# bfloat16/latent-diffusion-speech

Measured on AMD Instinct MI355X. Metric: mel_frames_per_sec, higher is better.
Workload: dtype f32; 1 GPU; configs[1]: batch=16x512-frame utterances per GPU, 50-step dpm-solver, unet1d denoiser, 80-ch mel; pipeline=sampler, utterances_per_gpu=16, frames=512, nfe=50, method=dpm-solver, parallelism=batch-shard x1

## Files before the change

latent-diffusion-speech_amd/csrc/attention_k4p.hip:

```cpp
#include "k4p.h"
#include "k8b3.h"
#include "kernels.h"

#include <hip/hip_ext.h>

#include <math.h>

namespace lds {

typedef float f32x16 __attribute__((ext_vector_type(16)));
typedef float f32x4 __attribute__((ext_vector_type(4)));
typedef float f32x2 __attribute__((ext_vector_type(2)));
typedef unsigned int att_u32x4 __attribute__((ext_vector_type(4)));
typedef _Float16 att_f16x8 __attribute__((ext_vector_type(8)));

static __device__ __forceinline__ void att_split8(const f32x4 e0, const f32x4 e1, att_u32x4& p1, att_u32x4& p2) {
    unsigned a[4], b[4];
    k8h_split_pair(e0[0], e0[1], a[0], b[0]);
    k8h_split_pair(e0[2], e0[3], a[1], b[1]);
    k8h_split_pair(e1[0], e1[1], a[2], b[2]);
    k8h_split_pair(e1[2], e1[3], a[3], b[3]);
    p1 = att_u32x4{a[0], a[1], a[2], a[3]};
    p2 = att_u32x4{b[0], b[1], b[2], b[3]};
}
static __device__ __forceinline__ f32x16 att_mfma3(const att_u32x4 a1, const att_u32x4 a2, const att_u32x4 b1, const att_u32x4 b2, f32x16 c) {
    c = __builtin_amdgcn_mfma_f32_32x32x16_f16(__builtin_bit_cast(att_f16x8, a2), __builtin_bit_cast(att_f16x8, b1), c, 0, 0, 0);
    c = __builtin_amdgcn_mfma_f32_32x32x16_f16(__builtin_bit_cast(att_f16x8, a1), __builtin_bit_cast(att_f16x8, b2), c, 0, 0, 0);
    c = __builtin_amdgcn_mfma_f32_32x32x16_f16(__builtin_bit_cast(att_f16x8, a1), __builtin_bit_cast(att_f16x8, b1), c, 0, 0, 0);
    return c;
}

template <int D, int NW, int NST, int KS = 1>
struct AttCfg {
    static constexpr int KB = 64;
    static constexpr int DQ = D / 8, DT = (D + 31) / 32;
    static constexpr int KROWS = DQ * 2;
    static constexpr int VCH = D / 4;
    static constexpr int KPW = KROWS / NW, VPW = VCH / NW;
    static constexpr int PER_TILE = KPW + VPW;
    static constexpr int STAGE = 2 * KB * D;
    static constexpr size_t LDS_BYTES = (size_t)NST * STAGE * sizeof(float) + 256;
    static_assert(KROWS % NW == 0 && VCH % NW == 0, "tile must split evenly over the waves");
    static_assert(KS == 1 || (size_t)(KS - 1) * (NW / KS) * (2 + 16 * DT) * 64 * sizeof(float) <= LDS_BYTES, "the join's partials reuse the K/V stages");
};

static __device__ __forceinline__ float max3(float a, float b, float c) {
    float d;
    asm("v_max3_f32 %0, %1, %2, %3" : "=v"(d) : "v"(a), "v"(b), "v"(c));
    return d;
}

template <int Y, int PER_TILE>
static __device__ __forceinline__ void att_wait_younger(int y) {
    if constexpr (Y == 0) {
        asm volatile("s_waitcnt vmcnt(0)" ::: "memory");
    } else {
        constexpr int N = (Y * PER_TILE > 63) ? 63 : Y * PER_TILE;
        if (y >= Y) asm volatile("s_waitcnt vmcnt(%0)" ::"n"(N) : "memory");
        else att_wait_younger<Y - 1, PER_TILE>(y);
    }
}

template <int D, int NW, int KPW, int VPW>
static __device__ __forceinline__ void att_issue_tile(const __amdgpu_buffer_rsrc_t rk, const __amdgpu_buffer_rsrc_t rv, const int* koff,
                                                      const int* voff, int wave, int kt, float* st) {
#pragma unroll
    for (int i = 0; i < KPW; ++i)
        __builtin_amdgcn_raw_ptr_buffer_load_lds(rk, (__attribute__((address_space(3))) void*)(st + (wave + NW * i) * 256), 16, koff[i], kt * (64 * 16), 0, 0);
#pragma unroll
    for (int i = 0; i < VPW; ++i)
        __builtin_amdgcn_raw_ptr_buffer_load_lds(rv, (__attribute__((address_space(3))) void*)(st + 64 * D + (wave + NW * i) * 256), 16, voff[i],
                                                 kt * (64 * D * 4), 0, 0);
}

template <int D, int NW, int NST, int KS, bool F16>
__global__ void __launch_bounds__(NW * 64) attention_k4p_kernel(const float* __restrict__ qk, const float* __restrict__ vt, float* __restrict__ out,
                                                                int C, int Tbuf, float scale2, int out_bf3, const int* __restrict__ lens, int lvl) {
    using Cfg = AttCfg<D, NW, NST, KS>;
    constexpr int NWQ = NW / KS;
    constexpr int KB = Cfg::KB, DQ = Cfg::DQ, DT = Cfg::DT, KPW = Cfg::KPW, VPW = Cfg::VPW, STAGE = Cfg::STAGE, PER_TILE = Cfg::PER_TILE;
    extern __shared__ __attribute__((aligned(16))) float smem[];
    const int lane = threadIdx.x & 63, wave = __builtin_amdgcn_readfirstlane((int)(threadIdx.x >> 6));
    const int c = lane & 31, h = lane >> 5;
    const int gx = gridDim.x, gy = gridDim.y, total = gx * gy * gridDim.z;
    const int id = (blockIdx.z * gy + blockIdx.y) * gx + blockIdx.x;
    const int per = total >> 3, rem = total & 7, xcd = id & 7;
    const int L = xcd * per + (xcd < rem ? xcd : rem) + (id >> 3);
    const int qblk = L % gx, hd = (L / gx) % gy, b = L / (gx * gy);
    const int qw = wave % NWQ, ks = wave / NWQ;
    const int tq = qblk * (NWQ * 32) + qw * 32 + c;
    const int T = ragged_len(lens, b, lvl, Tbuf);
    const int Tp = Tbuf + 2, T4 = (Tbuf + 3) & ~3;
    const float* qb = qk + ((long long)b * 2 * C + (long long)hd * D) * Tp;

    f32x4 qv[DQ];
#pragma unroll
    for (int kq = 0; kq < DQ; ++kq) {
        qv[kq] = f32x4{0.f, 0.f, 0.f, 0.f};
        if (tq < T) qv[kq] = *reinterpret_cast<const f32x4*>(qb + ((long long)(kq * 2 + h) * Tp + tq + 1) * 4);
    }

    const __amdgpu_buffer_rsrc_t rk =
        __builtin_amdgcn_make_buffer_rsrc(const_cast<float*>(qk + ((long long)b * 2 * C + C + (long long)hd * D) * Tp), 0, D * Tp * 4, 0x00020000);
    const __amdgpu_buffer_rsrc_t rv =
        __builtin_amdgcn_make_buffer_rsrc(const_cast<float*>(vt + ((long long)b * C + (long long)hd * D) * T4), 0, D * T4 * 4, 0x00020000);
    int koff[KPW], voff[VPW];
#pragma unroll
    for (int i = 0; i < KPW; ++i) koff[i] = (((wave + NW * i) * Tp) + lane + 1) * 16;
#pragma unroll
    for (int i = 0; i < VPW; ++i) voff[i] = ((wave + NW * i) * 64 + lane) * 16;
    const int nt = (qblk * (NWQ * 32) >= T) ? 0 : (T + KB - 1) / KB;
    for (int t = 0; t < NST - 1 && t < nt; ++t) att_issue_tile<D, NW, KPW, VPW>(rk, rv, koff, voff, wave, t, smem + t * STAGE);
#pragma unroll
    for (int kq = 0; kq < DQ; ++kq) qv[kq] *= scale2;
    att_u32x4 qh1[F16 ? DQ / 2 : 1], qh2[F16 ? DQ / 2 : 1];
    if constexpr (F16) {
#pragma unroll
        for (int t = 0; t < DQ / 2; ++t) att_split8(qv[2 * t], qv[2 * t + 1], qh1[t], qh2[t]);
    }

    f32x16 o[DT];
#pragma unroll
    for (int i = 0; i < DT; ++i)
#pragma unroll
        for (int r = 0; r < 16; ++r) o[i][r] = 0.f;
    float m_run = -INFINITY, l_run = 0.f;

    const bool resident = (KS == 4) && nt <= NST - 1;
    if (resident) {
        asm volatile("s_waitcnt vmcnt(0)" ::: "memory");
        __builtin_amdgcn_s_barrier();
        asm volatile("" ::: "memory");
    }
    int sc = 0, sn = NST - 1;
    for (int kt = 0; kt < nt; ++kt) {
        if (!resident) {
            const int younger = (nt - 1 - kt < NST - 2) ? (nt - 1 - kt) : (NST - 2);
            att_wait_younger<NST - 2, PER_TILE>(younger);
            __builtin_amdgcn_s_barrier();
            asm volatile("" ::: "memory");
            if (kt + NST - 1 < nt) att_issue_tile<D, NW, KPW, VPW>(rk, rv, koff, voff, wave, kt + NST - 1, smem + sn * STAGE);
        }
        const float* Kc = smem + sc * STAGE;
        const float* Vc = Kc + KB * D;
        const int h0 = (KS == 1) ? 0 : (KS == 2) ? ks : (ks & 1);
        const int h1 = (KS == 1) ? KB / 32 : (KS == 2 || (kt & 1) == (ks >> 1)) ? h0 + 1 : h0;
#pragma unroll 1
        for (int half = h0; half < h1; ++half) {
            const int kbase = kt * KB + half * 32;
            if (kbase >= T) break;
            f32x4 ka[DQ], va[4][DT];
#pragma unroll
            for (int kq = 0; kq < DQ; ++kq) ka[kq] = *reinterpret_cast<const f32x4*>(Kc + ((kq * 2 + h) * KB + half * 32 + c) * 4);
            __builtin_amdgcn_sched_barrier(0);
            f32x16 s;
// ... 53 lines not shown
#pragma unroll
                for (int ss = 0; ss < 2; ++ss) {
                    att_u32x4 p1, p2;
                    att_split8(f32x4{s[8 * ss], s[8 * ss + 1], s[8 * ss + 2], s[8 * ss + 3]}, f32x4{s[8 * ss + 4], s[8 * ss + 5], s[8 * ss + 6], s[8 * ss + 7]}, p1, p2);
#pragma unroll
                    for (int i = 0; i < DT; ++i) {
                        att_u32x4 v1, v2;
                        att_split8(va[2 * ss][i], va[2 * ss + 1][i], v1, v2);
                        o[i] = att_mfma3(v1, v2, p1, p2, o[i]);
                    }
                }
            } else {
#pragma unroll
                for (int g = 0; g < 4; ++g)
#pragma unroll
                    for (int i = 0; i < DT; ++i)
#pragma unroll
                        for (int e = 0; e < 4; ++e) o[i] = __builtin_amdgcn_mfma_f32_32x32x2f32(va[g][i][e], s[4 * g + e], o[i], 0, 0, 0);
            }
        }
        sc = (sc + 1 == NST) ? 0 : sc + 1;
        sn = (sn + 1 == NST) ? 0 : sn + 1;
    }
    if constexpr (KS >= 2) {
        __syncthreads();
        constexpr int RED = (2 + 16 * DT) * 64;
        if (ks >= 1) {
            float* red = smem + ((ks - 1) * NWQ + qw) * RED + lane;
            red[0] = m_run; red[64] = l_run;
#pragma unroll
            for (int i = 0; i < DT; ++i)
#pragma unroll
                for (int r = 0; r < 16; ++r) red[(2 + i * 16 + r) * 64] = o[i][r];
        }
        __syncthreads();
        if (ks >= 1) return;
#pragma unroll
        for (int q = 1; q < KS; ++q) {
            const float* red = smem + ((q - 1) * NWQ + qw) * RED + lane;
            const float m1 = red[0], l1 = red[64];
            const float m = fmaxf(m_run, m1);
            const float a0 = __builtin_amdgcn_exp2f(m_run - m), a1 = __builtin_amdgcn_exp2f(m1 - m);
            l_run = l_run * a0 + l1 * a1;
#pragma unroll
            for (int i = 0; i < DT; ++i)
#pragma unroll
                for (int r = 0; r < 16; ++r) o[i][r] = o[i][r] * a0 + red[(2 + i * 16 + r) * 64] * a1;
            m_run = m;
        }
    }
    float l;
    {
        const auto sw = __builtin_amdgcn_permlane32_swap(__float_as_uint(l_run), __float_as_uint(l_run), false, false);
        l = __uint_as_float(sw[0]) + __uint_as_float(sw[1]);
    }
    if (tq < Tbuf && out_bf3) {
        const bool live = tq < T;
        const float rl = 1.0f / l;
        char* ob = reinterpret_cast<char*>(out);
        const int npl = (out_bf3 == 2) ? 2 : 3;
#pragma unroll
        for (int i = 0; i < DT; ++i)
#pragma unroll
            for (int g = 0; g < 4; ++g) {
                if (i * 32 + 8 * g >= D) break;
                const int q = (hd * D + i * 32) / 8 + g;
                unsigned pa[3], pb[3];
                if (out_bf3 == 2) {
                    sp_split_pair<FMT_F16X2>(o[i][4 * g] * rl, o[i][4 * g + 1] * rl, pa);
                    sp_split_pair<FMT_F16X2>(o[i][4 * g + 2] * rl, o[i][4 * g + 3] * rl, pb);
                } else {
                    sp_split_pair<FMT_BF16X3>(o[i][4 * g] * rl, o[i][4 * g + 1] * rl, pa);
                    sp_split_pair<FMT_BF16X3>(o[i][4 * g + 2] * rl, o[i][4 * g + 3] * rl, pb);
                }
#pragma unroll
                for (int pl = 0; pl < 3; ++pl) {
                    if (pl >= npl) break;
                    char* e = ob + ((((long long)b * (C >> 3) + q) * npl + pl) * Tp + tq + 1) * 16 + h * 8;
                    k8_store_wt(e, live ? k8_u32x2{pa[pl], pb[pl]} : k8_u32x2{0u, 0u});
                    if (tq == 0) *reinterpret_cast<k8_u32x2*>(e - 16) = k8_u32x2{0u, 0u};
                    if (tq == Tbuf - 1) *reinterpret_cast<k8_u32x2*>(e + 16) = k8_u32x2{0u, 0u};
                }
            }
    } else if (tq < Tbuf) {
        const bool live = tq < T;
        const float rl = 1.0f / l;
        float* ob = out + (long long)b * C * Tp;
#pragma unroll
        for (int i = 0; i < DT; ++i)
#pragma unroll
            for (int g = 0; g < 4; ++g) {
                if (i * 32 + 8 * g >= D) break;
                const int q = (hd * D + i * 32) / 8 + g;
#pragma unroll
                for (int hh = 0; hh < 2; ++hh) {
                    const long long off = ((long long)(q * 2 + hh) * Tp + tq + 1) * 4 + 2 * h;
                    k4p_store_wt(ob + off, live ? f32x2{o[i][4 * g + hh] * rl, o[i][4 * g + 2 + hh] * rl} : f32x2{0.f, 0.f});
                    if (tq == 0) *reinterpret_cast<f32x2*>(ob + off - 4) = f32x2{0.f, 0.f};
                    if (tq == Tbuf - 1) *reinterpret_cast<f32x2*>(ob + off + 4) = f32x2{0.f, 0.f};
                }
            }
    }
}

template <int D, int NW, int NST, int KS, bool F16>
static hipError_t launch_cfg(const float* qk, const float* vt, float* out, int B, int C, int T, int heads, float scale, int out_bf3, const int* lens, int lvl, hipStream_t s) {
    using Cfg = AttCfg<D, NW, NST, KS>;
    auto kern = attention_k4p_kernel<D, NW, NST, KS, F16>;
    if (Cfg::LDS_BYTES > 48 * 1024) {
        static std::atomic<unsigned long long> attr_done{0};
        hipError_t e = ensure_max_dynamic_lds(reinterpret_cast<const void*>(kern), attr_done);
        if (e != hipSuccess) return e;
    }
    constexpr int QPB = NW / KS * 32;
    hipEvent_t e0, e1;
    if (prof_attach_events(&e0, &e1)) hipExtLaunchKernelGGL(kern, dim3((T + QPB - 1) / QPB, heads, B), dim3(NW * 64), Cfg::LDS_BYTES, s, e0, e1, 0, qk, vt, out, C, T, scale, out_bf3, lens, lvl);
    else hipLaunchKernelGGL(kern, dim3((T + QPB - 1) / QPB, heads, B), dim3(NW * 64), Cfg::LDS_BYTES, s, qk, vt, out, C, T, scale, out_bf3, lens, lvl);
    return hipGetLastError();
}

template <int D, bool F16>
static hipError_t launch_dk(const float* qk, const float* vt, float* out, int B, int C, int T, int heads, int out_bf3, int tile_batch, const int* lens, int lvl, hipStream_t s) {
    const float scale = 1.4426950408889634f / sqrtf((float)D);
    constexpr int NST = (D == 64) ? 2 : 3;
    const long long hb = (long long)heads * (tile_batch > 0 ? tile_batch : 16);
    if ((long long)((T + 127) / 128) * hb >= 512) return launch_cfg<D, 4, NST, 1, F16>(qk, vt, out, B, C, T, heads, scale, out_bf3, lens, lvl, s);
    constexpr int NSTL = (D == 32) ? 9 : (D == 48) ? 5 : 4;
    if (tile_batch > 0 && T > 64 && (long long)((T + 63) / 64) * hb < 256) return launch_cfg<D, 4, NSTL, 4, F16>(qk, vt, out, B, C, T, heads, scale, out_bf3, lens, lvl, s);
    if (T > 32) return launch_cfg<D, 4, NST, 2, F16>(qk, vt, out, B, C, T, heads, scale, out_bf3, lens, lvl, s);
    return launch_cfg<D, 1, 2, 1, F16>(qk, vt, out, B, C, T, heads, scale, out_bf3, lens, lvl, s);
}

static hipError_t attention_any(const float* qk, const float* vt, float* out, int B, int C, int T, int heads, int out_bf3, bool math_f16, int tile_batch, hipStream_t s,
                                const int* lens = nullptr, int lvl = 0) {
    if (C % heads) return hipErrorInvalidValue;
    ProfScope ps(s, math_f16 ? "attention_f16" : "attention", 4.0 * B * (double)T * T * C, 4.0 * 4.0 * B * C * T, true);
    if (math_f16) {
        switch (C / heads) {
            case 32: return launch_dk<32, true>(qk, vt, out, B, C, T, heads, out_bf3, tile_batch, lens, lvl, s);
            case 48: return launch_dk<48, true>(qk, vt, out, B, C, T, heads, out_bf3, tile_batch, lens, lvl, s);
            case 64: return launch_dk<64, true>(qk, vt, out, B, C, T, heads, out_bf3, tile_batch, lens, lvl, s);
            default: return hipErrorInvalidValue;
        }
    }
    switch (C / heads) {
        case 32: return launch_dk<32, false>(qk, vt, out, B, C, T, heads, out_bf3, tile_batch, lens, lvl, s);
        case 48: return launch_dk<48, false>(qk, vt, out, B, C, T, heads, out_bf3, tile_batch, lens, lvl, s);
        case 64: return launch_dk<64, false>(qk, vt, out, B, C, T, heads, out_bf3, tile_batch, lens, lvl, s);
        default: return hipErrorInvalidValue;
    }
}
hipError_t launch_attention_k4p(const float* qk, const float* vt, float* out, int B, int C, int T, int heads, hipStream_t s, int tile_batch, const int* lens, int lvl) {
    return attention_any(qk, vt, out, B, C, T, heads, 0, false, tile_batch, s, lens, lvl);
}
hipError_t launch_attention_k4p_out_bf3(const float* qk, const float* vt, void* out, int B, int C, int T, int heads, hipStream_t s, int fmt, int tile_batch, const int* lens, int lvl) {
    return attention_any(qk, vt, (float*)out, B, C, T, heads, fmt == FMT_F16X2 ? 2 : 1, fmt == FMT_F16X2, tile_batch, s, lens, lvl);
}
template <int NW, int NST, int KS>
__global__ void __launch_bounds__(NW * 64) attention_k4p_rel_kernel(const float* __restrict__ qk, const float* __restrict__ vt, const float* __restrict__ relp,
                                                                    float* __restrict__ out, int C, int Tbuf, float scale2, const int* __restrict__ qlens,
                                                                    const int* __restrict__ klens, int left, int right) {
    constexpr int D = 64;
    using Cfg = AttCfg<D, NW, NST, KS>;
    constexpr int NWQ = NW / KS;
    constexpr int KB = Cfg::KB, DQ = Cfg::DQ, DT = Cfg::DT, KPW = Cfg::KPW, VPW = Cfg::VPW, STAGE = Cfg::STAGE, PER_TILE = Cfg::PER_TILE;
    static_assert(KS == 1 || KS == 2, "no latency-mode variant");
    extern __shared__ __attribute__((aligned(16))) float smem[];
    const int lane = threadIdx.x & 63, wave = __builtin_amdgcn_readfirstlane((int)(threadIdx.x >> 6));
    const int c = lane & 31, h = lane >> 5;
    const int gx = gridDim.x, gy = gridDim.y, total = gx * gy * gridDim.z;
    const int id = (blockIdx.z * gy + blockIdx.y) * gx + blockIdx.x;
    const int per = total >> 3, rem = total & 7, xcd = id & 7;
    const int Lid = xcd * per + (xcd < rem ? xcd : rem) + (id >> 3);
    const int qblk = Lid % gx, hd = (Lid / gx) % gy, b = Lid / (gx * gy);
    const int qw = wave % NWQ, ks = wave / NWQ;
    const int q0 = qblk * (NWQ * 32) + qw * 32;
    const int tq = q0 + c;
    const int Tq = qlens ? (qlens[b] < Tbuf ? qlens[b] : Tbuf) : Tbuf;
    const int Tk = klens ? (klens[b] < Tq ? klens[b] : Tq) : Tq;
    const int Tp = Tbuf + 2, T4 = (Tbuf + 3) & ~3;
    const float* qb = qk + ((long long)b * 2 * C + (long long)hd * D) * Tp;

    f32x4 qv[DQ];
#pragma unroll
// ... 58 lines not shown
            __builtin_amdgcn_sched_barrier(0);
            if (kbase - q0 - 31 >= right) {
#pragma unroll
                for (int r = 0; r < 16; ++r) s[r] += pR;
            } else if (kbase + 31 - q0 <= -left) {
#pragma unroll
                for (int r = 0; r < 16; ++r) s[r] += pL;
            } else {
#pragma unroll
                for (int r = 0; r < 16; ++r) {
                    int d = kbase + (r & 3) + 8 * (r >> 2) + 4 * h - tq;
                    d = d < -left ? -left : (d > right ? right : d);
                    s[r] += rp[d + left];
                }
            }
            if (kbase + 32 > Tk) {
#pragma unroll
                for (int r = 0; r < 16; ++r)
                    if (kbase + (r & 3) + 8 * (r >> 2) + 4 * h >= Tk) s[r] = -INFINITY;
            }
            float mt = max3(max3(max3(s[0], s[1], s[2]), max3(s[3], s[4], s[5]), max3(s[6], s[7], s[8])),
                            max3(max3(s[9], s[10], s[11]), max3(s[12], s[13], s[14]), s[15]), m_run);
            {
                const auto sw = __builtin_amdgcn_permlane32_swap(__float_as_uint(mt), __float_as_uint(mt), false, false);
                mt = max3(mt, __uint_as_float(sw[0]), __uint_as_float(sw[1]));
            }
            const float alpha = __builtin_amdgcn_exp2f(m_run - mt);
            m_run = mt;
            const f32x2 mm = {mt, mt}, aa = {alpha, alpha};
            f32x2 lsum = {0.f, 0.f};
#pragma unroll
            for (int r = 0; r < 16; r += 2) {
                const f32x2 d = f32x2{s[r], s[r + 1]} - mm;
                s[r] = __builtin_amdgcn_exp2f(d[0]);
                s[r + 1] = __builtin_amdgcn_exp2f(d[1]);
                lsum += f32x2{s[r], s[r + 1]};
            }
            l_run = fmaf(l_run, alpha, lsum[0] + lsum[1]);
#pragma unroll
            for (int i = 0; i < DT; ++i)
#pragma unroll
                for (int r = 0; r < 16; r += 2) {
                    const f32x2 t = f32x2{o[i][r], o[i][r + 1]} * aa;
                    o[i][r] = t[0]; o[i][r + 1] = t[1];
                }
#pragma unroll
            for (int g = 0; g < 4; ++g)
#pragma unroll
                for (int i = 0; i < DT; ++i)
#pragma unroll
                    for (int e = 0; e < 4; ++e) o[i] = __builtin_amdgcn_mfma_f32_32x32x2f32(va[g][i][e], s[4 * g + e], o[i], 0, 0, 0);
        }
        sc = (sc + 1 == NST) ? 0 : sc + 1;
        sn = (sn + 1 == NST) ? 0 : sn + 1;
    }
    if constexpr (KS == 2) {
        __syncthreads();
        constexpr int RED = (2 + 16 * DT) * 64;
        if (ks >= 1) {
            float* red = smem + qw * RED + lane;
            red[0] = m_run; red[64] = l_run;
#pragma unroll
            for (int i = 0; i < DT; ++i)
#pragma unroll
                for (int r = 0; r < 16; ++r) red[(2 + i * 16 + r) * 64] = o[i][r];
        }
        __syncthreads();
        if (ks >= 1) return;
        const float* red = smem + qw * RED + lane;
        const float m1 = red[0], l1 = red[64];
        const float m = fmaxf(m_run, m1);
        const float a0 = (m_run == -INFINITY) ? 0.f : __builtin_amdgcn_exp2f(m_run - m), a1 = (m1 == -INFINITY) ? 0.f : __builtin_amdgcn_exp2f(m1 - m);
        l_run = l_run * a0 + l1 * a1;
#pragma unroll
        for (int i = 0; i < DT; ++i)
#pragma unroll
            for (int r = 0; r < 16; ++r) o[i][r] = o[i][r] * a0 + red[(2 + i * 16 + r) * 64] * a1;
    }
    float l;
    {
        const auto sw = __builtin_amdgcn_permlane32_swap(__float_as_uint(l_run), __float_as_uint(l_run), false, false);
        l = __uint_as_float(sw[0]) + __uint_as_float(sw[1]);
    }
    if (tq < Tbuf) {
        const bool live = tq < Tq;
        const float rl = 1.0f / l;
        float* ob = out + (long long)b * C * Tp;
#pragma unroll
        for (int i = 0; i < DT; ++i)
#pragma unroll
            for (int g = 0; g < 4; ++g) {
                const int q = (hd * D + i * 32) / 8 + g;
#pragma unroll
                for (int hh = 0; hh < 2; ++hh) {
                    const long long off = ((long long)(q * 2 + hh) * Tp + tq + 1) * 4 + 2 * h;
                    k4p_store_wt(ob + off, live ? f32x2{o[i][4 * g + hh] * rl, o[i][4 * g + 2 + hh] * rl} : f32x2{0.f, 0.f});
                    if (tq == 0) *reinterpret_cast<f32x2*>(ob + off - 4) = f32x2{0.f, 0.f};
                    if (tq == Tbuf - 1) *reinterpret_cast<f32x2*>(ob + off + 4) = f32x2{0.f, 0.f};
                }
            }
    }
}

template <int NW, int NST, int KS>
static hipError_t launch_rel_cfg(const float* qk, const float* vt, const float* relp, float* out, int B, int C, int T, int heads, const int* qlens,
                                 const int* klens, int left, int right, hipStream_t s) {
    using Cfg = AttCfg<64, NW, NST, KS>;
    auto kern = attention_k4p_rel_kernel<NW, NST, KS>;
    if (Cfg::LDS_BYTES > 48 * 1024) {
        static std::atomic<unsigned long long> attr_done{0};
        hipError_t e = ensure_max_dynamic_lds(reinterpret_cast<const void*>(kern), attr_done);
        if (e != hipSuccess) return e;
    }
    constexpr int QPB = NW / KS * 32;
    const float scale = 1.4426950408889634f / 8.0f;
    hipEvent_t e0, e1;
    const dim3 grid((T + QPB - 1) / QPB, heads, B);
    if (prof_attach_events(&e0, &e1)) hipExtLaunchKernelGGL(kern, grid, dim3(NW * 64), Cfg::LDS_BYTES, s, e0, e1, 0, qk, vt, relp, out, C, T, scale, qlens, klens, left, right);
    else hipLaunchKernelGGL(kern, grid, dim3(NW * 64), Cfg::LDS_BYTES, s, qk, vt, relp, out, C, T, scale, qlens, klens, left, right);
    return hipGetLastError();
}

hipError_t launch_attention_k4p_rel(const float* qk, const float* vt, const float* relp, float* out, int B, int C, int T, int heads, const int* qlens,
                                    const int* klens, int left, int right, hipStream_t s) {
    if (B <= 0 || heads < 1 || C != heads * 64 || T <= 0 || left < 0 || right < 0 || left + right + 1 > kW2vbertRelStride) return hipErrorInvalidValue;
    ProfScope ps(s, "attention_rel", 4.0 * B * (double)T * T * C, 4.0 * 4.0 * B * C * T, true);
    if ((long long)((T + 127) / 128) * heads * 16 >= 512) return launch_rel_cfg<4, 2, 1>(qk, vt, relp, out, B, C, T, heads, qlens, klens, left, right, s);
    if (T > 32) return launch_rel_cfg<4, 2, 2>(qk, vt, relp, out, B, C, T, heads, qlens, klens, left, right, s);
    return launch_rel_cfg<1, 2, 1>(qk, vt, relp, out, B, C, T, heads, qlens, klens, left, right, s);
}

hipError_t launch_attention_k4p_f16math(const float* qk, const float* vt, float* out, int B, int C, int T, int heads, hipStream_t s, int tile_batch) {
    return attention_any(qk, vt, out, B, C, T, heads, 0, true, tile_batch, s);
}

}
```

latent-diffusion-speech_amd/csrc/conv_dma.hip:

```cpp
#include "gn_chan.h"
#include "k4p.h"
#include "kernels.h"

#include <hip/hip_ext.h>

#include <stdio.h>
#include <stdlib.h>

namespace lds {

typedef float f32x16 __attribute__((ext_vector_type(16)));
typedef float f32x4 __attribute__((ext_vector_type(4)));
typedef float f32x2 __attribute__((ext_vector_type(2)));

static __device__ __forceinline__ float erf_fast(float x) {
    const float ax = fabsf(x);
    const float t = __builtin_amdgcn_rcpf(fmaf(0.3275911f, ax, 1.0f));
    float pl = fmaf(1.061405429f, t, -1.453152027f);
    pl = fmaf(pl, t, 1.421413741f);
    pl = fmaf(pl, t, -0.284496736f);
    pl = fmaf(pl, t, 0.254829592f);
    const float e = __builtin_amdgcn_exp2f(ax * ax * -1.4426950408889634f);
    return copysignf(fmaf(-pl * t, e, 1.0f), x);
}

template <int CTRL, int ROW_MASK, bool BOUND>
static __device__ __forceinline__ float dpp_add(float v) {
    return v + __builtin_bit_cast(float, __builtin_amdgcn_update_dpp(0, __builtin_bit_cast(int, v), CTRL, ROW_MASK, 0xf, BOUND));
}
static __device__ __forceinline__ float wave_sum_to_lane63(float v) {
    v = dpp_add<0x111, 0xf, true>(v);
    v = dpp_add<0x112, 0xf, true>(v);
    v = dpp_add<0x114, 0xf, true>(v);
    v = dpp_add<0x118, 0xf, true>(v);
    v = dpp_add<0x142, 0xa, false>(v);
    v = dpp_add<0x143, 0xc, false>(v);
    return v;
}

template <int BM, int BN, int KT, int STRIDE, bool UPS, int BK, int NST, int DIL = 1>
struct DmaCfg {
    static constexpr bool SPLIT = BM == 32;
    static constexpr int TM = SPLIT ? 1 : BM / 64, TN = BN / 64;
    static constexpr int KR = BK / 4;
    static constexpr int XW = UPS ? (BN / 2 + 2) : ((BN - 1) * STRIDE + (KT - 1) * DIL + 1);
    static constexpr int WI = KT * KR * BM / 64;
    static constexpr int WPW = WI / 4;
    static constexpr int RPW = KR / 4;
    static constexpr int NXI = (RPW * XW + 63) / 64;
    static constexpr int PER_TILE = WPW + NXI;
    static constexpr int KQW = SPLIT ? BK / 16 : BK / 8;
    static constexpr int G = KT * KQW;
    static constexpr int NB = (G % 3 == 0 && TM * TN < 4) ? 3 : 2;
    static constexpr int NACC = (TM * TN >= 2) ? 1 : 2;
    static constexpr int STAGE = KT * BK * BM + KR * XW * 4;
    static constexpr size_t LDS_BYTES = (size_t)NST * STAGE * sizeof(float);
    static constexpr int OCC_LDS = (int)((160 * 1024) / LDS_BYTES);
    static constexpr int OCC = (TM * TN >= 4) ? (OCC_LDS < 2 ? OCC_LDS : 2) : (OCC_LDS < 4 ? (OCC_LDS < 1 ? 1 : OCC_LDS) : 4);
    static_assert(WI % 4 == 0 && KR % 4 == 0, "tile does not split evenly over 4 waves");
    static_assert(!SPLIT || (BN == 64 && BK % 16 == 0), "split-K tile is 32 x 64");
};

template <int BM, int BN, int KT, int STRIDE, bool UPS, int BK, int NST, int DIL = 1, bool VOC = false, bool GNF = false, bool GELU = false, int ACT2 = 0>
struct DmaKernel {
    using Cfg = DmaCfg<BM, BN, KT, STRIDE, UPS, BK, NST, DIL>;
    static constexpr int TM = Cfg::TM, TN = Cfg::TN, KR = Cfg::KR, XW = Cfg::XW, WPW = Cfg::WPW, RPW = Cfg::RPW, NXI = Cfg::NXI;
    static constexpr int G = Cfg::G, NB = Cfg::NB, NACC = Cfg::NACC, STAGE = Cfg::STAGE, PER_TILE = Cfg::PER_TILE, KQW = Cfg::KQW;
    static constexpr bool SPLIT = Cfg::SPLIT;

    const DmaConvArgs& p;
    float* smem;
    int lane, wave, c, h, wm, wn, ks, b, m0, t0;
    int ksp, kc0, ctile;
    int Lout;
    float gcg[GNF ? 8 : 1], gkc;
    GnPart gp0, gp1;
    float gs, gsn, ginv;
    int kofs_a, kofs_b;
    int woff[WPW];
    int xoff[NXI];
    __amdgpu_buffer_rsrc_t rw, rx1, rx2;
    bool xact[NXI];
    int arow;
    int bcol[TN];
    f32x16 acc[NACC][TM][TN];
    f32x4 aop[NB][TM], bop[NB][TN];
    float lmu[TN], lrs[TN];
    static constexpr bool EARLY = TM * TN == 1 || VOC;
    f32x2 rsv[EARLY ? TM * TN * 8 : 1];
    float kbv[EARLY ? TM * 16 : 1];

    __device__ __forceinline__ DmaKernel(const DmaConvArgs& p_, float* s_) : p(p_), smem(s_) {}

    __device__ __forceinline__ void setup_keep_acc() {
        const int tid = threadIdx.x;
        lane = tid & 63;
        wave = __builtin_amdgcn_readfirstlane(tid >> 6);
        c = lane & 31; h = lane >> 5;
        wm = SPLIT ? 0 : wave >> 1; ks = SPLIT ? wave >> 1 : 0; wn = wave & 1;
        kofs_a = ks * KQW * 2 * BM * 4; kofs_b = ks * KQW * 2 * XW * 4;
        const int nMb = p.Mp / BM;
        const int gx = gridDim.x, total = gx * gridDim.y;
        const int id = blockIdx.y * gx + blockIdx.x;
        const int xcd = id & 7, slot = id >> 3, per = total >> 3, rem = total & 7;
        const int L = xcd * per + (xcd < rem ? xcd : rem) + slot;
        const int mb = L % nMb;
        const int tb = L / nMb;
        const int nN = gx / nMb;
        const int nb = tb % nN;
        const int by = tb / nN, S = p.ksplit > 1 ? p.ksplit : 1;
        b = by / S; ksp = by - b * S;
        kc0 = ksp * (p.Ci / BK / S);
        ctile = (b * nN + nb) * nMb + mb;
        m0 = mb * BM; t0 = nb * BN;
        Lout = ragged_len(p.lens, b, p.lvl_out, p.To);
#pragma unroll
        for (int i = 0; i < WPW; ++i) {
            const int q = (wave + 4 * i) * 64 + lane;
            const int tap = q / (KR * BM);
            const int rem = q - tap * (KR * BM);
            const int rr = rem / BM, m = rem - rr * BM;
            woff[i] = ((tap * (p.Ci / 4) + rr) * p.Mp + m0 + m) * 16;
        }
        const int Tp = p.Tsrc + 2 * p.xpad;
        const int e0 = UPS ? (((t0 - 1) >> 1) + p.xpad) : (t0 * STRIDE - p.pad + p.xpad);
#pragma unroll
        for (int i = 0; i < NXI; ++i) {
            const int qq = i * 64 + lane;
            const int rl = qq / XW, col = qq - rl * XW;
            xact[i] = qq < RPW * XW;
            xoff[i] = ((wave * RPW + rl) * Tp + e0 + col) * 16;
        }
        rw = __builtin_amdgcn_make_buffer_rsrc(const_cast<float*>(p.w), 0, KT * p.Ci * p.Mp * 4, 0x00020000);
        rx1 = __builtin_amdgcn_make_buffer_rsrc(const_cast<float*>(p.x1 + (long long)b * p.C1 * Tp), 0, p.C1 * Tp * 4, 0x00020000);
        rx2 = __builtin_amdgcn_make_buffer_rsrc(const_cast<float*>(p.x2 ? p.x2 + (long long)b * p.C2 * Tp : p.x1), 0, p.C2 * Tp * 4, 0x00020000);
        arow = wm * TM * 32 + c;
#pragma unroll
        for (int j = 0; j < TN; ++j) bcol[j] = wn * TN * 32 + j * 32 + c;
    }
    __device__ __forceinline__ bool dead_tile() const { return !VOC && p.lens && t0 >= Lout; }
    __device__ __forceinline__ int voc_len() const { return p.vlen[b]; }
    __device__ __forceinline__ void setup() {
        setup_keep_acc();
#pragma unroll
        for (int a = 0; a < NACC; ++a)
#pragma unroll
            for (int i = 0; i < TM; ++i)
#pragma unroll
                for (int j = 0; j < TN; ++j)
#pragma unroll
                    for (int r = 0; r < 16; ++r) acc[a][i][j][r] = 0.f;
    }

    __device__ __forceinline__ void issue_tile(int kc, float* st) {
        const int ws = kc * (KR * 16) * p.Mp;
#pragma unroll
        for (int i = 0; i < WPW; ++i)
            __builtin_amdgcn_raw_ptr_buffer_load_lds(rw, (__attribute__((address_space(3))) void*)(st + ((wave + 4 * i) * 64) * 4), 16, woff[i], ws, 0, 0);
        const int k0 = kc * BK;
        const bool s2 = k0 >= p.C1;
        const int xsoff = (s2 ? k0 - p.C1 : k0) * (p.Tsrc + 2 * p.xpad) * 4;
        float* xs = st + KT * BK * BM + wave * RPW * XW * 4;
#pragma unroll
        for (int i = 0; i < NXI; ++i)
            if (xact[i]) {
                if (s2) __builtin_amdgcn_raw_ptr_buffer_load_lds(rx2, (__attribute__((address_space(3))) void*)(xs + i * 64 * 4), 16, xoff[i], xsoff, 0, 0);
                else __builtin_amdgcn_raw_ptr_buffer_load_lds(rx1, (__attribute__((address_space(3))) void*)(xs + i * 64 * 4), 16, xoff[i], xsoff, 0, 0);
            }
    }

    template <int SLOT>
    __device__ __forceinline__ void load_ops(const float* st, int tap, int kq) {
        const float* wt = st + ((tap * KR + kq * 2 + h) * BM + arow) * 4 + kofs_a;
        const float* xs = st + KT * BK * BM + (kq * 2 + h) * XW * 4 + kofs_b;
#pragma unroll
        for (int i = 0; i < TM; ++i) aop[SLOT][i] = *reinterpret_cast<const f32x4*>(wt + i * 32 * 4);
#pragma unroll
        for (int j = 0; j < TN; ++j) {
            const int col = UPS ? (((t0 + bcol[j] + tap - 1) >> 1) - ((t0 - 1) >> 1)) : (bcol[j] * STRIDE + tap * DIL);
            bop[SLOT][j] = *reinterpret_cast<const f32x4*>(xs + col * 4);
        }
    }
    template <int SLOT>
    __device__ __forceinline__ void mfma_ops() {
        if constexpr (GNF) {
#pragma unroll
            for (int j = 0; j < TN; ++j) bop[SLOT][j] *= gs;
        }
#pragma unroll
        for (int jj = 0; jj < 4; ++jj)
#pragma unroll
            for (int i = 0; i < TM; ++i)
#pragma unroll
                for (int j = 0; j < TN; ++j)
                    acc[jj % NACC][i][j] = __builtin_amdgcn_mfma_f32_32x32x2f32(aop[SLOT][i][jj], bop[SLOT][j][jj], acc[jj % NACC][i][j], 0, 0, 0);
    }
    template <int g0, int g1>
    __device__ __forceinline__ void preload(const float* cur) {
        if constexpr (g0 < g1 && g0 < G) {
            load_ops<g0 % NB>(cur, g0 / KQW, g0 % KQW);
            preload<g0 + 1, g1>(cur);
        }
    }
    __device__ __forceinline__ void tile_sync(int kc, int nk, float* cur) {
        const int younger = (nk - 2 - kc < NST - 2) ? (nk - 2 - kc) : (NST - 2);
        wait_younger<NST - 2>(younger);
        asm volatile("s_waitcnt lgkmcnt(0)" ::: "memory");
        __builtin_amdgcn_s_barrier();
        asm volatile("" ::: "memory");
        if (kc + NST < nk) issue_tile(kc0 + kc + NST, cur);
    }
    template <int g>
    __device__ __forceinline__ void kstep(float* cur, const float* nxt, int kc, int nk) {
        if constexpr (g < G) {
            constexpr int gp = g + NB - 1;
            if constexpr (gp < G) {
                load_ops<gp % NB>(cur, gp / KQW, gp % KQW);
            } else {
                if (kc + 1 < nk) {
                    if constexpr (gp == G) tile_sync(kc, nk, cur);
                    load_ops<gp % NB>(nxt, (gp - G) / KQW, (gp - G) % KQW);
                }
            }
            mfma_ops<g % NB>();
            __builtin_amdgcn_sched_barrier(0);
            kstep<g + 1>(cur, nxt, kc, nk);
        }
    }

    __device__ __forceinline__ void ln_columns() {
#pragma unroll
        for (int j = 0; j < TN; ++j) {
            const int n = t0 + wn * TN * 32 + j * 32 + c;
            const bool ok = n < p.To;
            const float2* src = p.ln_part + (long long)b * p.ln_np * p.Tsrc + (ok ? n : 0);
            ln_column_stats(src, p.Tsrc, p.ln_np, p.ln_eps, ok, lmu[j], lrs[j]);
        }
    }

    __device__ __forceinline__ float* gnf_tail() const { return smem + NST * STAGE + BM; }
    __device__ __forceinline__ int gnf_group(int k) const {
        const int pos = (kc0 + k) * BK + ks * (SPLIT ? BK / 2 : BK);
        const int g = (int)(((float)pos + 0.5f) * ginv);
        return g < p.gnf_groups ? g : p.gnf_groups - 1;
    }
    __device__ __forceinline__ void gnf_request() {
        const int G_ = p.gnf_groups, gsz = p.Ci / G_;
        const int gTv = ragged_len(p.lens, b, p.lvl_in, p.Tsrc);
        ginv = 1.0f / (float)gsz;
        gp0 = gn_part_load(p.gnf_part, b, p.Ci, p.Tsrc, gsz >> 4, wave, lane, 0, gTv);
        gp1 = gn_part_load(p.gnf_part, b, p.Ci, p.Tsrc, gsz >> 4, (wave + 4 < G_) ? wave + 4 : wave, lane, 0, gTv);
        if ((int)threadIdx.x < BM) {
            const int m = m0 + (int)threadIdx.x;
            gkc = p.gnf_c2[m];
#pragma unroll
            for (int g = 0; g < 8; ++g) gcg[g] = (g < G_) ? p.gnf_cg[g * p.Mp + m] : 0.f;
        }
    }
    __device__ __forceinline__ void gnf_prepare() {
        const int G_ = p.gnf_groups, gsz = p.Ci / G_;
        float* tail = gnf_tail();
#pragma unroll
        for (int e = 0; e < 2; ++e) {
            const int g = wave + 4 * e;
            float rs = 1.f, rm = 0.f;
            if (g < G_) {
                float mu, var;
                gnf_group_stats(p.gnf_part, b, p.Ci, p.Tsrc, gsz >> 4, g, lane, e ? gp1 : gp0, mu, var, ragged_len(p.lens, b, p.lvl_in, p.Tsrc));
                rs = __builtin_amdgcn_rsqf(var + p.gnf_eps); rm = rs * mu;
            }
            if (lane == 0) { tail[g] = rs; tail[8 + g] = rm; }
        }
        asm volatile("s_waitcnt lgkmcnt(0)" ::: "memory");
    }
    __device__ __forceinline__ void gnf_rows() {
        const float* tail = gnf_tail();
        if ((int)threadIdx.x < BM) {
            float kc = gkc;
#pragma unroll
            for (int g = 0; g < 8; ++g) kc = fmaf(-tail[8 + g], gcg[g], kc);
            smem[NST * STAGE + threadIdx.x] = kc;
        }
        gs = tail[gnf_group(0)];
        gsn = tail[gnf_group(1)];
    }
    __device__ __forceinline__ void gnf_advance(int k) {
        gs = gsn;
        gsn = gnf_tail()[gnf_group(k + 2)];
    }

    template <int Y>
    __device__ __forceinline__ void wait_younger(int y) {
        if constexpr (Y == 0) {
            asm volatile("s_waitcnt vmcnt(0)" ::: "memory");
        } else {
            constexpr int N = (Y * PER_TILE > 63) ? 63 : Y * PER_TILE;
            if (y >= Y) asm volatile("s_waitcnt vmcnt(%0)" ::"n"(N) : "memory");
            else wait_younger<Y - 1>(y);
        }
    }

    __device__ __forceinline__ bool res_tile(int tile0, int n) const {
        return p.res && tile0 < p.plain_from && tile0 < p.Cout && n < p.To;
    }
    __device__ __forceinline__ void early_loads() {
#pragma unroll
        for (int i = 0; i < TM; ++i) {
            const int tile0 = m0 + wm * TM * 32 + i * 32;
#pragma unroll
            for (int j = 0; j < TN; ++j) {
                const int n = t0 + wn * TN * 32 + j * 32 + c;
                f32x2* rs = rsv + (i * TN + j) * 8;
#pragma unroll
                for (int e = 0; e < 8; ++e) rs[e] = f32x2{0.f, 0.f};
                if (res_tile(tile0, n)) {
                    const int Tpo = p.To + 2 * p.opad;
                    const float* rb = p.res + (long long)b * k4p_ck() * Tpo + k4p_off(tile0, n);
#pragma unroll
                    for (int e = 0; e < 8; ++e) rs[e] = *reinterpret_cast<const f32x2*>(rb + e * Tpo * 4);
                }
            }
#pragma unroll
            for (int r = 0; r < 16; ++r) kbv[i * 16 + r] = (p.bias && !p.ln_part) ? p.bias[tile0 + (r & 3) + 8 * (r >> 2) + 4 * h] : 0.f;
        }
    }

    __device__ __forceinline__ void mainloop() {
        static_assert(G % NB == 0 && NB - 1 <= G, "ring slots must keep their phase across K-steps");
        const int nk = p.Ci / BK / (p.ksplit > 1 ? p.ksplit : 1);
        if constexpr (GNF) gnf_request();
        if constexpr (EARLY) early_loads();
        for (int t = 0; t < NST && t < nk; ++t) issue_tile(kc0 + t, smem + t * STAGE);
        if (p.ln_part) ln_columns();
        if constexpr (GNF) gnf_prepare();
        wait_younger<NST - 1>((nk - 1 < NST - 1) ? nk - 1 : NST - 1);
        __builtin_amdgcn_s_barrier();
        asm volatile("" ::: "memory");
        if constexpr (GNF) gnf_rows();
        preload<0, NB - 1>(smem);
        int sc = 0;
        for (int kc = 0; kc < nk; ++kc) {
            const int sn = (sc + 1 == NST) ? 0 : sc + 1;
            kstep<0>(smem + sc * STAGE, smem + sn * STAGE, kc, nk);
            sc = sn;
            if constexpr (GNF) gnf_advance(kc);
        }
        if constexpr (GNF) __syncthreads();
    }

    __device__ __forceinline__ void finalize(bool geglu) {
        if constexpr (NACC == 2) {
#pragma unroll
            for (int i = 0; i < TM; ++i)
#pragma unroll
                for (int j = 0; j < TN; ++j) acc[0][i][j] += acc[1][i][j];
        }
        const bool ln = p.ln_part != nullptr;
        if (EARLY && !ln) {
#pragma unroll
            for (int i = 0; i < TM; ++i)
#pragma unroll
                for (int j = 0; j < TN; ++j)
#pragma unroll
                    for (int r = 0; r < 16; ++r) acc[0][i][j][r] += kbv[i * 16 + r];
        } else if (ln || p.bias) {
            float k1[TM][16], k2[TM][16];
#pragma unroll
            for (int i = 0; i < TM; ++i)
#pragma unroll
                for (int r = 0; r < 16; ++r) {
                    const int m = m0 + wm * TM * 32 + i * 32 + (r & 3) + 8 * (r >> 2) + 4 * h;
                    k1[i][r] = ln ? p.ln_c1[m] : 0.f;
                    k2[i][r] = ln ? p.ln_c2[m] : p.bias[m];
                }
#pragma unroll
            for (int i = 0; i < TM; ++i)
#pragma unroll
                for (int j = 0; j < TN; ++j)
#pragma unroll
                    for (int r = 0; r < 16; ++r) {
                        const float v = acc[0][i][j][r];
                        acc[0][i][j][r] = ln ? lrs[j] * (v - lmu[j] * k1[i][r]) + k2[i][r] : v + k2[i][r];
                    }
        }
        if constexpr (GNF) {
#pragma unroll
            for (int i = 0; i < TM; ++i)
#pragma unroll
                for (int r = 0; r < 16; ++r) {
                    const float kc = smem[NST * STAGE + wm * TM * 32 + i * 32 + (r & 3) + 8 * (r >> 2) + 4 * h];
#pragma unroll
                    for (int j = 0; j < TN; ++j) acc[0][i][j][r] += kc;
                }
        }
        if (geglu) {
#pragma unroll
            for (int j = 0; j < TN; ++j)
#pragma unroll
                for (int r = 0; r < 16; ++r) {
                    const float g = acc[0][TM - 1][j][r];
                    if constexpr (ACT2 == 2) acc[0][0][j][r] *= 1.0f / (1.0f + expf(-g));
                    else acc[0][0][j][r] *= 0.5f * g * (1.0f + erf_fast(g * 0.70710678118654752440f));
                }
        }
        if constexpr (ACT2 == 1) {
#pragma unroll
            for (int i = 0; i < TM; ++i)
#pragma unroll
                for (int j = 0; j < TN; ++j)
#pragma unroll
                    for (int r = 0; r < 16; ++r) {
                        const float v = acc[0][i][j][r];
                        acc[0][i][j][r] = v / (1.0f + expf(-v));
                    }
        }
        if constexpr (GELU) {
#pragma unroll
            for (int i = 0; i < TM; ++i)
#pragma unroll
                for (int j = 0; j < TN; ++j)
#pragma unroll
                    for (int r = 0; r < 16; ++r) {
                        const float v = acc[0][i][j][r];
                        acc[0][i][j][r] = 0.5f * v * (1.0f + erf_fast(v * 0.70710678118654752440f));
                    }
        }
// ... 16 lines not shown
            if (c0 + rl < Cn) ob[rl * p.To] = v;
        }
    }

    __device__ __forceinline__ void store_vt(int c0, int i, int j, int n) {
        const int T4 = (p.To + 3) & ~3, D = p.vt_D, Cv = p.Cout - p.plain_from;
        if (n >= T4) return;
        const bool real = n < p.To;
        const int head0 = c0 / D, rem0 = c0 - head0 * D;
        float* ob = p.out2 + (long long)b * Cv * T4 + (long long)(n >> 2) * D * 4 + (n & 3);
#pragma unroll
        for (int r = 0; r < 16; ++r) {
            const int rl = (r & 3) + 8 * (r >> 2) + 4 * h;
            int d = rem0 + rl, head = head0;
            if (d >= D) { d -= D; ++head; }
            if (c0 + rl < Cv) ob[(long long)head * D * T4 + d * 4] = real ? acc[0][i][j][r] : 0.f;
        }
    }

    __device__ __forceinline__ int k4p_off(int tile0, int n) const { return (((tile0 >> 3) * 2) * (p.To + 2 * p.opad) + n + p.opad) * 4 + 2 * h; }
    __device__ __forceinline__ int k4p_ck() const { return (p.plain_from < p.Cout) ? p.plain_from : p.Cout; }

    __device__ __forceinline__ void add_residual(int tile0, int i, int j, int n) {
        if (n >= p.To) return;
        f32x2 rv[8];
        if constexpr (EARLY) {
#pragma unroll
            for (int e = 0; e < 8; ++e) rv[e] = rsv[(i * TN + j) * 8 + e];
        } else {
            const int Tpo = p.To + 2 * p.opad;
            const float* rb = p.res + (long long)b * k4p_ck() * Tpo + k4p_off(tile0, n);
#pragma unroll
            for (int e = 0; e < 8; ++e) rv[e] = *reinterpret_cast<const f32x2*>(rb + e * Tpo * 4);
        }
#pragma unroll
        for (int g = 0; g < 4; ++g)
#pragma unroll
            for (int hh = 0; hh < 2; ++hh) {
                acc[0][i][j][4 * g + hh] += rv[2 * g + hh][0];
                acc[0][i][j][4 * g + 2 + hh] += rv[2 * g + hh][1];
            }
    }

    __device__ __forceinline__ void add_running_sum(int tile0, int i, int j, int n) {
        if (n >= p.To) return;
        const int Tpo = p.To + 2 * p.opad;
        const float* ab = p.acc_in + (long long)b * (p.out_plain ? p.Cout : k4p_ck()) * Tpo + k4p_off(tile0, n);
        f32x2 av[8];
#pragma unroll
        for (int e = 0; e < 8; ++e) av[e] = *reinterpret_cast<const f32x2*>(ab + e * Tpo * 4);
#pragma unroll
        for (int g = 0; g < 4; ++g)
#pragma unroll
            for (int hh = 0; hh < 2; ++hh) {
                acc[0][i][j][4 * g + hh] += av[2 * g + hh][0];
                acc[0][i][j][4 * g + 2 + hh] += av[2 * g + hh][1];
            }
    }

    __device__ __forceinline__ void store_phases(int tile0, int i, int j, int n) {
        const int lg = p.ph_log2, Tpo = p.ph_Tout + 2 * p.opad;
        const long long ob = (long long)b * p.ph_Cout * Tpo;
        const int Lv = p.vlen ? voc_len() : 0x7fffffff;
#pragma unroll
        for (int r = 0; r < 16; ++r) {
            const int m = tile0 + (r & 3) + 8 * (r >> 2) + 4 * h;
            const int co = m >> lg, f = (n << lg) + (m & ((1 << lg) - 1)) - p.ph_tpad;
            const bool ok = n < p.To && f >= 0 && f < p.ph_Tout && co < p.ph_Cout;
            const long long off = ob + (long long)(((co >> 3) * 2 + (co & 1)) * Tpo + f + p.opad) * 4 + ((co & 7) >> 1);
            const float v = (f < Lv) ? acc[0][i][j][r] : 0.f;
            if (ok) {
                p.out[off] = v;
                if (p.out_act) p.out_act[off] = (v >= 0.f) ? v : v * p.act_slope;
            }
        }
    }

    __device__ __forceinline__ void store_k4p(int tile0, int i, int j, int n) {
        const int Tpo = p.To + 2 * p.opad;
        const int Ck = k4p_ck();
        const bool ok = n < p.To;
        const long long o0 = (long long)b * Ck * Tpo + k4p_off(tile0, n);
        float* ob = p.out + o0;
        if (ok) {
            if constexpr (VOC) {
            if constexpr (BN < 256) {
                if (p.vlen && n >= voc_len()) {
#pragma unroll
                    for (int r = 0; r < 16; ++r) acc[0][i][j][r] = 0.f;
                }
            }
            if (p.out_div != 1.0f) {
#pragma unroll
                for (int r = 0; r < 16; ++r) acc[0][i][j][r] = acc[0][i][j][r] / p.out_div;
            }
            if (p.act_slope != 0.f && p.out_act) {
#pragma unroll
                for (int g = 0; g < 4; ++g)
#pragma unroll
                    for (int hh = 0; hh < 2; ++hh) k4p_store_wt(ob + (2 * g + hh) * Tpo * 4, f32x2{acc[0][i][j][4 * g + hh], acc[0][i][j][4 * g + 2 + hh]});
                ob = p.out_act + o0;
            }
            if (p.act_slope != 0.f) {
#pragma unroll
                for (int r = 0; r < 16; ++r) { const float v = acc[0][i][j][r]; acc[0][i][j][r] = (v >= 0.f) ? v : v * p.act_slope; }
            }
            }
#pragma unroll
            for (int g = 0; g < 4; ++g)
#pragma unroll
                for (int hh = 0; hh < 2; ++hh)
                    k4p_store_wt(ob + (2 * g + hh) * Tpo * 4, f32x2{acc[0][i][j][4 * g + hh], acc[0][i][j][4 * g + 2 + hh]});
            if (p.opad == 1) {
                if (n == 0) {
#pragma unroll
                    for (int e = 0; e < 8; ++e) *reinterpret_cast<f32x2*>(ob + e * Tpo * 4 - 4) = f32x2{0.f, 0.f};
                }
                if (n == p.To - 1) {
#pragma unroll
                    for (int e = 0; e < 8; ++e) *reinterpret_cast<f32x2*>(ob + e * Tpo * 4 + 4) = f32x2{0.f, 0.f};
                }
            }
        }
        if (p.gnpart_out) {
            const float k0 = __builtin_bit_cast(float, __builtin_amdgcn_readfirstlane(__builtin_bit_cast(int, acc[0][i][j][0])));
            const float k1 = __builtin_bit_cast(float, __builtin_amdgcn_readfirstlane(__builtin_bit_cast(int, acc[0][i][j][8])));
            float a1 = 0.f, a2 = 0.f, b1 = 0.f, b2 = 0.f;
#pragma unroll
            for (int r = 0; r < 8; ++r) {
                const float d0 = acc[0][i][j][r] - k0, d1 = acc[0][i][j][r + 8] - k1;
                a1 += d0; a2 = fmaf(d0, d0, a2);
                b1 += d1; b2 = fmaf(d1, d1, b2);
            }
            if (n >= Lout) { a1 = 0.f; a2 = 0.f; b1 = 0.f; b2 = 0.f; }
            a1 = wave_sum_to_lane63(a1); a2 = wave_sum_to_lane63(a2);
            b1 = wave_sum_to_lane63(b1); b2 = wave_sum_to_lane63(b2);
            const int n0 = n - c;
            const int nv = (Lout - n0 < 32) ? Lout - n0 : 32;
            if (lane == 63 && nv > 0) {
                const float cnt = 16.0f * (float)nv, rc = 1.0f / cnt;
                float2* gp = p.gnpart_out + ((long long)b * (Ck >> 4) + (tile0 >> 4)) * ((p.To + 31) >> 5) + (n0 >> 5);
                gp[0] = make_float2(k0 + a1 * rc, fmaxf(a2 - a1 * a1 * rc, 0.f));
                if (tile0 + 16 < Ck) gp[(p.To + 31) >> 5] = make_float2(k1 + b1 * rc, fmaxf(b2 - b1 * b1 * rc, 0.f));
            }
        }
        if (p.lnpart_out) {
            float s1 = 0.f;
#pragma unroll
            for (int r = 0; r < 16; ++r) s1 += acc[0][i][j][r];
            const float m16 = s1 * (1.0f / 16.0f);
            float qv = 0.f;
#pragma unroll
            for (int r = 0; r < 16; ++r) { const float d = acc[0][i][j][r] - m16; qv += d * d; }
            const float mo = __shfl_xor(m16, 32, 64), qo = __shfl_xor(qv, 32, 64);
            const float d = mo - m16;
            if (h == 0 && ok)
                p.lnpart_out[((long long)b * (Ck >> 5) + (tile0 >> 5)) * p.To + n] = make_float2(0.5f * (m16 + mo), (qv + qo) + d * d * 8.0f);
        }
    }

    __device__ __forceinline__ int tile_ch(int i, bool geglu) const {
        return geglu ? (m0 + wm * 64) / 2 : (m0 + wm * TM * 32 + i * 32);
    }

    __device__ __forceinline__ bool join_halves() {
        if constexpr (NACC == 2) acc[0][0][0] += acc[1][0][0];
        __syncthreads();
        float* red = smem + wn * 16 * 64 + lane;
        if (ks == 1) {
#pragma unroll
            for (int r = 0; r < 16; ++r) red[r * 64] = acc[0][0][0][r];
        }
        __syncthreads();
        if (ks == 1) return false;
#pragma unroll
        for (int r = 0; r < 16; ++r) acc[0][0][0][r] += red[r * 64];
        if constexpr (NACC == 2) acc[1][0][0] = f32x16{0.f, 0.f, 0.f, 0.f, 0.f, 0.f, 0.f, 0.f, 0.f, 0.f, 0.f, 0.f, 0.f, 0.f, 0.f, 0.f};
        return true;
    }

    __device__ __forceinline__ bool cluster_join() {
        const int S = p.ksplit;
        if constexpr (NACC == 2) {
#pragma unroll
            for (int i = 0; i < TM; ++i)
#pragma unroll
                for (int j = 0; j < TN; ++j) {
                    acc[0][i][j] += acc[1][i][j];
#pragma unroll
// ... 29 lines not shown
            const float* pq = all + (long long)q * (TM * TN * 1024);
#pragma unroll
            for (int i = 0; i < TM; ++i)
#pragma unroll
                for (int j = 0; j < TN; ++j)
#pragma unroll
                    for (int r = 0; r < 16; ++r) acc[0][i][j][r] += __hip_atomic_load(pq + ((i * TN + j) * 16 + r) * 64, __ATOMIC_RELAXED, __HIP_MEMORY_SCOPE_AGENT);
        }
        if (threadIdx.x == 0) __hip_atomic_store(p.kcount + ctile, 0u, __ATOMIC_RELAXED, __HIP_MEMORY_SCOPE_AGENT);
        return true;
    }

    __device__ __forceinline__ void epilogue() {
        const bool geglu = (p.epi == EPI_GEGLU || (ACT2 == 2 && p.epi == EPI_GLU)) && (TM == 2);
        if constexpr (SPLIT) {
            if (!join_halves()) return;
        }
        if constexpr (TM * TN <= 2 && !VOC) {
            if (p.ksplit > 1) {
                if (!cluster_join()) return;
            }
        }
        finalize(geglu);
        const int ni = geglu ? 1 : TM;
        if (p.res) {
#pragma unroll
            for (int i = 0; i < TM; ++i) {
                if (i >= ni) break;
#pragma unroll
                for (int j = 0; j < TN; ++j) {
                    const int tile0 = tile_ch(i, geglu);
                    if (tile0 < p.plain_from && tile0 < p.Cout) add_residual(tile0, i, j, t0 + wn * TN * 32 + j * 32 + c);
                }
            }
        }
        if constexpr (VOC) {
            if (p.acc_in) {
#pragma unroll
                for (int i = 0; i < TM; ++i)
#pragma unroll
                    for (int j = 0; j < TN; ++j) {
                        const int tile0 = tile_ch(i, geglu);
                        if (tile0 < p.Cout) add_running_sum(tile0, i, j, t0 + wn * TN * 32 + j * 32 + c);
                    }
            }
        } else {
            if (p.lens) {
#pragma unroll
                for (int j = 0; j < TN; ++j) {
                    if (t0 + wn * TN * 32 + j * 32 + c >= Lout) {
#pragma unroll
                        for (int i = 0; i < TM; ++i)
#pragma unroll
                            for (int r = 0; r < 16; ++r) acc[0][i][j][r] = 0.f;
                    }
                }
            }
        }
#pragma unroll
        for (int i = 0; i < TM; ++i) {
            if (i >= ni) break;
#pragma unroll
            for (int j = 0; j < TN; ++j) {
                const int n = t0 + wn * TN * 32 + j * 32 + c;
                const int tile0 = tile_ch(i, geglu);
                if constexpr (VOC && KT == 2) {
                    if (p.ph_Tout) { store_phases(tile0, i, j, n); continue; }
                }
                if (p.out_plain) store_plain(p.out, p.Cout, tile0, i, j, n);
                else if (tile0 >= p.plain_from) {
                    if (p.vt_D) store_vt(tile0 - p.plain_from, i, j, n);
                    else store_plain(p.out2, p.Cout - p.plain_from, tile0 - p.plain_from, i, j, n);
                }
                else if (tile0 < p.Cout) store_k4p(tile0, i, j, n);
            }
        }
    }
};

template <int BM, int BN, int KT, int STRIDE, bool UPS, int BK, int NST, int DIL = 1, bool VOC = false, bool GNF = false, bool GELU = false, int ACT2 = 0>
__global__ void __launch_bounds__(256, ((VOC && KT == 2) ? 2 : DmaCfg<BM, BN, KT, STRIDE, UPS, BK, NST, DIL>::OCC)) conv_dma_kernel(const DmaConvArgs p) {
    extern __shared__ __attribute__((aligned(16))) float smem[];
    DmaKernel<BM, BN, KT, STRIDE, UPS, BK, NST, DIL, VOC, GNF, GELU, ACT2> k(p, smem);
    k.setup();
    if (!k.dead_tile()) k.mainloop();
    k.epilogue();
}

struct DmaPairArgs { DmaConvArgs a3, a1; };

template <int BM, int BN, int BK3, int BK1, int NST>
struct PairCfg {
    using C3 = DmaCfg<BM, BN, 3, 1, false, BK3, NST, 1>;
    using C1 = DmaCfg<BM, BN, 1, 1, false, BK1, NST, 1>;
    static constexpr size_t LDS_BYTES = C3::LDS_BYTES > C1::LDS_BYTES ? C3::LDS_BYTES : C1::LDS_BYTES;
    static constexpr int OCC = C3::OCC < C1::OCC ? C3::OCC : C1::OCC;
    static_assert(C3::NACC == C1::NACC && C3::TM == C1::TM && C3::TN == C1::TN && C3::SPLIT == C1::SPLIT, "the phases share the accumulators");
};

template <int BM, int BN, int BK3, int BK1, int NST>
__global__ void __launch_bounds__(256, (PairCfg<BM, BN, BK3, BK1, NST>::OCC)) conv_dma_pair_kernel(const DmaPairArgs pp) {
    extern __shared__ __attribute__((aligned(16))) float smem[];
    using K3 = DmaKernel<BM, BN, 3, 1, false, BK3, NST, 1, false>;
    using K1 = DmaKernel<BM, BN, 1, 1, false, BK1, NST, 1, false>;
    K1 k1(pp.a1, smem);
    {
        K3 k3(pp.a3, smem);
        k3.setup();
        if (!k3.dead_tile()) k3.mainloop();
#pragma unroll
        for (int a = 0; a < K3::NACC; ++a)
#pragma unroll
            for (int i = 0; i < K3::TM; ++i)
#pragma unroll
                for (int j = 0; j < K3::TN; ++j) k1.acc[a][i][j] = k3.acc[a][i][j];
    }
    __syncthreads();
    k1.setup_keep_acc();
    if (!k1.dead_tile()) k1.mainloop();
    k1.epilogue();
}

static thread_local char g_dcfg[96] = "";
const char* conv_dma_last_config() { return g_dcfg; }

template <int BM, int BN, int KT, int STRIDE, bool UPS, int BK, int NST, int DIL = 1, bool VOC = false, bool GNF = false, bool GELU = false, int ACT2 = 0>
static hipError_t launch_dma_cfg(const DmaConvArgs& a, hipStream_t s) {
    using Cfg = DmaCfg<BM, BN, KT, STRIDE, UPS, BK, NST, DIL>;
    if (GNF != (a.gnf_part != nullptr) || GELU != (a.epi == EPI_GELU) || (ACT2 == 1) != (a.epi == EPI_SWISH) || (ACT2 == 2) != (a.epi == EPI_GLU)) return hipErrorInvalidValue;
    const size_t lds_bytes = Cfg::LDS_BYTES + (GNF ? (BM + 32) * sizeof(float) : 0);
    const int nN = (a.To + BN - 1) / BN;
    const int S = a.ksplit > 1 ? a.ksplit : 1;
    if (S > 1 && (Cfg::TM * Cfg::TN > 2 || VOC || (a.Ci / BK) % S)) return hipErrorInvalidValue;
    dim3 grid((a.Mp / BM) * nN, a.B * S);
    auto kern = conv_dma_kernel<BM, BN, KT, STRIDE, UPS, BK, NST, DIL, VOC, GNF, GELU, ACT2>;
    if (lds_bytes > 48 * 1024) {
        static std::atomic<unsigned long long> attr_done{0};
        hipError_t e = ensure_max_dynamic_lds(reinterpret_cast<const void*>(kern), attr_done);
        if (e != hipSuccess) return e;
    }
    const char* gtag = GNF ? " GNF" : GELU ? " GELU" : ACT2 == 1 ? " SWISH" : ACT2 == 2 ? " GLU" : "";
    if (!VOC && S > 1) snprintf(g_dcfg, sizeof(g_dcfg), "BM%d BN%d KT%d S%d U%d BK%d NST%d KS%d%s grid %ux%u lds %zu", BM, BN, KT, STRIDE, (int)UPS, BK, NST, S, gtag, grid.x, grid.y, lds_bytes);
    else if (!VOC) snprintf(g_dcfg, sizeof(g_dcfg), "BM%d BN%d KT%d S%d U%d BK%d NST%d%s grid %ux%u lds %zu", BM, BN, KT, STRIDE, (int)UPS, BK, NST, gtag, grid.x, grid.y, lds_bytes);
    else snprintf(g_dcfg, sizeof(g_dcfg), "BM%d BN%d KT%d S%d U%d BK%d NST%d D%d grid %ux%u lds %zu", BM, BN, KT, STRIDE, (int)UPS, BK, NST, DIL, grid.x, grid.y, Cfg::LDS_BYTES);
    hipEvent_t e0, e1;
    if (prof_attach_events(&e0, &e1)) hipExtLaunchKernelGGL(kern, grid, dim3(256), lds_bytes, s, e0, e1, 0, a);
    else hipLaunchKernelGGL(kern, grid, dim3(256), lds_bytes, s, a);
    return hipGetLastError();
}

#define DCASE(BM, BN, KT, ST, UP, BK, NS) return launch_dma_cfg<BM, BN, KT, ST, UP, BK, NS>(a, s)

static void dma_pick(const DmaConvArgs& a, int cfg, int& bm, int& bn, int& bk, int& nst) {
    const bool k32 = (a.Ci % 32 == 0) && (a.C1 % 32 == 0), k64 = (a.Ci % 64 == 0) && (a.C1 % 64 == 0);
    const long long kNominalBatch = a.tile_batch > 0 ? a.tile_batch : 16;
    auto blocks = [&](int bm, int bn) -> long long { return (a.Mp % bm) ? -1 : (long long)(a.Mp / bm) * ((a.To + bn - 1) / bn) * kNominalBatch; };
    if (cfg) {
        bm = cfg / 1000000; bn = (cfg / 1000) % 1000; bk = (cfg / 10) % 100; nst = cfg % 10;
    } else if (a.stride == 1 && !a.ups && a.epi != EPI_GEGLU && k32 && (blocks(64, 64) <= 256 || (blocks(64, 64) < 512 && blocks(64, 64) % 256))) {
        bm = 32; bn = 64; bk = (a.KT == 1 && k64) ? 64 : 32; nst = 2;
    } else {
        struct Cand { int bm, bn, bk, nst; double eff; };
        Cand cands[3];
        int nc = 0;
        if (a.stride == 2 || a.ups) {
            cands[nc++] = {64, 64, 32, 2, 0.93};
        } else if (a.KT == 3) {
            cands[nc++] = {64, 64, 32, 2, 0.93};
            if (a.Mp % 128 == 0) cands[nc++] = {128, 128, 16, 2, 1.0};
        } else if (a.epi == EPI_GEGLU) {
            if (a.To > 64) cands[nc++] = {128, 128, a.Ci >= 384 ? 16 : 32, 2, 1.0};
            else cands[nc++] = {128, 64, 32, 2, 0.97};
        } else {
            if (a.Ci > 512) cands[nc++] = {64, 64, 64, 2, 0.93};
            else if (blocks(64, 64) <= 768) cands[nc++] = {64, 64, 32, 2, 0.93};
            else cands[nc++] = {64, 64, 16, 3, 0.93};
            if (a.Mp % 128 == 0) cands[nc++] = {128, 64, 32, 2, 0.97};
        }
        double best = 1e300;
        bm = cands[0].bm; bn = cands[0].bn; bk = cands[0].bk; nst = cands[0].nst;
        for (int i = 0; i < nc; ++i) {
            const Cand& c = cands[i];
            const long long nblk = blocks(c.bm, c.bn);
            if (nblk < 0) continue;
            const int xw = a.ups ? c.bn / 2 + 2 : (c.bn - 1) * a.stride + a.KT;
            const double lds = 4.0 * c.nst * (a.KT * c.bk * c.bm + (c.bk / 4) * xw * 4);
            int r = (int)(160.0 * 1024 / lds);
            r = r < 1 ? 1 : (r > 4 ? 4 : r);
            if (c.bm * c.bn >= 128 * 128 && r > 2) r = 2;
            const long long n = (nblk + 255) / 256;
            static const double e[5] = {1.0, 0.62, 0.9, 1.0, 1.0};
            const double cost = ((double)(n / r) * r / e[r] + (double)(n % r) / e[n % r]) * c.bm * c.bn / c.eff;
            if (cost < best) { best = cost; bm = c.bm; bn = c.bn; bk = c.bk; nst = c.nst; }
        }
        if (bm == 128 && bn == 128 && (long long)(a.Mp / 128) * ((a.To + 127) / 128) * a.B < 192) bn = 64;
    }
}

static int cluster_split(const DmaConvArgs& a, int bm, int bn, int nk, int nk2, int min_steps) {
    if (a.tile_batch <= 0 || !a.kpart || !a.kcount || a.voc || bm * bn > 128 * 64) return 1;
    const int blk = bm * bn > 64 * 64 ? 2 : 1;
    const long long tiles = (long long)(a.Mp / bm) * ((a.To + bn - 1) / bn) * a.B;
    if (tiles * 4 > a.kcount_cap) return 1;
    int S = 1;
    while (S < 16 && tiles * S * 2 <= 256 && nk % (S * 2) == 0 && nk / (S * 2) >= min_steps && (nk2 == 0 || (nk2 % (S * 2) == 0)) &&
           tiles * 4 * (S * 2) * blk * 1024 <= a.kpart_cap)
        S *= 2;
    return S;
}

template <int BM, int BN, int BK3, int BK1, int NST>
static hipError_t launch_pair_cfg(const DmaConvArgs& a3, const DmaConvArgs& a1, hipStream_t s) {
    using Cfg = PairCfg<BM, BN, BK3, BK1, NST>;
    const int nN = (a1.To + BN - 1) / BN;
    const int S = a1.ksplit > 1 ? a1.ksplit : 1;
    if (S > 1 && (Cfg::C1::TM * Cfg::C1::TN != 1 || a3.ksplit != a1.ksplit || (a3.Ci / BK3) % S || (a1.Ci / BK1) % S)) return hipErrorInvalidValue;
    dim3 grid((a1.Mp / BM) * nN, a1.B * S);
    auto kern = conv_dma_pair_kernel<BM, BN, BK3, BK1, NST>;
    if (Cfg::LDS_BYTES > 48 * 1024) {
        static std::atomic<unsigned long long> attr_done{0};
        hipError_t e = ensure_max_dynamic_lds(reinterpret_cast<const void*>(kern), attr_done);
        if (e != hipSuccess) return e;
    }
    if (S > 1) snprintf(g_dcfg, sizeof(g_dcfg), "BM%d BN%d KT3+1 S1 U0 BK%d+%d NST%d KS%d grid %ux%u lds %zu", BM, BN, BK3, BK1, NST, S, grid.x, grid.y, Cfg::LDS_BYTES);
    else snprintf(g_dcfg, sizeof(g_dcfg), "BM%d BN%d KT3+1 S1 U0 BK%d+%d NST%d grid %ux%u lds %zu", BM, BN, BK3, BK1, NST, grid.x, grid.y, Cfg::LDS_BYTES);
    DmaPairArgs pp{a3, a1};
    hipEvent_t e0, e1;
    if (prof_attach_events(&e0, &e1)) hipExtLaunchKernelGGL(kern, grid, dim3(256), Cfg::LDS_BYTES, s, e0, e1, 0, pp);
    else hipLaunchKernelGGL(kern, grid, dim3(256), Cfg::LDS_BYTES, s, pp);
    return hipGetLastError();
}

static int pair_variant(const DmaConvArgs& a3, const DmaConvArgs& a1) {
    auto plain = [](const DmaConvArgs& a) {
        return !a.voc && a.stride == 1 && !a.ups && a.dil == 1 && a.epi == EPI_NONE && a.xpad == 1 && a.opad == 1 && !a.ln_part && !a.ph_Tout && a.act_slope == 0.f &&
               !a.acc_in && a.out_div == 1.0f && a.Ci % 16 == 0 && a.C1 % 16 == 0 && a.Mp % 64 == 0 && a.B > 0 && a.To > 0;
    };
    if (!plain(a3) || !plain(a1) || a3.KT != 3 || a3.pad != 1 || a1.KT != 1 || a1.pad != 0 || a3.Mp != a1.Mp || a3.To != a1.To || a3.B != a1.B ||
        a3.Tsrc != a1.Tsrc || a1.res || a1.out_plain || a1.plain_from < a1.Cout || a1.lnpart_out)
        return 0;
    int bm, bn, bk, nst;
    dma_pick(a3, 0, bm, bn, bk, nst);
    const bool k3_32 = (a3.Ci % 32 == 0) && (a3.C1 % 32 == 0);
    const bool k1_64 = (a1.Ci % 64 == 0) && (a1.C1 % 64 == 0), k1_32 = (a1.Ci % 32 == 0) && (a1.C1 % 32 == 0);
    if (!k3_32 || bk != 32 || nst != 2 || !k1_32 || bn != 64 || (bm != 32 && bm != 64)) return 0;
    return (bm << 16) | (bn << 8) | (k1_64 ? 64 : 32);
}
bool conv_dma_pair_applies(const DmaConvArgs& a3, const DmaConvArgs& a1) { return pair_variant(a3, a1) != 0; }

hipError_t launch_conv_dma_pair(const DmaConvArgs& a3_, const DmaConvArgs& a1_, hipStream_t s) {
    DmaConvArgs a3 = a3_, a1 = a1_;
    const int pv = pair_variant(a3, a1);
    if (pv) {
        const int bm = pv >> 16, bn = (pv >> 8) & 255, bk1 = pv & 255;
        a3.ksplit = a1.ksplit = cluster_split(a1, bm, bn, a3.Ci / 32, a1.Ci / bk1, 1);
    }
    switch (pv) {
        case (32 << 16) | (64 << 8) | 64: return launch_pair_cfg<32, 64, 32, 64, 2>(a3, a1, s);
        case (32 << 16) | (64 << 8) | 32: return launch_pair_cfg<32, 64, 32, 32, 2>(a3, a1, s);
        case (64 << 16) | (64 << 8) | 64: return launch_pair_cfg<64, 64, 32, 64, 2>(a3, a1, s);
        case (64 << 16) | (64 << 8) | 32: return launch_pair_cfg<64, 64, 32, 32, 2>(a3, a1, s);
        default: return hipErrorNotSupported;
    }
}

hipError_t launch_conv_dma(const DmaConvArgs& a_, int cfg, hipStream_t s) {
    DmaConvArgs a = a_;
    a.ksplit = 1;
    if (a.Ci % 16 || a.C1 % 16 || a.Mp % 64 || a.B <= 0 || a.To <= 0 || a.xpad < 1 || a.opad < 1 || a.pad < 0 || a.pad > a.xpad) return hipErrorInvalidValue;
    if (a.voc) {
        if (a.stride != 1 || a.ups || a.epi != EPI_NONE || cfg != 0) return hipErrorInvalidValue;
        if (a.ph_Tout) {
            if (a.KT != 2 || a.dil != 1 || a.pad != 1 || a.res || a.acc_in || a.out_plain || a.out_div != 1.0f || a.ph_log2 < 0 || a.ph_log2 > 4 ||
                a.ph_Cout << a.ph_log2 != a.Co || a.ph_Cout % 8)
                return hipErrorInvalidValue;
            return launch_dma_cfg<64, 128, 2, 1, false, 16, 2, 1, true>(a, s);
        }
#define VCASE(KT_, D_) if (a.KT == KT_ && a.dil == D_) return launch_dma_cfg<64, 128, KT_, 1, false, 16, 2, D_, true>(a, s)
        if (a.Mp == 64 && a.KT == 11 && a.To >= 1024 && !a.vlen) {
#define WCASE(D_) if (a.dil == D_) return launch_dma_cfg<64, 256, 11, 1, false, 16, 2, D_, true>(a, s)
            WCASE(1); WCASE(3); WCASE(5);
#undef WCASE
        }
        VCASE(3, 1); VCASE(3, 3); VCASE(3, 5); VCASE(7, 1); VCASE(7, 3); VCASE(7, 5); VCASE(11, 1); VCASE(11, 3); VCASE(11, 5);
#undef VCASE
        return hipErrorInvalidValue;
    }
    if (a.dil != 1 || a.act_slope != 0.f || a.acc_in || a.out_div != 1.0f || a.ph_Tout) return hipErrorInvalidValue;
    if (a.KT != 1 && a.KT != 3 && !(a.KT == 2 && a.stride == 2 && (a.epi == EPI_GELU || a.epi == EPI_NONE))) return hipErrorInvalidValue;
    const bool k32 = (a.Ci % 32 == 0) && (a.C1 % 32 == 0), k64 = (a.Ci % 64 == 0) && (a.C1 % 64 == 0);
    int bm, bn, bk, nst;
    if (a.epi == EPI_GLU) {
        DmaConvArgs t = a;
        t.epi = EPI_GEGLU;
        dma_pick(t, cfg, bm, bn, bk, nst);
    } else {
        dma_pick(a, cfg, bm, bn, bk, nst);
    }
    if ((a.epi == EPI_GEGLU || a.epi == EPI_GLU) && bm != 128) return hipErrorInvalidValue;
    if (a.Mp % bm) return hipErrorInvalidValue;
// ... 34 lines not shown
            if (k32) ECASE(64, 64, 1, 1, 32, 2);
            ECASE(64, 64, 1, 1, 16, 2);
        } else if (a.KT == 3 && a.stride == 1) {
            if (bm == 128 && bn == 128) ECASE(128, 128, 3, 1, 16, 2);
            if (bm == 128 && bn == 64) ECASE(128, 64, 3, 1, 16, 2);
            if (k32) ECASE(64, 64, 3, 1, 32, 2);
            ECASE(64, 64, 3, 1, 16, 2);
        } else if (a.KT == 3 && a.stride == 2) {
            if (k32) ECASE(64, 64, 3, 2, 32, 2);
            ECASE(64, 64, 3, 2, 16, 2);
        } else if (a.KT == 2 && a.stride == 2) {
            if (k32) ECASE(64, 64, 2, 2, 32, 2);
            ECASE(64, 64, 2, 2, 16, 2);
        }
#undef ECASE
        return hipErrorInvalidValue;
    }
    if (cfg == 0) a.ksplit = cluster_split(a, bm, bn, a.Ci / bk, 0, 2);
    const int key = a.KT * 100 + a.stride * 10 + (a.ups ? 1 : 0);
    const int tk = bm * 1000 + bn;
    if (key == 110) {
        if (tk == 64064) {
            if (bk == 64 && nst == 2) DCASE(64, 64, 1, 1, false, 64, 2);
            if (bk == 64 && nst == 3) DCASE(64, 64, 1, 1, false, 64, 3);
            if (bk == 32 && nst == 2) DCASE(64, 64, 1, 1, false, 32, 2);
            if (bk == 32 && nst == 3) DCASE(64, 64, 1, 1, false, 32, 3);
            if (bk == 16 && nst == 2) DCASE(64, 64, 1, 1, false, 16, 2);
            if (bk == 16 && nst == 3) DCASE(64, 64, 1, 1, false, 16, 3);
            if (bk == 64 && nst == 4) DCASE(64, 64, 1, 1, false, 64, 4);
            if (bk == 32 && nst == 4) DCASE(64, 64, 1, 1, false, 32, 4);
            if (bk == 32 && nst == 5) DCASE(64, 64, 1, 1, false, 32, 5);
            if (bk == 16 && nst == 4) DCASE(64, 64, 1, 1, false, 16, 4);
            if (bk == 16 && nst == 6) DCASE(64, 64, 1, 1, false, 16, 6);
        } else if (tk == 32064) {
            if (bk == 64) DCASE(32, 64, 1, 1, false, 64, 2);
            if (bk == 32) DCASE(32, 64, 1, 1, false, 32, 2);
        } else if (tk == 128064) {
            if (bk == 32 && nst == 2) DCASE(128, 64, 1, 1, false, 32, 2);
            if (bk == 32 && nst == 3) DCASE(128, 64, 1, 1, false, 32, 3);
            if (bk == 16 && nst == 2) DCASE(128, 64, 1, 1, false, 16, 2);
            if (bk == 16 && nst == 3) DCASE(128, 64, 1, 1, false, 16, 3);
            if (bk == 32 && nst == 4) DCASE(128, 64, 1, 1, false, 32, 4);
            if (bk == 16 && nst == 4) DCASE(128, 64, 1, 1, false, 16, 4);
        } else if (tk == 128128) {
            if (bk == 32 && nst == 2) DCASE(128, 128, 1, 1, false, 32, 2);
            if (bk == 32 && nst == 3) DCASE(128, 128, 1, 1, false, 32, 3);
            if (bk == 16 && nst == 2) DCASE(128, 128, 1, 1, false, 16, 2);
            if (bk == 16 && nst == 3) DCASE(128, 128, 1, 1, false, 16, 3);
            if (bk == 16 && nst == 4) DCASE(128, 128, 1, 1, false, 16, 4);
        }
    } else if (key == 310) {
        if (tk == 64064) {
            if (bk == 32 && nst == 2) DCASE(64, 64, 3, 1, false, 32, 2);
            if (bk == 32 && nst == 3) DCASE(64, 64, 3, 1, false, 32, 3);
            if (bk == 16 && nst == 2) DCASE(64, 64, 3, 1, false, 16, 2);
            if (bk == 16 && nst == 3) DCASE(64, 64, 3, 1, false, 16, 3);
            if (bk == 16 && nst == 4) DCASE(64, 64, 3, 1, false, 16, 4);
            if (bk == 32 && nst == 4) DCASE(64, 64, 3, 1, false, 32, 4);
        } else if (tk == 32064) {
            if (bk == 32) DCASE(32, 64, 3, 1, false, 32, 2);
        } else if (tk == 128064) {
            if (bk == 16 && nst == 2) DCASE(128, 64, 3, 1, false, 16, 2);
            if (bk == 16 && nst == 3) DCASE(128, 64, 3, 1, false, 16, 3);
        } else if (tk == 128128) {
            if (bk == 16 && nst == 2) DCASE(128, 128, 3, 1, false, 16, 2);
            if (bk == 16 && nst == 3) DCASE(128, 128, 3, 1, false, 16, 3);
        }
    } else if (key == 320 && tk == 64064) {
        if (bk == 32 && nst == 2) DCASE(64, 64, 3, 2, false, 32, 2);
        if (bk >= 16 && nst == 3) DCASE(64, 64, 3, 2, false, 16, 3);
        if (bk == 16 && nst == 2) DCASE(64, 64, 3, 2, false, 16, 2);
    } else if (key == 220 && tk == 64064) {
        if (bk == 32) DCASE(64, 64, 2, 2, false, 32, 2);
        DCASE(64, 64, 2, 2, false, 16, 2);
    } else if (key == 311 && tk == 64064) {
        if (bk == 32 && nst == 2) DCASE(64, 64, 3, 1, true, 32, 2);
        if (bk >= 16 && nst == 3) DCASE(64, 64, 3, 1, true, 16, 3);
        if (bk == 16 && nst == 2) DCASE(64, 64, 3, 1, true, 16, 2);
    }
    return hipErrorInvalidValue;
}

}
```

latent-diffusion-speech_amd/csrc/k4p.h:

```cpp
#pragma once
#include <hip/hip_runtime.h>

namespace lds {

__host__ __device__ inline long long k4p_index(int C, int T, int b, int c, int t) {
    return ((((long long)b * (C >> 3) + (c >> 3)) * 2 + (c & 1)) * (T + 2) + (t + 1)) * 4 + ((c & 7) >> 1);
}
__host__ __device__ inline long long k4p_floats(int B, int C, int T) { return (long long)B * C * (T + 2); }

typedef float k4p_f32x2 __attribute__((ext_vector_type(2)));
static __device__ __forceinline__ void k4p_store_wt(float* p, k4p_f32x2 v) {
    __hip_atomic_store(reinterpret_cast<unsigned long long*>(p), __builtin_bit_cast(unsigned long long, v), __ATOMIC_RELAXED, __HIP_MEMORY_SCOPE_AGENT);
}

static __device__ __forceinline__ int ragged_len(const int* lens, int b, int lvl, int T) {
    if (!lens) return T;
    int n = lens[b];
    for (int i = 0; i < lvl; ++i) n = (n - 1) / 2 + 1;
    return n < T ? n : T;
}

}
```

latent-diffusion-speech_amd/csrc/kernels.h:

```cpp
#pragma once
#include <hip/hip_runtime.h>
#include <stddef.h>
#include <stdint.h>

#include <atomic>
#include <string>

namespace lds {

enum { ACT_NONE = 0, ACT_LRELU = 2 };
enum { EPI_NONE = 0, EPI_GEGLU = 1, EPI_TANH = 2, EPI_GELU = 3, EPI_SWISH = 4, EPI_GLU = 5 };

struct ConvArgs {
    const float* x1; const float* x2;
    int C1, C2;
    int Tsrc;
    int Tin;
    long long xb1, xb2;
    const float* w;
    int Mp, Co, Ci, KT, stride, dil, pad, ups;
    int act_in; float slope;
    const float* bias;
    const float* bias_bc;
    const float* res;
    int epi;
    int accum;
    float out_div;
    float* out;
    int Cout;
    int To;
    int phases, tpad, Tout;
    int B;
    const int* vlen; const int* vlen_in;
};

hipError_t launch_conv_gemm(const ConvArgs& a, int tile, hipStream_t s);
const char* conv_gemm_last_config();

bool conv_small_applies(const ConvArgs& a);
hipError_t launch_conv_small(const ConvArgs& a, hipStream_t s);
bool conv_mono_applies(const ConvArgs& a);
hipError_t launch_conv_mono(const ConvArgs& a, hipStream_t s);
const char* conv_small_last_config();

struct ConvDownArgs {
    const float* x; const float* w; const float* bias; float* out;
    int Ci, Co, K, stride, pad, L, To, B;
    float slope;
    int tile;
    const int* vlen_in; const int* vlen;
};
hipError_t launch_conv_down(const ConvDownArgs& a, hipStream_t s);
const char* conv_down_last_config();
hipError_t launch_vae_head(const float* y, const float* noise, float* out, float* z, int B, int C, int T, int only_mean, hipStream_t s,
                           const int* tlen = nullptr);

struct VocPairArgs {
    const float* x; float* out;
    const float* w1; const float* b1; int Mp1;
    const float* w2; const float* b2; int Mp2;
    int C, KT, dil, B, T;
    int accum; float out_div; float slope;
    const int* vlen;
};
bool voc_pair_applies(int C, int KT, int dil);
hipError_t launch_voc_pair(const VocPairArgs& a, hipStream_t s);
const char* voc_pair_last_config();

size_t packed_conv_elems(int Co, int Ci, int K, int* Mp_out);

struct DmaConvArgs {
    const float* x1; const float* x2;
    int C1, C2, Tsrc;
    const float* w;
    const float* bias;
    int Mp, Co, Ci, KT, stride, pad, ups;
    const float* res;
    int epi;
    float* out;
    int out_plain;
    int plain_from; float* out2;
    int vt_D;
    float2* lnpart_out;
    float2* gnpart_out;
    const float2* ln_part; int ln_np; float ln_eps; const float* ln_c1; const float* ln_c2;
    const float2* gnf_part; int gnf_groups; float gnf_eps; const float* gnf_cg; const float* gnf_c2;
    int Cout, To, B;
    int voc;
    int dil;
    int xpad, opad;
    float act_slope;
    float* out_act;
    const float* acc_in;
    float out_div;
    int ph_log2, ph_tpad, ph_Tout, ph_Cout;
    int out_f32;
    float acc_scale;
    int tile_batch;
    const int* lens; int lvl_in, lvl_out;
    const int* vlen;
    int ksplit;
    float* kpart; unsigned* kcount;
    long long kpart_cap; int kcount_cap;
};
hipError_t launch_conv_dma(const DmaConvArgs& a, int cfg, hipStream_t s);
hipError_t launch_conv_dma_pair(const DmaConvArgs& a3, const DmaConvArgs& a1, hipStream_t s);
bool conv_dma_pair_applies(const DmaConvArgs& a3, const DmaConvArgs& a1);
const char* conv_dma_last_config();

hipError_t launch_conv_bf3(const DmaConvArgs& a, int cfg, int nprod, int fmt, hipStream_t s);
hipError_t launch_conv_bf3_pair(const DmaConvArgs& a3, const DmaConvArgs& a1, int fmt, hipStream_t s);
bool conv_bf3_pair_applies(const DmaConvArgs& a3, const DmaConvArgs& a1);
const char* conv_bf3_last_config();
void conv_bf3_set_debug_rule(int r);
hipError_t launch_to_k8b3(const float* in, void* out, int B, int C, int T, int Ctot, int c_off, hipStream_t s, int fmt = 0, const int* lens = nullptr);
hipError_t launch_from_k8b3(const void* in, float* out, int B, int C, int T, hipStream_t s, int fmt = 0);
hipError_t launch_gn_stream_bf3(const void* x1, const void* x2, int C1, int C2, int T, int groups, float eps, const float* gamma,
                                const float* beta, const float* scale_shift, int ss_stride, int ss_off, int silu, const float2* gp1,
                                const float2* gp2, void* y, int B, hipStream_t s, int fmt = 0, const int* lens = nullptr, int lvl = 0);
hipError_t launch_gn_partials_bf3(const void* x, int C, int T, float2* gp, int B, hipStream_t s, int fmt = 0);
hipError_t launch_resample_k8b3(const void* in, void* out, int B, int C, int Tin, int Tout, hipStream_t s, int fmt = 0, const int* lens = nullptr, int lvl_in = 0, int lvl_out = 0);

hipError_t launch_to_k4p(const float* in, float* out, int B, int C, int T, int Ctot, int c_off, hipStream_t s, const int* lens = nullptr);
hipError_t launch_from_k4p(const float* in, float* out, int B, int C, int T, hipStream_t s);
hipError_t launch_from_k4p_pad(const float* in, float* out, int B, int C, int T, int pad, hipStream_t s);
hipError_t launch_plain_to_vt(const float* in, float* out, int B, int C, int T, int D, hipStream_t s);
hipError_t launch_gn_stream(const float* x1, const float* x2, int C1, int C2, int T, int groups, float eps,
                            const float* gamma, const float* beta, const float* scale_shift, int ss_stride, int ss_off,
                            int silu, const float2* gp1, const float2* gp2, float* y, int B, hipStream_t s, const int* lens = nullptr, int lvl = 0);
hipError_t launch_gn_partials(const float* x, int C, int T, float2* gp, int B, hipStream_t s);
hipError_t launch_to_k4p_act(const float* in, float* raw, float* act, float slope, int B, int C, int T, int pad, hipStream_t s, const int* vlen = nullptr);
hipError_t launch_k4p_zero_pads(float* x, int B, int C, int T, int pad, hipStream_t s);
hipError_t launch_resample_k4p(const float* in, float* out, int B, int C, int Tin, int Tout, hipStream_t s, const int* lens = nullptr, int lvl_in = 0, int lvl_out = 0);
hipError_t launch_attention_k4p(const float* qk, const float* vt, float* out, int B, int C, int T, int heads, hipStream_t s, int tile_batch = 0,
                                const int* lens = nullptr, int lvl = 0);
hipError_t launch_attention_k4p_f16math(const float* qk, const float* vt, float* out, int B, int C, int T, int heads, hipStream_t s, int tile_batch = 0);
hipError_t launch_attention_k4p_out_bf3(const float* qk, const float* vt, void* out, int B, int C, int T, int heads, hipStream_t s, int fmt = 0, int tile_batch = 0,
                                        const int* lens = nullptr, int lvl = 0);

hipError_t launch_logmel(const float* audio, const int* slen, long long L, int Fmax, const double* basis, const float* filtT, int n_mels,
                         float* logspec, float* pmax, float* out, int out_k4p, int B, hipStream_t s);
hipError_t launch_whisper_pos(float* x, const float* posk, int n_ctx, float2* lnpart, const int* lens, int B, int C, int T, hipStream_t s);
hipError_t launch_whisper_ln_post(const float* x, const float2* lnpart, const float* gamma, const float* beta, float eps, float* out, const int* lens,
                                  int B, int C, int T, hipStream_t s, int lvl = 1);

hipError_t launch_hubert_conv0(const float* audio, const int* slen, long long L, int pad, const float* w0, const float* gamma, const float* beta, float eps,
                               const int* nlen, int N0, int C, float2* part, float2* stat, float* out, int B, hipStream_t s);
hipError_t launch_hubert_posconv(const float* x, const float* wp, const float* bias, float* out, const int* nlen, int B, int C, int T, int K, int groups,
                                 hipStream_t s);
hipError_t launch_hubert_ln(const float* x, const float* gamma, const float* beta, float eps, float* out, const int* nlen, int B, int C, int T, hipStream_t s);
hipError_t launch_hubert_store_frames(const float* x, float* out, const int* nlen, int B, int C, int T, hipStream_t s);

hipError_t launch_w2v_conv0(const float* audio, const int* slen, long long L, const float* w0, const float* bias, const float* gamma, const float* beta,
                            float eps, const int* nlen, int N0, int C, float* out, int B, hipStream_t s);
hipError_t launch_w2v_ln_act(const float* x, const float* gamma, const float* beta, float eps, float* out, float2* part, const int* nlen, int B, int C, int T,
                             hipStream_t s);
hipError_t launch_w2v_lnpart(const float* x, float2* part, const int* nlen, int B, int C, int T, hipStream_t s);

constexpr int kW2vbertRelStride = 80;
hipError_t launch_w2vbert_fbank(const float* audio, const int* slen, long long L, int Nmax, int Rmax, const double* basis, const float* filtT, int n_mels,
                                int stride, float mel_floor, float* logspec, double2* stat, float* out, int B, hipStream_t s);
hipError_t launch_w2vbert_feats_k4p(const float* feats, float* out, float2* part, const int* vlen, int B, int C, int T, hipStream_t s);
hipError_t launch_w2vbert_relpos(const float* qk, const float* E, float* relp, const int* qlen, int B, int C, int T, int heads, int NR, hipStream_t s);
hipError_t launch_attention_k4p_rel(const float* qk, const float* vt, const float* relp, float* out, int B, int C, int T, int heads, const int* qlens,
                                    const int* klens, int left, int right, hipStream_t s);
hipError_t launch_w2vbert_dwconv(const float* x, const float* wp, const float* gamma, const float* beta, float eps, float* out, const int* vlen,
                                 const int* nlen, int B, int C, int T, int K, hipStream_t s);

enum { IN_PLAIN = 0, IN_SILU = 1, IN_SINUSOID = 2 };
hipError_t launch_small_linear(const float* W, const float* bias, const float* in, int in_stride, int in_mode,
                               const float* freqs, float* out, int out_stride, int out_silu, int M, int K, int B, hipStream_t s);

enum {
    EW_X0 = 1,
    EW_AXPBY = 2,
    EW_DPM2 = 3,
    EW_UNIPC_PRED = 4,
    EW_UNIPC_CORR = 5,
    EW_UNIPC_CORR1 = 6,
    EW_DDPM = 7,
    EW_DDIM = 8,
    EW_PLMS_PRED = 9,
    EW_LIN4 = 10,
    EW_COPY = 11
};
hipError_t launch_ew(int op, float* out, const float* a, const float* b, const float* c, const float* d,
                     float c0, float c1, float c2, float c3, float c4, long long n, hipStream_t s);
// ... 39 lines not shown
```

latent-diffusion-speech_amd/csrc/model.hip:

```cpp
#include "../../include/lds.h"
#include "../../include/lds_test.h"
#include "k4p.h"
#include "k8b3.h"
#include "kernels.h"

#include <math.h>
#include <stdarg.h>
#include <stdio.h>
#include <stdlib.h>
#include <string.h>

#include <algorithm>
#include <atomic>
#include <map>
#include <mutex>
#include <string>
#include <vector>

using namespace lds;

static thread_local char g_err[512] = "";
static int fail(int code, const char* fmt, ...) {
    va_list ap;
    va_start(ap, fmt);
// ... 3058 lines not shown
        HIP_TRY(launch_attention_k4p_rel(w.qk, w.v, w.relp, w.att, B, C, T, c.n_head, w.rows, w.valid, c.left_max, c.right_max, st));
        DOpt oo;
        oo.res = x; oo.lnpart_out = w.lnp;
        LDS_TRY(run_dconv(bw.out, w.att, C, nullptr, 0, T, oo, xn, B, st));
        std::swap(x, xn);
        {
            LensScope lv(w.valid);
            DOpt og;
            og.epi = EPI_GLU;
            og.ln_part = w.lnp; og.ln_np = C / 32; og.ln_eps = c.eps; og.ln_c1 = bw.pw1_c1; og.ln_c2 = bw.pw1_c2;
            LDS_TRY(run_dconv(bw.pw1, x, C, nullptr, 0, T, og, glu, B, st));
        }
        HIP_TRY(launch_w2vbert_dwconv(glu, bw.dw, bw.dw_g, bw.dw_b, c.eps, dwo, w.valid, w.rows, B, C, T, c.dw_kernel, st));
        DOpt op;
        op.res = x; op.lnpart_out = w.lnp;
        LDS_TRY(run_dconv(bw.pw2, dwo, C, nullptr, 0, T, op, xn, B, st));
        std::swap(x, xn);
        LDS_TRY(ffn(bw.f2a, bw.f2_c1, bw.f2_c2, bw.f2b, x, xn, nullptr));
        std::swap(x, xn);
        HIP_TRY(launch_hubert_ln(x, bw.fin_g, bw.fin_b, c.eps, xn, w.rows, B, C, T, st));
        std::swap(x, xn);
        if (&bw != &h->blocks.back()) { HIP_TRY(launch_w2v_lnpart(x, w.lnp, w.rows, B, C, T, st)); }
    }
    HIP_TRY(launch_hubert_store_frames(x, enc, w.rows, B, C, T, st));
    return LDS_OK;
}

static int w2vbert_audio_check(const lds_w2vbert* h, const float* audio, const int32_t* lengths, const void* out, const void* ws, int B, int64_t L, int& N,
                               int& R, int32_t* nfr) {
    if (!h || !audio || !out || !ws) return fail(LDS_EINVAL, "null argument");
    LDS_TRY(w2vbert_shape_check(h, B, L, N, R));
    if (lengths) LDS_TRY(clip_lens_check("length", lengths, B, kW2vbertMinSamples, L));
    for (int b = 0; b < B; ++b) nfr[b] = lengths ? w2vbert_frames(lengths[b]) : N;
    return LDS_OK;
}
extern "C" int lds_w2vbert_fbank(lds_w2vbert* h, const float* audio, const int32_t* lengths, float* out, void* ws, size_t ws_bytes, int B, int64_t L, void* stream) {
    int N, R;
    int32_t nfr[64];
    LDS_TRY(w2vbert_audio_check(h, audio, lengths, out, ws, B, L, N, R, nfr));
    return w2vbert_run(h, audio, L, lengths, nullptr, nfr, N, R, out, nullptr, ws, ws_bytes, B, stream);
}
extern "C" int lds_w2vbert_encode(lds_w2vbert* h, const float* audio, const int32_t* lengths, float* out, void* ws, size_t ws_bytes, int B, int64_t L, void* stream) {
    int N, R;
    int32_t nfr[64];
    LDS_TRY(w2vbert_audio_check(h, audio, lengths, out, ws, B, L, N, R, nfr));
    return w2vbert_run(h, audio, L, lengths, nullptr, nfr, N, R, nullptr, out, ws, ws_bytes, B, stream);
}
extern "C" int lds_w2vbert_encode_features(lds_w2vbert* h, const float* feats, const int32_t* n_frames, float* out, void* ws, size_t ws_bytes, int B, int R,
                                           void* stream) {
    if (!h || !feats || !out || !ws) return fail(LDS_EINVAL, "null argument");
    LDS_TRY(range_check("w2vbert", "B", B, 1, 64));
    if (R < 1 || R > h->cfg.n_ctx) return fail(LDS_EINVAL, "w2vbert: %d rows outside 1 .. n_ctx %d", R, h->cfg.n_ctx);
    const int st = h->cfg.stride;
    int32_t nfr[64];
    for (int b = 0; b < B; ++b) {
        nfr[b] = n_frames ? n_frames[b] : R * st;
        if (nfr[b] < 2 || nfr[b] < st || (nfr[b] + st - 1) / st > R) return fail(LDS_EINVAL, "n_frames[%d] = %d outside %d .. %d", b, nfr[b], st > 2 ? st : 2, R * st);
    }
    return w2vbert_run(h, nullptr, 0, nullptr, feats, nfr, R * st, R, nullptr, out, ws, ws_bytes, B, stream);
}

extern "C" int lds_test_conv(const lds_conv_test* a, float* out, int B, void* stream) {
    if (!a || !out) return fail(LDS_EINVAL, "bad argument");
    hipStream_t st = (hipStream_t)stream;
    Owner own;
    ConvW W;
    const int Ci = a->C1 + a->C2;
    if (!pack_conv(own, a->w, a->bias, a->Co, Ci, a->K, W)) return fail(LDS_ENOMEM, "test conv: upload failed");
    ConvOpt o;
    o.pad = a->pad; o.dil = a->dil;
    o.act_in = a->act_in; o.slope = a->slope; o.res = a->res; o.epi = a->epilogue; o.tile = a->tile;
    Src s{a->x1, a->C1, a->x2, a->C2, a->Tsrc};
    const int r = run_conv(W, s, o, out, B, st);
    HIP_TRY(hipStreamSynchronize(st));
    return r;
}

struct TmpDev {
    std::vector<void*> p;
    ~TmpDev() { for (void* q : p) (void)hipFree(q); }
    float* f(size_t n) { void* d = nullptr; if (hipMalloc(&d, n * sizeof(float) + 65536) != hipSuccess) return nullptr; p.push_back(d); return (float*)d; }
};

static int dconv_test_impl(const lds_dconv_test* a, float* out, float* lnpart, int B, int iters, float* ms_out, void* stream, int bf3 = 0, int nprod = 0, int fmt = 0,
                           const int* alt_cfgs = nullptr, int n_alt = 0) {
    hipStream_t st = (hipStream_t)stream;
    Owner own;
    TmpDev tmp;
    ConvW W;
    const int Ci = a->C1 + a->C2, T = a->T;
    bool ok = (a->epilogue == EPI_GEGLU) ? pack_geglu(own, a->w, a->bias, a->Co, Ci, W) : pack_conv(own, a->w, a->bias, a->Co, Ci, a->K, W);
    if (ok && bf3) ok = make_split_twin(own, W, fmt);
    if (!ok) return fail(LDS_ENOMEM, "test dconv: upload failed");
    auto act_floats = [&](int C, int Tl) { return bf3 ? (size_t)B * split_floats(fmt, C, Tl) : (size_t)B * C * (Tl + 2); };
    auto to_act = [&](const float* src, float* dst, int C, int Tl) { return bf3 ? launch_to_k8b3(src, dst, B, C, Tl, C, 0, st, fmt) : launch_to_k4p(src, dst, B, C, Tl, C, 0, st); };
    auto from_act = [&](const float* src, float* dst, int C, int Tl) { return bf3 ? launch_from_k8b3(src, dst, B, C, Tl, st, fmt) : launch_from_k4p(src, dst, B, C, Tl, st); };
    float* k1 = tmp.f(act_floats(a->C1, T));
    float* k2 = a->C2 ? tmp.f(act_floats(a->C2, T)) : nullptr;
    if (!k1 || (a->C2 && !k2)) return fail(LDS_ENOMEM, "test dconv: alloc failed");
    HIP_TRY(to_act(a->x1, k1, a->C1, T));
    if (a->C2) HIP_TRY(to_act(a->x2, k2, a->C2, T));
    const int Cout = (a->epilogue == EPI_GEGLU) ? a->Co / 2 : a->Co;
    const int Tin = a->ups ? 2 * T : T;
    const int To = (Tin + 2 * a->pad - (a->K - 1) - 1) / a->stride + 1;
    const int Ck = a->v_split ? (Cout / 3) * 2 : Cout;
    DOpt o;
    o.stride = a->stride; o.pad = a->pad; o.ups = a->ups; o.epi = a->epilogue; o.cfg = a->cfg; o.out_plain = a->plain_out;
    const bool qk_f32 = bf3 && a->v_split;
    o.out_f32 = qk_f32 ? 1 : 0;
    float* kres = nullptr;
    if (a->res) {
        kres = tmp.f(act_floats(Ck, To));
        if (!kres) return fail(LDS_ENOMEM, "alloc");
        HIP_TRY(to_act(a->res, kres, Ck, To));
        o.res = kres;
    }
    float* kout = a->plain_out ? out : tmp.f(qk_f32 ? (size_t)B * Ck * (To + 2) : act_floats(Ck, To));
    float* vout = nullptr;
    if (!kout) return fail(LDS_ENOMEM, "alloc");
    const int To4 = (To + 3) & ~3;
    if (a->v_split) {
        vout = tmp.f((size_t)B * (Cout - Ck) * To4);
        if (!vout) return fail(LDS_ENOMEM, "alloc");
        HIP_TRY(hipMemsetAsync(vout, 0xff, sizeof(float) * B * (Cout - Ck) * To4, st));
        o.plain_from = Ck; o.out2 = vout;
        if (a->v_split > 1) o.vt_D = a->v_split;
    }
    o.lnpart_out = (float2*)lnpart;
    auto run = [&]() { return bf3 ? run_dconv_bf3(W, k1, a->C1, k2, a->C2, T, o, kout, B, st, nprod, fmt) : run_dconv(W, k1, a->C1, k2, a->C2, T, o, kout, B, st); };
    int r = run();
    if (r == LDS_OK && iters > 0 && ms_out) {
        hipEvent_t e0, e1;
        HIP_TRY(hipEventCreate(&e0));
        HIP_TRY(hipEventCreate(&e1));
        HIP_TRY(hipEventRecord(e0, st));
        for (int i = 0; i < iters && r == LDS_OK; ++i) {
            if (n_alt > 0) o.cfg = alt_cfgs[i % n_alt];
            r = run();
        }
        HIP_TRY(hipEventRecord(e1, st));
        HIP_TRY(hipEventSynchronize(e1));
        float ms = 0.f;
        HIP_TRY(hipEventElapsedTime(&ms, e0, e1));
        *ms_out = ms / iters;
        (void)hipEventDestroy(e0);
        (void)hipEventDestroy(e1);
    }
    auto from_out = [&](const float* src, float* dst, int C, int Tl) { return qk_f32 ? launch_from_k4p(src, dst, B, C, Tl, st) : from_act(src, dst, C, Tl); };
    if (r == LDS_OK && !a->plain_out) {
        if (a->v_split > 1) {
            HIP_TRY(from_out(kout, out, Ck, To));
            HIP_TRY(hipMemcpyAsync(out + (size_t)B * Ck * To, vout, sizeof(float) * B * (Cout - Ck) * To4, hipMemcpyDeviceToDevice, st));
        } else if (a->v_split) {
            float* tmpo = tmp.f((size_t)B * Ck * To);
            if (!tmpo) return fail(LDS_ENOMEM, "alloc");
            HIP_TRY(from_out(kout, tmpo, Ck, To));
            for (int b = 0; b < B; ++b) {
                HIP_TRY(hipMemcpyAsync(out + (size_t)b * Cout * To, tmpo + (size_t)b * Ck * To, sizeof(float) * Ck * To, hipMemcpyDeviceToDevice, st));
                HIP_TRY(hipMemcpyAsync(out + (size_t)b * Cout * To + (size_t)Ck * To, vout + (size_t)b * (Cout - Ck) * To,
                                       sizeof(float) * (Cout - Ck) * To, hipMemcpyDeviceToDevice, st));
            }
        } else {
            HIP_TRY(from_out(kout, out, Ck, To));
        }
    }
    HIP_TRY(hipStreamSynchronize(st));
    return r;
}
extern "C" int lds_test_dconv(const lds_dconv_test* a, float* out, float* lnpart, int B, void* stream) {
    if (!a || !out) return fail(LDS_EINVAL, "bad argument");
    return dconv_test_impl(a, out, lnpart, B, 0, nullptr, stream);
}
extern "C" int lds_bench_dconv(const lds_dconv_test* a, float* out, int B, int iters, float* ms_out, char* cfg_out, size_t cfg_cap, void* stream) {
    if (!a || !out || !ms_out || iters <= 0) return fail(LDS_EINVAL, "bad argument");
    int r = dconv_test_impl(a, out, nullptr, B, iters, ms_out, stream);
    if (cfg_out && cfg_cap) snprintf(cfg_out, cfg_cap, "%s", conv_dma_last_config());
    return r;
}
extern "C" int lds_bench_dconv_alt(const lds_dconv_test* a, float* out, int B, int iters, const int* cfgs, int n, float* ms_out, void* stream) {
    if (!a || !out || !cfgs || n < 1 || !ms_out) return fail(LDS_EINVAL, "bad argument");
    return dconv_test_impl(a, out, nullptr, B, iters, ms_out, stream, 0, 0, 0, cfgs, n);
}
extern "C" int lds_test_dconv_split(const lds_dconv_test* a, float* out, float* lnpart, int B, int nprod, int fmt, void* stream) {
    if (!a || !out || (fmt != FMT_BF16X3 && fmt != FMT_F16X2)) return fail(LDS_EINVAL, "bad argument");
    return dconv_test_impl(a, out, lnpart, B, 0, nullptr, stream, 1, nprod, fmt);
}
extern "C" int lds_test_dconv_bf3(const lds_dconv_test* a, float* out, float* lnpart, int B, int nprod, void* stream) {
    return lds_test_dconv_split(a, out, lnpart, B, nprod, FMT_BF16X3, stream);
}
extern "C" int lds_bench_dconv_split(const lds_dconv_test* a, float* out, int B, int iters, int nprod, int fmt, float* ms_out, char* cfg_out, size_t cfg_cap,
                                     void* stream) {
    if (!a || !out || !ms_out || iters <= 0 || (fmt != FMT_BF16X3 && fmt != FMT_F16X2)) return fail(LDS_EINVAL, "bad argument");
    int r = dconv_test_impl(a, out, nullptr, B, iters, ms_out, stream, 1, nprod, fmt);
    if (cfg_out && cfg_cap) snprintf(cfg_out, cfg_cap, "%s", conv_bf3_last_config());
    return r;
}
extern "C" int lds_bench_dconv_bf3(const lds_dconv_test* a, float* out, int B, int iters, int nprod, float* ms_out, char* cfg_out, size_t cfg_cap, void* stream) {
    if (!a || !out || !ms_out || iters <= 0) return fail(LDS_EINVAL, "bad argument");
    int r = dconv_test_impl(a, out, nullptr, B, iters, ms_out, stream, 1, nprod, FMT_BF16X3);
    if (cfg_out && cfg_cap) snprintf(cfg_out, cfg_cap, "%s", conv_bf3_last_config());
    return r;
}

extern "C" int lds_test_gn_apply(const float* x1, const float* x2, int C1, int C2, int T, int groups, float eps, const float* gamma,
                                 const float* beta, const float* scale_shift, int silu, float* out, int B, void* stream) {
    hipStream_t st = (hipStream_t)stream;
    Owner own;
    TmpDev tmp;
    const int C = C1 + C2, nT = (T + 31) / 32;
    float* g = up_vec(own, gamma, C);
    float* be = up_vec(own, beta, C);
    float* k1 = tmp.f((size_t)B * C1 * (T + 2));
    float* k2 = C2 ? tmp.f((size_t)B * C2 * (T + 2)) : nullptr;
    float* ky = tmp.f((size_t)B * C * (T + 2));
    float* p1 = tmp.f((size_t)B * (C1 / 16) * nT * 2);
    float* p2 = C2 ? tmp.f((size_t)B * (C2 / 16) * nT * 2) : nullptr;
    if (!g || !be || !k1 || (C2 && (!k2 || !p2)) || !ky || !p1) return fail(LDS_ENOMEM, "alloc");
    HIP_TRY(launch_to_k4p(x1, k1, B, C1, T, C1, 0, st));
    HIP_TRY(launch_gn_partials(k1, C1, T, (float2*)p1, B, st));
    if (C2) {
        HIP_TRY(launch_to_k4p(x2, k2, B, C2, T, C2, 0, st));
        HIP_TRY(launch_gn_partials(k2, C2, T, (float2*)p2, B, st));
    }
    HIP_TRY(launch_gn_stream(k1, k2, C1, C2, T, groups, eps, g, be, scale_shift, 2 * C, 0, silu, (const float2*)p1, (const float2*)p2, ky, B, st));
    HIP_TRY(launch_from_k4p(ky, out, B, C, T, st));
    HIP_TRY(hipStreamSynchronize(st));
    return LDS_OK;
}

extern "C" int lds_bench_gn_stream(int C1, int C2, int T, int B, int iters, float* ms_out, void* stream) {
    hipStream_t st = (hipStream_t)stream;
// ... 111 lines not shown
    float* gp = tmp.f((size_t)B * (Cm / 16) * nT * 2);
    float* kpart = tmp.f((size_t)kClusterPartFloats);
    unsigned* kcount = (unsigned*)tmp.f(kClusterCounters);
    if (!kx || !km || !ko || !gp || !kpart || !kcount) return fail(LDS_ENOMEM, "alloc");
    HIP_TRY(hipMemsetAsync(kcount, 0, sizeof(unsigned) * kClusterCounters, st));
    HIP_TRY(to_act_any(f32 ? 0 : fmt + 1, x, kx, B, C, T, C, 0, st));
    DOpt o1;
    o1.gnpart_out = (float2*)gp;
    LDS_TRY(dconv_any(f32 ? 0 : fmt + 1, W1, kx, C, nullptr, 0, T, o1, km, B, st));
    if (f32) HIP_TRY(launch_from_k4p(km, mid, B, Cm, T, st));
    else HIP_TRY(launch_from_k8b3(km, mid, B, Cm, T, st, fmt));
    for (int rep = 0; rep < reps; ++rep) {
        {
            TileBatchScope tbs(tile_batch, kpart, kcount);
            DOpt o2;
            o2.cfg = cfg;
            o2.gnf_part = (const float2*)gp; o2.gnf_groups = groups; o2.gnf_eps = eps; o2.gnf_cg = cg; o2.gnf_c2 = c2;
            LDS_TRY(dconv_any(f32 ? 0 : fmt + 1, W2, km, Cm, nullptr, 0, T, o2, ko, B, st));
        }
        float* dst = out + (size_t)rep * B * Co * T;
        if (f32) HIP_TRY(launch_from_k4p(ko, dst, B, Co, T, st));
        else HIP_TRY(launch_from_k8b3(ko, dst, B, Co, T, st, fmt));
    }
    HIP_TRY(hipStreamSynchronize(st));
    return LDS_OK;
}

extern "C" int lds_test_cluster_join(const float* xa, const float* xb, const float* w, const float* bias, int Ci, int Co, int K, int T, int B, int fmt, int reps,
                                     float* out, float* ref_a, float* ref_b, char* cfg_out, size_t cfg_cap, void* stream) {
    hipStream_t st = (hipStream_t)stream;
    if (!xa || !xb || !w || !out || !ref_a || !ref_b || reps < 1 || (K != 1 && K != 3) || (fmt != -1 && fmt != FMT_BF16X3 && fmt != FMT_F16X2)) return fail(LDS_EINVAL, "bad argument");
    const bool f32 = fmt < 0;
    const int mode = f32 ? 0 : fmt + 1;
    Owner own;
    TmpDev tmp;
    ConvW W;
    if (!pack_conv(own, w, bias, Co, Ci, K, W) || (!f32 && !make_split_twin(own, W, fmt))) return fail(LDS_ENOMEM, "upload failed");
    auto act = [&](int Cc) { return f32 ? (size_t)Cc * (T + 2) : split_floats(fmt, Cc, T); };
    float* ka = tmp.f((size_t)B * act(Ci));
    float* kb = tmp.f((size_t)B * act(Ci));
    float* ko = tmp.f((size_t)B * act(Co));
    float* kpart = tmp.f((size_t)kClusterPartFloats);
    unsigned* kcount = (unsigned*)tmp.f(kClusterCounters);
    if (!ka || !kb || !ko || !kpart || !kcount) return fail(LDS_ENOMEM, "alloc");
    HIP_TRY(hipMemsetAsync(kcount, 0, sizeof(unsigned) * kClusterCounters, st));
    HIP_TRY(to_act_any(mode, xa, ka, B, Ci, T, Ci, 0, st));
    HIP_TRY(to_act_any(mode, xb, kb, B, Ci, T, Ci, 0, st));
    DOpt o;
    o.pad = K / 2;
    auto back = [&](float* dst) { return f32 ? launch_from_k4p(ko, dst, B, Co, T, st) : launch_from_k8b3(ko, dst, B, Co, T, st, fmt); };
    {
        TileBatchScope tbs(B, nullptr, nullptr);
        LDS_TRY(dconv_any(mode, W, ka, Ci, nullptr, 0, T, o, ko, B, st));
        HIP_TRY(back(ref_a));
        LDS_TRY(dconv_any(mode, W, kb, Ci, nullptr, 0, T, o, ko, B, st));
        HIP_TRY(back(ref_b));
    }
    for (int rep = 0; rep < reps; ++rep) {
        {
            TileBatchScope tbs(B, kpart, kcount);
            LDS_TRY(dconv_any(mode, W, (rep & 1) ? kb : ka, Ci, nullptr, 0, T, o, ko, B, st));
        }
        if (rep == 0 && cfg_out && cfg_cap) snprintf(cfg_out, cfg_cap, "%s", f32 ? conv_dma_last_config() : conv_bf3_last_config());
        HIP_TRY(back(out + (size_t)rep * B * Co * T));
    }
    HIP_TRY(hipStreamSynchronize(st));
    return LDS_OK;
}

extern "C" int lds_test_ln_chain_k4p(const float* x, const float* w1, const float* w2, const float* gamma, const float* beta, float eps,
                                     float* mid, float* out, int B, int C, int Co, int T, void* stream) {
    hipStream_t st = (hipStream_t)stream;
    Owner own;
    TmpDev tmp;
    ConvW W1, W2;
    float *c1 = nullptr, *c2 = nullptr;
    if (!pack_conv(own, w1, nullptr, C, C, 1, W1) || !pack_ln_fold(own, w2, nullptr, gamma, beta, Co, C, {}, W2, c1, c2)) return fail(LDS_ENOMEM, "upload failed");
    float* kx = tmp.f((size_t)B * C * (T + 2));
    float* km = tmp.f((size_t)B * C * (T + 2));
    float* ko = tmp.f((size_t)B * Co * (T + 2));
    float* part = tmp.f((size_t)B * (C / 32) * T * 2);
    if (!kx || !km || !ko || !part) return fail(LDS_ENOMEM, "alloc");
    HIP_TRY(launch_to_k4p(x, kx, B, C, T, C, 0, st));
    DOpt o1;
    o1.lnpart_out = (float2*)part;
    LDS_TRY(run_dconv(W1, kx, C, nullptr, 0, T, o1, km, B, st));
    DOpt o2;
    o2.ln_part = (const float2*)part; o2.ln_np = C / 32; o2.ln_eps = eps; o2.ln_c1 = c1; o2.ln_c2 = c2;
    LDS_TRY(run_dconv(W2, km, C, nullptr, 0, T, o2, ko, B, st));
    HIP_TRY(launch_from_k4p(km, mid, B, C, T, st));
    HIP_TRY(launch_from_k4p(ko, out, B, Co, T, st));
    HIP_TRY(hipStreamSynchronize(st));
    return LDS_OK;
}

extern "C" int lds_test_voc_step(const float* x, const float* w1, const float* b1, const float* w2, const float* b2, int C, int T, int K, int dil, int mode,
                                 const float* acc, float div, float* out, float* out_act, int B, void* stream) {
    hipStream_t st = (hipStream_t)stream;
    if (!x || !w1 || !w2 || !out || C % 64 || (K != 3 && K != 7 && K != 11)) return fail(LDS_EINVAL, "bad argument");
    Owner own;
    TmpDev tmp;
    ConvW W1, W2;
    if (!pack_conv(own, w1, b1, C, C, K, W1) || !pack_conv(own, w2, b2, C, C, K, W2)) return fail(LDS_ENOMEM, "upload failed");
    const int P = kVocPad;
    const size_t n = (size_t)B * C * (T + 2 * P) + 4096;
    float *raw = tmp.f(n), *act = tmp.f(n), *mid = tmp.f(n), *o_raw = tmp.f(n), *o_act = tmp.f(n), *kacc = tmp.f(n);
    if (!raw || !act || !mid || !o_raw || !o_act || !kacc) return fail(LDS_ENOMEM, "alloc");
    HIP_TRY(hipMemsetAsync(mid, 0xff, n * sizeof(float), st));
    HIP_TRY(hipMemsetAsync(act, 0xff, n * sizeof(float), st));
    HIP_TRY(launch_to_k4p_act(x, raw, act, 0.1f, B, C, T, P, st));
    HIP_TRY(launch_k4p_zero_pads(act, B, C, T, P, st));
    HIP_TRY(launch_k4p_zero_pads(mid, B, C, T, P, st));
    DOpt o1;
    o1.voc = 1; o1.xpad = P; o1.opad = P; o1.dil = dil; o1.pad = (K * dil - dil) / 2; o1.act_slope = 0.1f;
    LDS_TRY(run_dconv(W1, act, C, nullptr, 0, T, o1, mid, B, st));
    DOpt o2;
    o2.voc = 1; o2.xpad = P; o2.opad = P; o2.pad = (K - 1) / 2; o2.res = raw;
    if (mode == 0) {
        o2.out_plain = 1;
        LDS_TRY(run_dconv(W2, mid, C, nullptr, 0, T, o2, out, B, st));
    } else if (mode == 1) {
        o2.out_act = o_act; o2.act_slope = 0.1f;
        LDS_TRY(run_dconv(W2, mid, C, nullptr, 0, T, o2, o_raw, B, st));
        HIP_TRY(launch_from_k4p_pad(o_raw, out, B, C, T, P, st));
        if (out_act) HIP_TRY(launch_from_k4p_pad(o_act, out_act, B, C, T, P, st));
    } else {
        if (!acc) return fail(LDS_EINVAL, "mode 2 needs acc");
        HIP_TRY(launch_to_k4p_act(acc, kacc, nullptr, 0.f, B, C, T, P, st));
        o2.acc_in = kacc; o2.out_div = div; o2.out_plain = 1;
        LDS_TRY(run_dconv(W2, mid, C, nullptr, 0, T, o2, out, B, st));
    }
    HIP_TRY(hipStreamSynchronize(st));
    return LDS_OK;
}

static int attention_test_impl(const float* qkv, float* out, int B, int C, int T, int heads, int f16math, void* stream, int tile_batch = 0);
extern "C" int lds_test_attention_k4p(const float* qkv, float* out, int B, int C, int T, int heads, void* stream) {
    return attention_test_impl(qkv, out, B, C, T, heads, 0, stream);
}
extern "C" int lds_test_attention_f16math(const float* qkv, float* out, int B, int C, int T, int heads, void* stream) {
    return attention_test_impl(qkv, out, B, C, T, heads, 1, stream);
}
extern "C" int lds_test_attention_latency(const float* qkv, float* out, int B, int C, int T, int heads, int f16math, void* stream) {
    return attention_test_impl(qkv, out, B, C, T, heads, f16math, stream, B);
}
static int attention_test_impl(const float* qkv, float* out, int B, int C, int T, int heads, int f16math, void* stream, int tile_batch) {
    hipStream_t st = (hipStream_t)stream;
    TmpDev tmp;
    float* qkp = tmp.f((size_t)B * 2 * C * T);
    float* vpl = tmp.f((size_t)B * C * T);
    float* vt = tmp.f((size_t)B * C * (T + 3));
    float* kqk = tmp.f((size_t)B * 2 * C * (T + 2));
    float* ko = tmp.f((size_t)B * C * (T + 2));
    if (!qkp || !vpl || !vt || !kqk || !ko) return fail(LDS_ENOMEM, "alloc");
    for (int b = 0; b < B; ++b) {
        HIP_TRY(hipMemcpyAsync(qkp + (size_t)b * 2 * C * T, qkv + (size_t)b * 3 * C * T, sizeof(float) * 2 * C * T, hipMemcpyDeviceToDevice, st));
        HIP_TRY(hipMemcpyAsync(vpl + (size_t)b * C * T, qkv + (size_t)b * 3 * C * T + (size_t)2 * C * T, sizeof(float) * C * T, hipMemcpyDeviceToDevice, st));
    }
    HIP_TRY(launch_to_k4p(qkp, kqk, B, 2 * C, T, 2 * C, 0, st));
    HIP_TRY(launch_plain_to_vt(vpl, vt, B, C, T, C / heads, st));
    if (f16math) HIP_TRY(launch_attention_k4p_f16math(kqk, vt, ko, B, C, T, heads, st, tile_batch));
    else HIP_TRY(launch_attention_k4p(kqk, vt, ko, B, C, T, heads, st, tile_batch));
    HIP_TRY(launch_from_k4p(ko, out, B, C, T, st));
    HIP_TRY(hipStreamSynchronize(st));
    return LDS_OK;
}

extern "C" int lds_test_conv_transpose(const float* x, const float* w, const float* bias, float* out, int B, int Ci, int Co, int T, int K,
                                       int stride, int pad, float in_slope, void* stream) {
    hipStream_t st = (hipStream_t)stream;
    if (K % stride || pad != (K - stride + 1) / 2) return fail(LDS_EINVAL, "unsupported transposed-conv geometry");
    Owner own;
    ConvW W;
    if (!pack_convT(own, w, bias, Ci, Co, K, stride, W)) return fail(LDS_ENOMEM, "upload failed");
    Src s{x, Ci, nullptr, 0, T};
    ConvOpt o;
    o.pad = W.K - 1; o.phases = stride; o.tpad = pad; o.To = T + 1; o.Tout = (T - 1) * stride - 2 * pad + K; o.Cout = Co;
    if (in_slope != 1.0f) { o.act_in = ACT_LRELU; o.slope = in_slope; }
    int r = run_conv(W, s, o, out, B, st);
    HIP_TRY(hipStreamSynchronize(st));
    return r;
}

extern "C" int lds_test_split_roundtrip(const float* x, float* out, int B, int C, int T, int fmt, void* stream) {
    hipStream_t st = (hipStream_t)stream;
    if (!x || !out || (C & 7) || (fmt != FMT_BF16X3 && fmt != FMT_F16X2)) return fail(LDS_EINVAL, "bad argument");
    TmpDev tmp;
    float* k = tmp.f((size_t)B * split_floats(fmt, C, T));
    if (!k) return fail(LDS_ENOMEM, "alloc");
    HIP_TRY(launch_to_k8b3(x, k, B, C, T, C, 0, st, fmt));
    HIP_TRY(launch_from_k8b3(k, out, B, C, T, st, fmt));
    HIP_TRY(hipStreamSynchronize(st));
    return LDS_OK;
}
extern "C" int lds_test_k8b3_roundtrip(const float* x, float* out, int B, int C, int T, void* stream) { return lds_test_split_roundtrip(x, out, B, C, T, FMT_BF16X3, stream); }

extern "C" int lds_test_gn_apply_bf3(const float* x1, const float* x2, int C1, int C2, int T, int groups, float eps, const float* gamma,
                                     const float* beta, const float* scale_shift, int silu, float* out, int B, void* stream) {
    return lds_test_gn_apply_split(x1, x2, C1, C2, T, groups, eps, gamma, beta, scale_shift, silu, out, B, FMT_BF16X3, stream);
}
extern "C" int lds_test_gn_apply_split(const float* x1, const float* x2, int C1, int C2, int T, int groups, float eps, const float* gamma,
                                       const float* beta, const float* scale_shift, int silu, float* out, int B, int fmt, void* stream) {
    hipStream_t st = (hipStream_t)stream;
    if (fmt != FMT_BF16X3 && fmt != FMT_F16X2) return fail(LDS_EINVAL, "bad argument");
    Owner own;
    TmpDev tmp;
    const int C = C1 + C2, nT = (T + 31) / 32;
    float* g = up_vec(own, gamma, C);
    float* be = up_vec(own, beta, C);
    float* k1 = tmp.f((size_t)B * split_floats(fmt, C1, T));
    float* k2 = C2 ? tmp.f((size_t)B * split_floats(fmt, C2, T)) : nullptr;
    float* ky = tmp.f((size_t)B * split_floats(fmt, C, T));
    float* p1 = tmp.f((size_t)B * (C1 / 16) * nT * 2);
    float* p2 = C2 ? tmp.f((size_t)B * (C2 / 16) * nT * 2) : nullptr;
    if (!g || !be || !k1 || (C2 && (!k2 || !p2)) || !ky || !p1) return fail(LDS_ENOMEM, "alloc");
    HIP_TRY(launch_to_k8b3(x1, k1, B, C1, T, C1, 0, st, fmt));
    HIP_TRY(launch_gn_partials_bf3(k1, C1, T, (float2*)p1, B, st, fmt));
    if (C2) {
        HIP_TRY(launch_to_k8b3(x2, k2, B, C2, T, C2, 0, st, fmt));
        HIP_TRY(launch_gn_partials_bf3(k2, C2, T, (float2*)p2, B, st, fmt));
    }
    HIP_TRY(launch_gn_stream_bf3(k1, k2, C1, C2, T, groups, eps, g, be, scale_shift, 2 * C, 0, silu, (const float2*)p1, (const float2*)p2, ky, B, st, fmt));
    HIP_TRY(launch_from_k8b3(ky, out, B, C, T, st, fmt));
    HIP_TRY(hipStreamSynchronize(st));
    return LDS_OK;
}

extern "C" int lds_debug_set_touch_weights(int on) {
    g_touch_w.store(on ? 1 : 0);
    return LDS_OK;
}
extern "C" int lds_debug_set_voc_pair(int on) {
    g_voc_pair.store(on ? 1 : 0);
    return LDS_OK;
}
extern "C" int lds_test_voc_pair(const float* x, const float* w1, const float* b1, const float* w2, const float* b2, int C, int T, int K, int dil,
                                 const float* acc, float div, const int32_t* lengths, float* out, int B, void* stream) {
    hipStream_t st = (hipStream_t)stream;
    if (!x || !w1 || !w2 || !out || !voc_pair_applies(C, K, dil) || B < 1 || B > 64) return fail(LDS_EINVAL, "bad argument");
    Owner own;
    TmpDev tmp;
    ConvW W1, W2;
    if (!pack_conv(own, w1, b1, C, C, K, W1) || !pack_conv(own, w2, b2, C, C, K, W2)) return fail(LDS_ENOMEM, "upload failed");
    int* vl = nullptr;
    if (lengths) {
// ... 39 lines not shown
    return LDS_OK;
}
extern "C" int lds_test_conv_down(const float* x, const float* w, const float* b, int Ci, int Co, int K, int stride, int T, int B, float slope,
                                  int tile, float* out, char* cfg_out, size_t cfg_cap, void* stream) {
    return conv_down_test_impl(x, w, b, Ci, Co, K, stride, T, B, slope, nullptr, nullptr, tile, out, cfg_out, cfg_cap, stream);
}
extern "C" int lds_test_conv_down_ragged(const float* x, const float* w, const float* b, int Ci, int Co, int K, int stride, int T, int B, float slope,
                                         const int32_t* lengths_in, const int32_t* lengths_out, int tile, float* out, char* cfg_out, size_t cfg_cap,
                                         void* stream) {
    if (!lengths_in || !lengths_out || B < 1 || B > 64) return fail(LDS_EINVAL, "bad argument: lengths_in / lengths_out null or B %d outside 1 .. 64", B);
    return conv_down_test_impl(x, w, b, Ci, Co, K, stride, T, B, slope, lengths_in, lengths_out, tile, out, cfg_out, cfg_cap, stream);
}
extern "C" int lds_debug_set_gn_fold(int on) {
    g_gn_fold.store(on ? 1 : 0);
    return LDS_OK;
}
extern "C" int lds_debug_set_split_rule(int rule) {
    conv_bf3_set_debug_rule(rule);
    return LDS_OK;
}

static int test_upload_lens(TmpDev& tmp, const int32_t* host, int B, int*& dev, hipStream_t st) {
    dev = nullptr;
    if (!host) return LDS_OK;
    if (B < 1 || B > 64) return fail(LDS_EINVAL, "per-utterance lengths: 1 .. 64 batch elements (got %d)", B);
    dev = (int*)tmp.f(64);
    if (!dev) return fail(LDS_ENOMEM, "alloc");
    float t4[64];
    memcpy(t4, host, sizeof(int) * B);
    HIP_TRY(launch_set_list((float*)dev, t4, B, st));
    return LDS_OK;
}
struct TestActs {
    int fmt, B; hipStream_t st;
    size_t floats(int C, int T) const { return fmt < 0 ? (size_t)B * C * (T + 2) : (size_t)B * split_floats(fmt, C, T); }
    hipError_t to(const float* src, float* dst, int C, int T) const { return fmt < 0 ? launch_to_k4p(src, dst, B, C, T, C, 0, st) : launch_to_k8b3(src, dst, B, C, T, C, 0, st, fmt); }
    hipError_t from(const float* src, float* dst, int C, int T) const { return fmt < 0 ? launch_from_k4p(src, dst, B, C, T, st) : launch_from_k8b3(src, dst, B, C, T, st, fmt); }
};

extern "C" int lds_test_dconv_pair(const float* h, const float* x1, const float* x2, const float* w3, const float* b3, const float* w1, const float* b1, int B,
                                   int Cm, int C1, int C2, int Co, int T, const int32_t* lengths, int lvl, int tile_batch, int fmt, float* out, float* gnpart,
                                   char* cfg_out, size_t cfg_cap, void* stream) {
    hipStream_t st = (hipStream_t)stream;
    if (!h || !x1 || (C2 > 0) != (x2 != nullptr) || !w3 || !b3 || !w1 || !b1 || !out || !gnpart || B < 1 || T < 1 || Cm < 8 || C1 < 8 || C2 < 0 || (Cm & 7) || (C1 & 7) ||
        (C2 & 7) || Co < 32 || Co % 32 || lvl < 0 || tile_batch < 0 || (fmt != -1 && fmt != FMT_BF16X3 && fmt != FMT_F16X2))
        return fail(LDS_EINVAL, "bad argument");
    const bool f32 = fmt < 0;
    Owner own;
    TmpDev tmp;
    ConvW W3, W1;
    if (!pack_conv(own, w3, nullptr, Co, Cm, 3, W3) || !pack_conv(own, w1, nullptr, Co, C1 + C2, 1, W1)) return fail(LDS_ENOMEM, "upload failed");
    if (!f32 && !make_split_twin_pair(own, W3, W1, fmt)) return fail(LDS_ENOMEM, "upload failed");
    std::vector<float> bp(W3.Mp, 0.f);
    for (int co = 0; co < Co; ++co) bp[co] = b3[co] + b1[co];
    float* bias_pair = own.upload(bp);
    if (!bias_pair) return fail(LDS_ENOMEM, "upload failed");
    int* lens = nullptr;
    LDS_TRY(test_upload_lens(tmp, lengths, B, lens, st));
    const TestActs act{fmt, B, st};
    const int nT = (T + 31) / 32;
    float* kh = tmp.f(act.floats(Cm, T));
    float* k1 = tmp.f(act.floats(C1, T));
    float* k2 = C2 ? tmp.f(act.floats(C2, T)) : nullptr;
    float* ko = tmp.f(act.floats(Co, T));
    float* kpart = tile_batch ? tmp.f((size_t)kClusterPartFloats) : nullptr;
    unsigned* kcount = tile_batch ? (unsigned*)tmp.f(kClusterCounters) : nullptr;
    if (!kh || !k1 || (C2 && !k2) || !ko || (tile_batch && (!kpart || !kcount))) return fail(LDS_ENOMEM, "alloc");
    if (kcount) HIP_TRY(hipMemsetAsync(kcount, 0, sizeof(unsigned) * kClusterCounters, st));
    HIP_TRY(hipMemsetAsync(ko, 0xff, sizeof(float) * act.floats(Co, T), st));
    HIP_TRY(hipMemsetAsync(gnpart, 0xff, sizeof(float) * (size_t)B * (Co / 16) * nT * 2, st));
    HIP_TRY(act.to(h, kh, Cm, T));
    HIP_TRY(act.to(x1, k1, C1, T));
    if (C2) HIP_TRY(act.to(x2, k2, C2, T));
    int rc;
    {
        LensScope ls(lens);
        TileBatchScope tbs(tile_batch, kpart, kcount);
        rc = f32 ? run_dconv_pair(W3, kh, W1, k1, C1, k2, C2, T, bias_pair, (float2*)gnpart, ko, B, st, lvl)
                 : run_dconv_pair_bf3(W3, kh, W1, k1, C1, k2, C2, T, bias_pair, (float2*)gnpart, ko, B, st, fmt, lvl);
    }
    if (rc == 1) rc = fail(LDS_EINVAL, "dconv pair: no fused variant for Cm %d C1 %d C2 %d Co %d T %d (fmt %d, tile_batch %d)", Cm, C1, C2, Co, T, fmt, tile_batch);
    if (rc == LDS_OK) {
        if (cfg_out && cfg_cap) snprintf(cfg_out, cfg_cap, "%s", f32 ? conv_dma_last_config() : conv_bf3_last_config());
        HIP_TRY(act.from(ko, out, Co, T));
    }
    HIP_TRY(hipStreamSynchronize(st));
    return rc;
}

extern "C" int lds_test_dconv_ex(const lds_dconv_ex_test* a, float* out, float* gnpart, int B, char* cfg_out, size_t cfg_cap, void* stream) {
    hipStream_t st = (hipStream_t)stream;
    if (!a || !a->x1 || !a->w || !out || B < 1 || a->T < 1 || (a->C2 > 0) != (a->x2 != nullptr) || a->C1 < 8 || (a->C1 & 7) || a->C2 < 0 || (a->C2 & 7) || a->Co < 32 ||
        a->Co % 32 || a->K < 1 || a->stride < 1 || a->pad < 0 || (a->epilogue != EPI_NONE && a->epilogue != EPI_GELU) || a->lvl_in < 0 || a->lvl_out < 0 ||
        a->tile_batch < 0 || (a->fmt != -1 && a->fmt != FMT_BF16X3 && a->fmt != FMT_F16X2) || (a->ln_gamma != nullptr) != (a->ln_beta != nullptr))
        return fail(LDS_EINVAL, "bad argument");
    const bool f32 = a->fmt < 0, ln = a->ln_gamma != nullptr;
    const int mode = f32 ? 0 : a->fmt + 1;
    const int Ci = a->C1 + a->C2, T = a->T;
    const int To = (T + 2 * a->pad - (a->K - 1) - 1) / a->stride + 1;
    if (To < 1) return fail(LDS_EINVAL, "bad argument: no output frame");
    if (ln && (a->K != 1 || a->C2 || Ci % 32)) return fail(LDS_EINVAL, "the LayerNorm fold takes a 1x1 convolution over one source of a multiple of 32 channels");
    Owner own;
    TmpDev tmp;
    ConvW W, Wid;
    float *c1 = nullptr, *c2 = nullptr;
    bool ok = ln ? pack_ln_fold(own, a->w, a->bias, a->ln_gamma, a->ln_beta, a->Co, Ci, {}, W, c1, c2) : pack_conv(own, a->w, a->bias, a->Co, Ci, a->K, W);
    if (ok && ln) {
        std::vector<float> eye((size_t)Ci * Ci, 0.f);
        for (int c = 0; c < Ci; ++c) eye[(size_t)c * Ci + c] = 1.0f;
        ok = pack_conv(own, eye.data(), nullptr, Ci, Ci, 1, Wid);
    }
    if (ok && !f32) ok = make_split_twin(own, W, a->fmt) && (!ln || make_split_twin(own, Wid, a->fmt));
    if (!ok) return fail(LDS_ENOMEM, "test dconv: upload failed");
    int* lens = nullptr;
    LDS_TRY(test_upload_lens(tmp, a->lengths, B, lens, st));
    const TestActs act{a->fmt, B, st};
    float* k1 = tmp.f(act.floats(a->C1, T));
    float* k2 = a->C2 ? tmp.f(act.floats(a->C2, T)) : nullptr;
    float* kx = ln ? tmp.f(act.floats(Ci, T)) : nullptr;
    float* part = ln ? tmp.f((size_t)B * (Ci / 32) * T * 2) : nullptr;
    float* kres = a->res ? tmp.f(act.floats(a->Co, To)) : nullptr;
    float* ko = tmp.f(act.floats(a->Co, To));
    float* kpart = a->tile_batch ? tmp.f((size_t)kClusterPartFloats) : nullptr;
    unsigned* kcount = a->tile_batch ? (unsigned*)tmp.f(kClusterCounters) : nullptr;
    if (!k1 || (a->C2 && !k2) || (ln && (!kx || !part)) || (a->res && !kres) || !ko || (a->tile_batch && (!kpart || !kcount))) return fail(LDS_ENOMEM, "alloc");
    if (kcount) HIP_TRY(hipMemsetAsync(kcount, 0, sizeof(unsigned) * kClusterCounters, st));
    HIP_TRY(hipMemsetAsync(ko, 0xff, sizeof(float) * act.floats(a->Co, To), st));
    if (gnpart) HIP_TRY(hipMemsetAsync(gnpart, 0xff, sizeof(float) * (size_t)B * (a->Co / 16) * ((To + 31) / 32) * 2, st));
    HIP_TRY(act.to(a->x1, k1, a->C1, T));
    if (a->C2) HIP_TRY(act.to(a->x2, k2, a->C2, T));
    if (a->res) HIP_TRY(act.to(a->res, kres, a->Co, To));
    int rc = LDS_OK;
    {
        LensScope ls(lens);
        const float* xin = k1;
        if (ln) {
            DOpt oi;
            oi.lvl_in = oi.lvl_out = a->lvl_in;
            oi.lnpart_out = (float2*)part;
            rc = dconv_any(mode, Wid, k1, Ci, nullptr, 0, T, oi, kx, B, st);
            xin = kx;
        }
        if (rc == LDS_OK) {
            TileBatchScope tbs(a->tile_batch, kpart, kcount);
            DOpt o;
            o.stride = a->stride; o.pad = a->pad; o.epi = a->epilogue; o.res = kres;
            o.lvl_in = a->lvl_in; o.lvl_out = a->lvl_out;
            o.gnpart_out = (float2*)gnpart;
            if (ln) { o.ln_part = (const float2*)part; o.ln_np = Ci / 32; o.ln_eps = a->ln_eps; o.ln_c1 = c1; o.ln_c2 = c2; }
            rc = dconv_any(mode, W, xin, a->C1, k2, a->C2, T, o, ko, B, st);
        }
    }
    if (rc == LDS_OK) {
        if (cfg_out && cfg_cap) snprintf(cfg_out, cfg_cap, "%s", f32 ? conv_dma_last_config() : conv_bf3_last_config());
        HIP_TRY(act.from(ko, out, a->Co, To));
    }
    HIP_TRY(hipStreamSynchronize(st));
    return rc;
}

extern "C" int lds_test_voc_ups(const float* x, const float* w, const float* bias, int B, int Ci, int Co, int T, int K, int stride, const int32_t* lengths_in,
                                const int32_t* lengths_out, float* out, float* out_act, char* cfg_out, size_t cfg_cap, void* stream) {
    hipStream_t st = (hipStream_t)stream;
    int lg = 0;
    while ((1 << lg) < stride) ++lg;
    if (!x || !w || !out || !out_act || B < 1 || T < 1 || Ci < 16 || Ci % 16 || Co < 64 || Co % 64 || stride < 2 || stride > 16 || (1 << lg) != stride || K != 2 * stride ||
        (lengths_in != nullptr) != (lengths_out != nullptr))
        return fail(LDS_EINVAL, "bad argument");
    const int P = kVocPad, tpad = (K - stride + 1) / 2, Tn = (T - 1) * stride - 2 * tpad + K;
    for (int b = 0; b < B && lengths_in; ++b)
        if (lengths_in[b] < 0 || lengths_in[b] > T || lengths_out[b] < 0 || lengths_out[b] > Tn)
            return fail(LDS_EINVAL, "lengths_in[%d] = %d / lengths_out[%d] = %d outside 0 .. %d / 0 .. %d", b, lengths_in[b], b, lengths_out[b], T, Tn);
    Owner own;
    TmpDev tmp;
    ConvW W;
    if (!pack_convT(own, w, bias, Ci, Co, K, stride, W)) return fail(LDS_ENOMEM, "upload failed");
    int *vin = nullptr, *vout = nullptr;
    LDS_TRY(test_upload_lens(tmp, lengths_in, B, vin, st));
    LDS_TRY(test_upload_lens(tmp, lengths_out, B, vout, st));
    const size_t n_in = (size_t)B * Ci * (T + 2 * P), n_out = (size_t)B * Co * (Tn + 2 * P);
    float *scratch = tmp.f(n_in), *kin = tmp.f(n_in), *o_raw = tmp.f(n_out), *o_act = tmp.f(n_out);
    if (!scratch || !kin || !o_raw || !o_act) return fail(LDS_ENOMEM, "alloc");
    HIP_TRY(hipMemsetAsync(kin, 0xff, n_in * sizeof(float), st));
    HIP_TRY(hipMemsetAsync(o_raw, 0xff, n_out * sizeof(float), st));
    HIP_TRY(hipMemsetAsync(o_act, 0xff, n_out * sizeof(float), st));
    HIP_TRY(launch_to_k4p_act(x, scratch, kin, 0.1f, B, Ci, T, P, st, vin));
    HIP_TRY(launch_k4p_zero_pads(kin, B, Ci, T, P, st));
    DOpt o;
    o.voc = 1; o.xpad = P; o.opad = P; o.pad = 1; o.act_slope = 0.1f; o.out_act = o_act;
    o.ph_log2 = lg; o.ph_tpad = tpad; o.ph_Tout = Tn; o.vlen = vout;
    const int rc = run_dconv(W, kin, Ci, nullptr, 0, T, o, o_raw, B, st);
    if (rc == LDS_OK) {
        if (cfg_out && cfg_cap) snprintf(cfg_out, cfg_cap, "%s", conv_dma_last_config());
        HIP_TRY(launch_from_k4p_pad(o_raw, out, B, Co, Tn, P, st));
        HIP_TRY(launch_from_k4p_pad(o_act, out_act, B, Co, Tn, P, st));
    }
    HIP_TRY(hipStreamSynchronize(st));
    return rc;
}

extern "C" int lds_test_w2v_conv0(const float* audio, const int32_t* lengths, const float* w, const float* bias, const float* gamma, const float* beta,
                                  float eps, float* out, int B, int C, int64_t L, void* stream) {
    if (!audio || !w || !bias || !gamma || !beta || !out || B < 1 || B > 64 || L < 10 || L > ((int64_t)1 << 30)) return fail(LDS_EINVAL, "bad argument");
    hipStream_t st = (hipStream_t)stream;
    TmpDev tmp;
    const int N0 = (int)((L - 10) / 5 + 1);
    float* ko = tmp.f((size_t)B * C * (N0 + 2));
    int* dl = (int*)tmp.f(128);
    if (!ko || !dl) return fail(LDS_ENOMEM, "alloc");
    const int *slen = nullptr, *nlen = nullptr;
    if (lengths) {
        int32_t n0[64];
        for (int b = 0; b < B; ++b) {
            if (lengths[b] < 10 || lengths[b] > L) return fail(LDS_EINVAL, "length[%d] = %d outside 10 .. %lld", b, lengths[b], (long long)L);
            n0[b] = (lengths[b] - 10) / 5 + 1;
        }
        LDS_TRY(upload_clip_ints(lengths, B, dl, st));
        LDS_TRY(upload_clip_ints(n0, B, dl + 64, st));
        slen = dl; nlen = dl + 64;
    }
    HIP_TRY(launch_w2v_conv0(audio, slen, L, w, bias, gamma, beta, eps, nlen, N0, C, ko, B, st));
    HIP_TRY(launch_from_k4p(ko, out, B, C, N0, st));
    HIP_TRY(hipStreamSynchronize(st));
    return LDS_OK;
}
extern "C" int lds_test_w2v_ln_act(const float* x, const int32_t* n_frames, const float* gamma, const float* beta, float eps, float* out, float* part, int B,
                                   int C, int T, void* stream) {
    if (!x || !gamma || !beta || !out || B < 1 || B > 64 || T < 1 || C < 64 || C % 64) return fail(LDS_EINVAL, "bad argument");
    hipStream_t st = (hipStream_t)stream;
    TmpDev tmp;
    float* kx = tmp.f((size_t)B * C * (T + 2));
    float* ko = tmp.f((size_t)B * C * (T + 2));
    int* dl = (int*)tmp.f(64);
    if (!kx || !ko || !dl) return fail(LDS_ENOMEM, "alloc");
    const int* nlen = nullptr;
    if (n_frames) {
        for (int b = 0; b < B; ++b)
// ... 101 lines not shown
```

latent-diffusion-speech_amd/lds/native.py:

```python
import ctypes as C
import os

import numpy as np

_HERE = os.path.dirname(os.path.abspath(__file__))
LIB_PATH = os.path.join(_HERE, "liblds.so")
_lib = None

METHODS = {"dpm-solver": 1, "unipc": 2, "ddpm": 3, "ddim": 4, "pndm": 5}
TABLE_STRIDE = 16


class UNetCfg(C.Structure):
    _fields_ = [("out_dims", C.c_int), ("n_hidden", C.c_int), ("n_layers", C.c_int), ("n_heads", C.c_int),
                ("norm_groups", C.c_int), ("n_blocks", C.c_int), ("block_out_channels", C.c_int * 8)]


class VocoderCfg(C.Structure):
    _fields_ = [("inter_channels", C.c_int), ("upsample_initial_channel", C.c_int), ("n_ups", C.c_int),
                ("upsample_rates", C.c_int * 8), ("upsample_kernel_sizes", C.c_int * 8), ("resblock", C.c_int),
                ("n_kernels", C.c_int), ("resblock_kernel_sizes", C.c_int * 4), ("n_dil", C.c_int),
                ("resblock_dilation_sizes", (C.c_int * 4) * 4)]


# ... 81 lines not shown
lds_hubert_destroy               v:p
lds_hubert_workspace_bytes       i:piqip
lds_hubert_features              i:pppppziqip
lds_hubert_encode                i:ppppiipziqip
lds_w2v_create                   i:pipppp
lds_w2v_destroy                  v:p
lds_w2v_workspace_bytes          i:piqp
lds_w2v_features                 i:pppppziqp
lds_w2v_encode                   i:pppppziqp
lds_w2vbert_create               i:pipppp
lds_w2vbert_destroy              v:p
lds_w2vbert_workspace_bytes      i:piqp
lds_w2vbert_fbank                i:pppppziqp
lds_w2vbert_encode_features      i:pppppziip
lds_w2vbert_encode               i:pppppziqp
lds_lm_create                    i:pipppp
lds_lm_destroy                   v:p
lds_lm_workspace_bytes           i:piiip
lds_lm_encode                    i:pppppppziip
lds_lm_generate                  i:pppiiiiifffpppppzp
lds_lm_workspace_bytes_opts      i:piiiip
lds_lm_generate_opts             i:pppiiippppppzp
lds_kmeans_workspace_bytes       i:qiip
lds_kmeans_prepare               i:piipp
lds_kmeans_assign                i:pqppiipppzp
lds_kmeans_assign_ragged         i:piipqppiipppzp
lds_kmeans_update                i:ppqpppiippzp
lds_kmeans_seed                  i:pqiiqppppzp
lds_resample                     i:ppppiiiiqqp
lds_resample_ragged              i:ppppppiiiiqqp
lds_frame_rms                    i:ppqiiiqp
lds_volume_extract               i:ppqpqp
lds_volume_mask                  i:ppqifp
lds_resample_frames_ragged       i:ppppiiiip
lds_overlap_assemble             i:pqppipqpqp
lds_prof_enable                  i:i
lds_prof_summary                 i:pz
lds_unet_set_gemm_mode           i:pi
lds_unet_get_gemm_mode           i:p
lds_unet_set_latency_mode        i:pi
lds_unet_get_latency_mode        i:p
"""
_TEST = """
lds_test_conv                    i:ppip
lds_test_dconv                   i:pppip
lds_bench_dconv                  i:ppiippzp
lds_test_gn_apply                i:ppiiiifpppipip
lds_bench_gn_stream              i:iiiiipp
lds_test_gn_chain_k4p            i:pppppfiippiiiiip
lds_test_ln_chain_k4p            i:pppppfppiiiip
lds_test_attention_k4p           i:ppiiiip
lds_test_conv_transpose          i:ppppiiiiiiifp
lds_test_voc_step                i:pppppiiiiipfppip
lds_test_dconv_bf3               i:pppiip
lds_bench_dconv_bf3              i:ppiiippzp
lds_test_k8b3_roundtrip          i:ppiiip
lds_test_gn_apply_bf3            i:ppiiiifpppipip
lds_test_dconv_split             i:pppiiip
lds_bench_dconv_split            i:ppiiiippzp
lds_test_split_roundtrip         i:ppiiiip
lds_test_gn_apply_split          i:ppiiiifpppipiip
lds_debug_set_split_rule         i:i
lds_test_attention_f16math       i:ppiiiip
lds_test_attention_latency       i:ppiiiiip
lds_debug_set_gn_fold            i:i
lds_debug_set_voc_pair           i:i
lds_debug_set_touch_weights      i:i
lds_test_voc_pair                i:pppppiiiipfppip
lds_test_gn_fold_k4p             i:pppppfippppiiiiiiip
lds_bench_dconv_alt              i:ppiipipp
lds_debug_fill_u32               i:pzup
lds_debug_trace                  i:i
lds_debug_trace_count            i:
lds_debug_trace_get              i:ipzpp
lds_debug_unet_plan              i:piipz
lds_test_gn_fold_split           i:pppppfippppiiiiiiiiip
lds_test_cluster_join            i:ppppiiiiiiippppzp
lds_test_lm_sample               i:piiiifffppipp
lds_test_conv_down               i:pppiiiiiifippzp
lds_test_conv_down_ragged        i:pppiiiiiifppippzp
lds_test_lm_beam_step            i:piiiiiifiippppppppppppppppp
lds_test_dconv_pair              i:pppppppiiiiiipiiipppzp
lds_test_dconv_ex                i:pppipzp
lds_test_voc_ups                 i:pppiiiiiipppppzp
lds_test_w2v_conv0               i:ppppppfpiiqp
lds_test_w2v_ln_act              i:ppppfppiiip
lds_test_w2vbert_fbank           i:pppiqp
lds_test_w2vbert_attention       i:pppppiiiiiip
lds_test_w2vbert_dwconv          i:ppppfpppiiiip
lds_test_stft_dft                i:pppiiiippiqp
"""
SIGNATURES = dict(ln.split() for ln in (_PUBLIC + _TEST).splitlines() if ln)
EXPORTS = [ln.split()[0] for ln in _PUBLIC.splitlines() if ln]
TEST_EXPORTS = [ln.split()[0] for ln in _TEST.splitlines() if ln]


def lib():
    global _lib
    if _lib is None:
        if not os.path.exists(LIB_PATH):
            raise RuntimeError(f"{LIB_PATH} is missing: build it with `make -C latent-diffusion-speech_amd/csrc` "
                               "(there is no CPU fallback for the hot path)")
        L = C.CDLL(LIB_PATH)
        for n in EXPORTS + TEST_EXPORTS:
            ret, _, args = SIGNATURES[n].partition(":")
            fn = getattr(L, n)
            fn.restype, fn.argtypes = _RETURN[ret], [_KIND[k] for k in args]
        _lib = L
    return _lib


def check(rc):
    if rc != 0:
        raise RuntimeError(f"liblds error {rc}: {lib().lds_last_error().decode()}")


def _stream():
    import torch
    return C.c_void_p(torch.cuda.current_stream().cuda_stream)


def _dev(t, dtype=None):
    import torch
    if not t.is_cuda:
        raise RuntimeError("liblds needs tensors on a HIP device (no CPU fallback for the hot path)")
    if not t.is_contiguous():
        raise RuntimeError("liblds needs contiguous tensors")
    if dtype is not None and t.dtype != dtype:
        raise RuntimeError(f"expected {dtype}, got {t.dtype}")
    return C.c_void_p(t.data_ptr())


def _host_tensor_table(state):
    names, ptrs, numel, keep = [], [], [], []
    for k, v in state.items():
        a = v.detach().cpu().numpy() if hasattr(v, "detach") else np.asarray(v)
        a = np.ascontiguousarray(a, dtype=np.float32)
        keep.append(a)
        names.append(k.encode())
        ptrs.append(a.ctypes.data)
        numel.append(a.size)
    n = len(names)
    return (n, (C.c_char_p * n)(*names), (C.c_void_p * n)(*ptrs), (C.c_int64 * n)(*numel), keep)


class Workspace:

    def __init__(self):
        self.bufs = {}

    def get(self, nbytes, device):
        import torch
        key = (str(device), int(torch.cuda.current_stream(device).cuda_stream))
        buf = self.bufs.get(key)
        if buf is None or buf.numel() < nbytes:
            buf = torch.empty(int(nbytes), dtype=torch.uint8, device=device)
            self.bufs[key] = buf
        return buf


def _dev_or_null(t, dtype=None):
    return None if t is None else _dev(t, dtype)


def _host(a):
    return None if a is None else a.ctypes.data
# ... 875 lines not shown
```

Before: 23990 mel-frames/s.

## Vectorize k4p attention stores, magic-div tile order, late epilogue loads in DMA conv

```diff
diff --git a/latent-diffusion-speech_amd/csrc/attention_k4p.hip b/latent-diffusion-speech_amd/csrc/attention_k4p.hip
--- a/latent-diffusion-speech_amd/csrc/attention_k4p.hip
+++ b/latent-diffusion-speech_amd/csrc/attention_k4p.hip
@@ -71,6 +71,30 @@
     for (int i = 0; i < VPW; ++i)
         __builtin_amdgcn_raw_ptr_buffer_load_lds(rv, (__attribute__((address_space(3))) void*)(st + 64 * D + (wave + NW * i) * 256), 16, voff[i],
                                                  kt * (64 * D * 4), 0, 0);
+}
+
+template <int D>
+static __device__ __forceinline__ void att_store_k4p(const f32x16* o, float rl, float* ob, int C, int Tp, int hd, int h, int tq, int Tbuf, bool live) {
+    constexpr int DT = (D + 31) / 32;
+    const __amdgpu_buffer_rsrc_t ro = __builtin_amdgcn_make_buffer_rsrc(ob, 0, C * Tp * 4, 0x00020000);
+#pragma unroll
+    for (int i = 0; i < DT; ++i) {
+        f32x16 v;
+#pragma unroll
+        for (int r = 0; r < 16; ++r) v[r] = live ? o[i][r] * rl : 0.f;
+        k4p_f32x4 ent[4];
+        k4p_tile_entries(v, ent);
+        if (tq < Tbuf) {
+#pragma unroll
+            for (int g = 0; g < 4; ++g) {
+                if (i * 32 + 8 * g >= D) break;
+                const int off = k4p_entry_off((hd * D + i * 32) / 8 + g, h, Tp, tq + 1);
+                k4p_store16_wt(ro, off, ent[g]);
+                if (tq == 0) k4p_store16(ro, off - 16, k4p_f32x4{0.f, 0.f, 0.f, 0.f});
+                if (tq == Tbuf - 1) k4p_store16(ro, off + 16, k4p_f32x4{0.f, 0.f, 0.f, 0.f});
+            }
+        }
+    }
 }
 
 template <int D, int NW, int NST, int KS, bool F16>
@@ -290,24 +314,8 @@
                     if (tq == Tbuf - 1) *reinterpret_cast<k8_u32x2*>(e + 16) = k8_u32x2{0u, 0u};
                 }
             }
-    } else if (tq < Tbuf) {
-        const bool live = tq < T;
-        const float rl = 1.0f / l;
-        float* ob = out + (long long)b * C * Tp;
-#pragma unroll
-        for (int i = 0; i < DT; ++i)
-#pragma unroll
-            for (int g = 0; g < 4; ++g) {
-                if (i * 32 + 8 * g >= D) break;
-                const int q = (hd * D + i * 32) / 8 + g;
-#pragma unroll
-                for (int hh = 0; hh < 2; ++hh) {
-                    const long long off = ((long long)(q * 2 + hh) * Tp + tq + 1) * 4 + 2 * h;
-                    k4p_store_wt(ob + off, live ? f32x2{o[i][4 * g + hh] * rl, o[i][4 * g + 2 + hh] * rl} : f32x2{0.f, 0.f});
-                    if (tq == 0) *reinterpret_cast<f32x2*>(ob + off - 4) = f32x2{0.f, 0.f};
-                    if (tq == Tbuf - 1) *reinterpret_cast<f32x2*>(ob + off + 4) = f32x2{0.f, 0.f};
-                }
-            }
+    } else if (!out_bf3) {
+        att_store_k4p<D>(o, 1.0f / l, out + (long long)b * C * Tp, C, Tp, hd, h, tq, Tbuf, tq < T);
     }
 }
 
@@ -532,24 +540,7 @@
         const auto sw = __builtin_amdgcn_permlane32_swap(__float_as_uint(l_run), __float_as_uint(l_run), false, false);
         l = __uint_as_float(sw[0]) + __uint_as_float(sw[1]);
     }
-    if (tq < Tbuf) {
-        const bool live = tq < Tq;
-        const float rl = 1.0f / l;
-        float* ob = out + (long long)b * C * Tp;
-#pragma unroll
-        for (int i = 0; i < DT; ++i)
-#pragma unroll
-            for (int g = 0; g < 4; ++g) {
-                const int q = (hd * D + i * 32) / 8 + g;
-#pragma unroll
-                for (int hh = 0; hh < 2; ++hh) {
-                    const long long off = ((long long)(q * 2 + hh) * Tp + tq + 1) * 4 + 2 * h;
-                    k4p_store_wt(ob + off, live ? f32x2{o[i][4 * g + hh] * rl, o[i][4 * g + 2 + hh] * rl} : f32x2{0.f, 0.f});
-                    if (tq == 0) *reinterpret_cast<f32x2*>(ob + off - 4) = f32x2{0.f, 0.f};
-                    if (tq == Tbuf - 1) *reinterpret_cast<f32x2*>(ob + off + 4) = f32x2{0.f, 0.f};
-                }
-            }
-    }
+    att_store_k4p<D>(o, 1.0f / l, out + (long long)b * C * Tp, C, Tp, hd, h, tq, Tbuf, tq < Tq);
 }
 
 template <int NW, int NST, int KS>
diff --git a/latent-diffusion-speech_amd/csrc/conv_dma.hip b/latent-diffusion-speech_amd/csrc/conv_dma.hip
--- a/latent-diffusion-speech_amd/csrc/conv_dma.hip
+++ b/latent-diffusion-speech_amd/csrc/conv_dma.hip
@@ -1,6 +1,7 @@
 #include "gn_chan.h"
 #include "k4p.h"
 #include "kernels.h"
+#include "../../include/lds_test.h"
 
 #include <hip/hip_ext.h>
 
@@ -70,6 +71,11 @@
 
     const DmaConvArgs& p;
     float* smem;
+    struct Hot {
+        const float *x1, *x2, *w;
+        int C1, C2, Tsrc, Mp, Ci, xpad, pad, ksplit, To, lvl_out;
+        unsigned om0, om1, om2, os, gx, gy;
+    } hp;
     int lane, wave, c, h, wm, wn, ks, b, m0, t0;
     int ksp, kc0, ctile;
     int Lout;
@@ -87,61 +93,80 @@
     f32x4 aop[NB][TM], bop[NB][TN];
     float lmu[TN], lrs[TN];
     static constexpr bool EARLY = TM * TN == 1 || VOC;
+    static constexpr bool LATE = EARLY && !VOC && !GNF;
+    static constexpr int NLATE = LATE ? TM * TN * 8 + TM * 4 : 0;
+    static_assert(PER_TILE * (NST - 1) + NLATE <= 63 || !LATE, "vmcnt is a 6-bit field");
     f32x2 rsv[EARLY ? TM * TN * 8 : 1];
     float kbv[EARLY ? TM * 16 : 1];
 
     __device__ __forceinline__ DmaKernel(const DmaConvArgs& p_, float* s_) : p(p_), smem(s_) {}
 
+    typedef const __attribute__((address_space(4))) int* const_int_ptr;
+    __device__ __forceinline__ int len_at(int lvl, int T) const {
+        if (!p.lens) return T;
+        int n = ((const_int_ptr)(unsigned long long)p.lens)[b];
+        for (int i = 0; i < lvl; ++i) n = (n - 1) / 2 + 1;
+        return n < T ? n : T;
+    }
+    __device__ __forceinline__ void load_hot() {
+        hp.x1 = p.x1; hp.x2 = p.x2; hp.w = p.w;
+        hp.C1 = p.C1; hp.C2 = p.C2; hp.Tsrc = p.Tsrc; hp.Mp = p.Mp; hp.Ci = p.Ci; hp.xpad = p.xpad; hp.pad = p.pad; hp.ksplit = p.ksplit; hp.To = p.To;
+        hp.lvl_out = p.lvl_out; hp.om0 = p.ord_m[0]; hp.om1 = p.ord_m[1]; hp.om2 = p.ord_m[2]; hp.os = p.ord_s; hp.gx = gridDim.x; hp.gy = gridDim.y;
+        asm volatile("" : "+s"(hp.x1), "+s"(hp.x2), "+s"(hp.w), "+s"(hp.C1), "+s"(hp.C2), "+s"(hp.Tsrc), "+s"(hp.Mp), "+s"(hp.Ci),
+                          "+s"(hp.xpad), "+s"(hp.pad), "+s"(hp.ksplit), "+s"(hp.To), "+s"(hp.lvl_out), "+s"(hp.om0), "+s"(hp.om1), "+s"(hp.om2),
+                          "+s"(hp.os), "+s"(hp.gx), "+s"(hp.gy));
+    }
     __device__ __forceinline__ void setup_keep_acc() {
+        load_hot();
         const int tid = threadIdx.x;
         lane = tid & 63;
         wave = __builtin_amdgcn_readfirstlane(tid >> 6);
         c = lane & 31; h = lane >> 5;
         wm = SPLIT ? 0 : wave >> 1; ks = SPLIT ? wave >> 1 : 0; wn = wave & 1;
         kofs_a = ks * KQW * 2 * BM * 4; kofs_b = ks * KQW * 2 * XW * 4;
-        const int nMb = p.Mp / BM;
-        const int gx = gridDim.x, total = gx * gridDim.y;
+        const int nMb = (int)((unsigned)hp.Mp / BM), nN = (int)((unsigned)(hp.To + BN - 1) / BN);
+        const int gx = (int)hp.gx, total = gx * (int)hp.gy;
         const int id = blockIdx.y * gx + blockIdx.x;
         const int xcd = id & 7, slot = id >> 3, per = total >> 3, rem = total & 7;
-        const int L = xcd * per + (xcd < rem ? xcd : rem) + slot;
-        const int mb = L % nMb;
-        const int tb = L / nMb;
-        const int nN = gx / nMb;
-        const int nb = tb % nN;
-        const int by = tb / nN, S = p.ksplit > 1 ? p.ksplit : 1;
-        b = by / S; ksp = by - b * S;
-        kc0 = ksp * (p.Ci / BK / S);
+        const unsigned L = (unsigned)(xcd * per + (xcd < rem ? xcd : rem) + slot);
+        const unsigned tb = dma_magic_div(L, hp.om0, hp.os & 255);
+        const int mb = (int)(L - tb * nMb);
+        const unsigned by = dma_magic_div(tb, hp.om1, (hp.os >> 8) & 255);
+        const int nb = (int)(tb - by * nN);
+        const int S = hp.ksplit > 1 ? hp.ksplit : 1;
+        b = (int)dma_magic_div(by, hp.om2, (hp.os >> 16) & 255); ksp = (int)by - b * S;
+        kc0 = ksp * steps_per_share();
         ctile = (b * nN + nb) * nMb + mb;
         m0 = mb * BM; t0 = nb * BN;
-        Lout = ragged_len(p.lens, b, p.lvl_out, p.To);
+        Lout = len_at(hp.lvl_out, hp.To);
 #pragma unroll
         for (int i = 0; i < WPW; ++i) {
-            const int q = (wave + 4 * i) * 64 + lane;
-            const int tap = q / (KR * BM);
-            const int rem = q - tap * (KR * BM);
-            const int rr = rem / BM, m = rem - rr * BM;
-            woff[i] = ((tap * (p.Ci / 4) + rr) * p.Mp + m0 + m) * 16;
-        }
-        const int Tp = p.Tsrc + 2 * p.xpad;
-        const int e0 = UPS ? (((t0 - 1) >> 1) + p.xpad) : (t0 * STRIDE - p.pad + p.xpad);
+            const unsigned q = (unsigned)(wave + 4 * i) * 64u + (unsigned)lane;
+            const unsigned tap = q / (unsigned)(KR * BM);
+            const unsigned rem = q - tap * (unsigned)(KR * BM);
+            const unsigned rr = rem / (unsigned)BM, m = rem - rr * (unsigned)BM;
+            woff[i] = (int)(((tap * ((unsigned)hp.Ci / 4u) + rr) * (unsigned)hp.Mp + (unsigned)m0 + m) * 16u);
+        }
+        const int Tp = hp.Tsrc + 2 * hp.xpad;
+        const int e0 = UPS ? (((t0 - 1) >> 1) + hp.xpad) : (t0 * STRIDE - hp.pad + hp.xpad);
 #pragma unroll
         for (int i = 0; i < NXI; ++i) {
-            const int qq = i * 64 + lane;
-            const int rl = qq / XW, col = qq - rl * XW;
-            xact[i] = qq < RPW * XW;
+            const unsigned qq = (unsigned)(i * 64 + lane);
+            const int rl = (int)(qq / (unsigned)XW), col = (int)qq - rl * XW;
+            xact[i] = (int)qq < RPW * XW;
             xoff[i] = ((wave * RPW + rl) * Tp + e0 + col) * 16;
         }
-        rw = __builtin_amdgcn_make_buffer_rsrc(const_cast<float*>(p.w), 0, KT * p.Ci * p.Mp * 4, 0x00020000);
-        rx1 = __builtin_amdgcn_make_buffer_rsrc(const_cast<float*>(p.x1 + (long long)b * p.C1 * Tp), 0, p.C1 * Tp * 4, 0x00020000);
-        rx2 = __builtin_amdgcn_make_buffer_rsrc(const_cast<float*>(p.x2 ? p.x2 + (long long)b * p.C2 * Tp : p.x1), 0, p.C2 * Tp * 4, 0x00020000);
+        rw = __builtin_amdgcn_make_buffer_rsrc(const_cast<float*>(hp.w), 0, KT * hp.Ci * hp.Mp * 4, 0x00020000);
+        rx1 = __builtin_amdgcn_make_buffer_rsrc(const_cast<float*>(hp.x1 + (long long)b * hp.C1 * Tp), 0, hp.C1 * Tp * 4, 0x00020000);
+        rx2 = __builtin_amdgcn_make_buffer_rsrc(const_cast<float*>(hp.x2 ? hp.x2 + (long long)b * hp.C2 * Tp : hp.x1), 0, hp.C2 * Tp * 4, 0x00020000);
         arow = wm * TM * 32 + c;
 #pragma unroll
         for (int j = 0; j < TN; ++j) bcol[j] = wn * TN * 32 + j * 32 + c;
     }
+    __device__ __forceinline__ int steps_per_share() const { return (int)dma_magic_div((unsigned)hp.Ci / BK, hp.om2, (hp.os >> 16) & 255); }
     __device__ __forceinline__ bool dead_tile() const { return !VOC && p.lens && t0 >= Lout; }
-    __device__ __forceinline__ int voc_len() const { return p.vlen[b]; }
-    __device__ __forceinline__ void setup() {
-        setup_keep_acc();
+    __device__ __forceinline__ int voc_len() const { return ((const_int_ptr)(unsigned long long)p.vlen)[b]; }
+    __device__ __forceinline__ void zero_acc() {
 #pragma unroll
         for (int a = 0; a < NACC; ++a)
 #pragma unroll
@@ -153,13 +178,13 @@
     }
 
     __device__ __forceinline__ void issue_tile(int kc, float* st) {
-        const int ws = kc * (KR * 16) * p.Mp;
+        const int ws = kc * (KR * 16) * hp.Mp;
 #pragma unroll
         for (int i = 0; i < WPW; ++i)
             __builtin_amdgcn_raw_ptr_buffer_load_lds(rw, (__attribute__((address_space(3))) void*)(st + ((wave + 4 * i) * 64) * 4), 16, woff[i], ws, 0, 0);
         const int k0 = kc * BK;
-        const bool s2 = k0 >= p.C1;
-        const int xsoff = (s2 ? k0 - p.C1 : k0) * (p.Tsrc + 2 * p.xpad) * 4;
+        const bool s2 = k0 >= hp.C1;
+        const int xsoff = (s2 ? k0 - hp.C1 : k0) * (hp.Tsrc + 2 * hp.xpad) * 4;
         float* xs = st + KT * BK * BM + wave * RPW * XW * 4;
 #pragma unroll
         for (int i = 0; i < NXI; ++i)
@@ -202,15 +227,17 @@
             preload<g0 + 1, g1>(cur);
         }
     }
+    template <bool EPI>
     __device__ __forceinline__ void tile_sync(int kc, int nk, float* cur) {
         const int younger = (nk - 2 - kc < NST - 2) ? (nk - 2 - kc) : (NST - 2);
-        wait_younger<NST - 2>(younger);
+        if (EPI && NLATE > 0 && kc + 1 < NST) wait_younger<NST - 2, NLATE>(younger);
+        else wait_younger<NST - 2, 0>(younger);
         asm volatile("s_waitcnt lgkmcnt(0)" ::: "memory");
         __builtin_amdgcn_s_barrier();
         asm volatile("" ::: "memory");
         if (kc + NST < nk) issue_tile(kc0 + kc + NST, cur);
     }
-    template <int g>
+    template <int g, bool EPI>
     __device__ __forceinline__ void kstep(float* cur, const float* nxt, int kc, int nk) {
         if constexpr (g < G) {
             constexpr int gp = g + NB - 1;
@@ -218,13 +245,13 @@
                 load_ops<gp % NB>(cur, gp / KQW, gp % KQW);
             } else {
                 if (kc + 1 < nk) {
-                    if constexpr (gp == G) tile_sync(kc, nk, cur);
+                    if constexpr (gp == G) tile_sync<EPI>(kc, nk, cur);
                     load_ops<gp % NB>(nxt, (gp - G) / KQW, (gp - G) % KQW);
                 }
             }
             mfma_ops<g % NB>();
             __builtin_amdgcn_sched_barrier(0);
-            kstep<g + 1>(cur, nxt, kc, nk);
+            kstep<g + 1, EPI>(cur, nxt, kc, nk);
         }
     }
 
@@ -246,7 +273,7 @@
     }
     __device__ __forceinline__ void gnf_request() {
         const int G_ = p.gnf_groups, gsz = p.Ci / G_;
-        const int gTv = ragged_len(p.lens, b, p.lvl_in, p.Tsrc);
+        const int gTv = len_at(p.lvl_in, p.Tsrc);
         ginv = 1.0f / (float)gsz;
         gp0 = gn_part_load(p.gnf_part, b, p.Ci, p.Tsrc, gsz >> 4, wave, lane, 0, gTv);
         gp1 = gn_part_load(p.gnf_part, b, p.Ci, p.Tsrc, gsz >> 4, (wave + 4 < G_) ? wave + 4 : wave, lane, 0, gTv);
@@ -266,7 +293,7 @@
             float rs = 1.f, rm = 0.f;
             if (g < G_) {
                 float mu, var;
-                gnf_group_stats(p.gnf_part, b, p.Ci, p.Tsrc, gsz >> 4, g, lane, e ? gp1 : gp0, mu, var, ragged_len(p.lens, b, p.lvl_in, p.Tsrc));
+                gnf_group_stats(p.gnf_part, b, p.Ci, p.Tsrc, gsz >> 4, g, lane, e ? gp1 : gp0, mu, var, len_at(p.lvl_in, p.Tsrc));
                 rs = __builtin_amdgcn_rsqf(var + p.gnf_eps); rm = rs * mu;
             }
             if (lane == 0) { tail[g] = rs; tail[8 + g] = rm; }
@@ -289,14 +316,14 @@
         gsn = gnf_tail()[gnf_group(k + 2)];
     }
 
-    template <int Y>
+    template <int Y, int X = 0>
     __device__ __forceinline__ void wait_younger(int y) {
         if constexpr (Y == 0) {
-            asm volatile("s_waitcnt vmcnt(0)" ::: "memory");
+            asm volatile("s_waitcnt vmcnt(%0)" ::"n"(X > 63 ? 63 : X) : "memory");
         } else {
-            constexpr int N = (Y * PER_TILE > 63) ? 63 : Y * PER_TILE;
+            constexpr int N = (Y * PER_TILE + X > 63) ? 63 : Y * PER_TILE + X;
             if (y >= Y) asm volatile("s_waitcnt vmcnt(%0)" ::"n"(N) : "memory");
-            else wait_younger<Y - 1>(y);
+            else wait_younger<Y - 1, X>(y);
         }
     }
 
@@ -325,15 +352,57 @@
         }
     }
 
+    __device__ __forceinline__ void late_loads() {
+        static_assert(TM * TN == 1, "single-tile waves");
+        const int tile0 = m0 + wm * 32, n = t0 + wn * 32 + c;
+        const int Tpo = p.To + 2 * p.opad, Ck = k4p_ck();
+        const bool rt = p.res && tile0 < p.plain_from && tile0 < p.Cout;
+        const __amdgpu_buffer_rsrc_t rr = __builtin_amdgcn_make_buffer_rsrc(const_cast<float*>(rt ? p.res + (long long)b * Ck * Tpo : p.res), 0, rt ? Ck * Tpo * 4 : 0, 0x00020000);
+        const int vo = k4p_off(tile0, n) * 4;
+#pragma unroll
+        for (int e = 0; e < 8; ++e) rsv[e] = __builtin_bit_cast(f32x2, __builtin_amdgcn_raw_buffer_load_b64(rr, vo + e * Tpo * 16, 0, 0));
+        const bool hb = p.bias && !p.ln_part;
+        const __amdgpu_buffer_rsrc_t rb = __builtin_amdgcn_make_buffer_rsrc(const_cast<float*>(p.bias), 0, hb ? p.Mp * 4 : 0, 0x00020000);
+#pragma unroll
+        for (int g = 0; g < 4; ++g) {
+            const f32x4 v = __builtin_bit_cast(f32x4, __builtin_amdgcn_raw_buffer_load_b128(rb, (tile0 + 8 * g + 4 * h) * 4, 0, 0));
+#pragma unroll
+            for (int k = 0; k < 4; ++k) kbv[4 * g + k] = v[k];
+        }
+    }
+
+    template <bool EPI = true, bool ZERO = true>
     __device__ __forceinline__ void mainloop() {
         static_assert(G % NB == 0 && NB - 1 <= G, "ring slots must keep their phase across K-steps");
-        const int nk = p.Ci / BK / (p.ksplit > 1 ? p.ksplit : 1);
+        constexpr int XL = EPI ? NLATE : 0;
+        const int nk = steps_per_share();
         if constexpr (GNF) gnf_request();
-        if constexpr (EARLY) early_loads();
+        if constexpr (EARLY && !LATE) early_loads();
         for (int t = 0; t < NST && t < nk; ++t) issue_tile(kc0 + t, smem + t * STAGE);
+        if constexpr (XL > 0) {
+            asm volatile("" ::: "memory");
+            __builtin_amdgcn_sched_barrier(0);
+            late_loads();
+            asm volatile("" ::: "memory");
+            __builtin_amdgcn_sched_barrier(0);
+        }
+        if constexpr (ZERO) {
+#pragma unroll
+            for (int a = 0; a < NACC; ++a)
+#pragma unroll
+                for (int i = 0; i < TM; ++i)
+#pragma unroll
+                    for (int j = 0; j < TN; ++j)
+#pragma unroll
+                        for (int r = 0; r < 16; ++r) {
+                            float z;
+                            asm volatile("v_mov_b32 %0, 0" : "=v"(z));
+                            acc[a][i][j][r] = z;
+                        }
+        }
         if (p.ln_part) ln_columns();
         if constexpr (GNF) gnf_prepare();
-        wait_younger<NST - 1>((nk - 1 < NST - 1) ? nk - 1 : NST - 1);
+        wait_younger<NST - 1, XL>((nk - 1 < NST - 1) ? nk - 1 : NST - 1);
         __builtin_amdgcn_s_barrier();
         asm volatile("" ::: "memory");
         if constexpr (GNF) gnf_rows();
@@ -341,7 +410,7 @@
         int sc = 0;
         for (int kc = 0; kc < nk; ++kc) {
             const int sn = (sc + 1 == NST) ? 0 : sc + 1;
-            kstep<0>(smem + sc * STAGE, smem + sn * STAGE, kc, nk);
+            kstep<0, EPI>(smem + sc * STAGE, smem + sn * STAGE, kc, nk);
             sc = sn;
             if constexpr (GNF) gnf_advance(kc);
         }
@@ -524,8 +593,26 @@
         const bool ok = n < p.To;
         const long long o0 = (long long)b * Ck * Tpo + k4p_off(tile0, n);
         float* ob = p.out + o0;
-        if (ok) {
-            if constexpr (VOC) {
+        if constexpr (!VOC) {
+            k4p_f32x4 ent[4];
+            k4p_tile_entries(acc[0][i][j], ent);
+            const __amdgpu_buffer_rsrc_t ro = __builtin_amdgcn_make_buffer_rsrc(p.out + (long long)b * Ck * Tpo, 0, Ck * Tpo * 4, 0x00020000);
+            const int e0 = k4p_entry_off(tile0 >> 3, h, Tpo, n + p.opad);
+            if (ok) {
+#pragma unroll
+                for (int g = 0; g < 4; ++g) k4p_store16_wt(ro, e0 + g * 2 * Tpo * 16, ent[g]);
+                if (p.opad == 1) {
+                    if (n == 0) {
+#pragma unroll
+                        for (int g = 0; g < 4; ++g) k4p_store16(ro, e0 + g * 2 * Tpo * 16 - 16, k4p_f32x4{0.f, 0.f, 0.f, 0.f});
+                    }
+                    if (n == p.To - 1) {
+#pragma unroll
+                        for (int g = 0; g < 4; ++g) k4p_store16(ro, e0 + g * 2 * Tpo * 16 + 16, k4p_f32x4{0.f, 0.f, 0.f, 0.f});
+                    }
+                }
+            }
+        } else if (ok) {
             if constexpr (BN < 256) {
                 if (p.vlen && n >= voc_len()) {
 #pragma unroll
@@ -546,7 +633,6 @@
             if (p.act_slope != 0.f) {
 #pragma unroll
                 for (int r = 0; r < 16; ++r) { const float v = acc[0][i][j][r]; acc[0][i][j][r] = (v >= 0.f) ? v : v * p.act_slope; }
-            }
             }
 #pragma unroll
             for (int g = 0; g < 4; ++g)
@@ -742,8 +828,9 @@
 __global__ void __launch_bounds__(256, ((VOC && KT == 2) ? 2 : DmaCfg<BM, BN, KT, STRIDE, UPS, BK, NST, DIL>::OCC)) conv_dma_kernel(const DmaConvArgs p) {
     extern __shared__ __attribute__((aligned(16))) float smem[];
     DmaKernel<BM, BN, KT, STRIDE, UPS, BK, NST, DIL, VOC, GNF, GELU, ACT2> k(p, smem);
-    k.setup();
+    k.setup_keep_acc();
     if (!k.dead_tile()) k.mainloop();
+    else k.zero_acc();
     k.epilogue();
 }
 
@@ -766,8 +853,9 @@
     K1 k1(pp.a1, smem);
     {
         K3 k3(pp.a3, smem);
-        k3.setup();
-        if (!k3.dead_tile()) k3.mainloop();
+        k3.setup_keep_acc();
+        if (!k3.dead_tile()) k3.template mainloop<false, true>();
+        else k3.zero_acc();
 #pragma unroll
         for (int a = 0; a < K3::NACC; ++a)
 #pragma unroll
@@ -777,15 +865,21 @@
     }
     __syncthreads();
     k1.setup_keep_acc();
-    if (!k1.dead_tile()) k1.mainloop();
+    if (!k1.dead_tile()) k1.template mainloop<true, false>();
     k1.epilogue();
+}
+
+static void dma_set_order(DmaConvArgs& a, int nMb, int nN, int S) {
+    const DmaMagic m0 = dma_magic((unsigned)nMb), m1 = dma_magic((unsigned)nN), m2 = dma_magic((unsigned)S);
+    a.ord_m[0] = m0.m; a.ord_m[1] = m1.m; a.ord_m[2] = m2.m;
+    a.ord_s = m0.s | (m1.s << 8) | (m2.s << 16);
 }
 
 static thread_local char g_dcfg[96] = "";
 const char* conv_dma_last_config() { return g_dcfg; }
 
 template <int BM, int BN, int KT, int STRIDE, bool UPS, int BK, int NST, int DIL = 1, bool VOC = false, bool GNF = false, bool GELU = false, int ACT2 = 0>
-static hipError_t launch_dma_cfg(const DmaConvArgs& a, hipStream_t s) {
+static hipError_t launch_dma_cfg(DmaConvArgs& a, hipStream_t s) {
     using Cfg = DmaCfg<BM, BN, KT, STRIDE, UPS, BK, NST, DIL>;
     if (GNF != (a.gnf_part != nullptr) || GELU != (a.epi == EPI_GELU) || (ACT2 == 1) != (a.epi == EPI_SWISH) || (ACT2 == 2) != (a.epi == EPI_GLU)) return hipErrorInvalidValue;
     const size_t lds_bytes = Cfg::LDS_BYTES + (GNF ? (BM + 32) * sizeof(float) : 0);
@@ -793,6 +887,7 @@
     const int S = a.ksplit > 1 ? a.ksplit : 1;
     if (S > 1 && (Cfg::TM * Cfg::TN > 2 || VOC || (a.Ci / BK) % S)) return hipErrorInvalidValue;
     dim3 grid((a.Mp / BM) * nN, a.B * S);
+    dma_set_order(a, a.Mp / BM, nN, S);
     auto kern = conv_dma_kernel<BM, BN, KT, STRIDE, UPS, BK, NST, DIL, VOC, GNF, GELU, ACT2>;
     if (lds_bytes > 48 * 1024) {
         static std::atomic<unsigned long long> attr_done{0};
@@ -870,12 +965,14 @@
 }
 
 template <int BM, int BN, int BK3, int BK1, int NST>
-static hipError_t launch_pair_cfg(const DmaConvArgs& a3, const DmaConvArgs& a1, hipStream_t s) {
+static hipError_t launch_pair_cfg(DmaConvArgs& a3, DmaConvArgs& a1, hipStream_t s) {
     using Cfg = PairCfg<BM, BN, BK3, BK1, NST>;
     const int nN = (a1.To + BN - 1) / BN;
     const int S = a1.ksplit > 1 ? a1.ksplit : 1;
     if (S > 1 && (Cfg::C1::TM * Cfg::C1::TN != 1 || a3.ksplit != a1.ksplit || (a3.Ci / BK3) % S || (a1.Ci / BK1) % S)) return hipErrorInvalidValue;
     dim3 grid((a1.Mp / BM) * nN, a1.B * S);
+    dma_set_order(a3, a1.Mp / BM, nN, S);
+    dma_set_order(a1, a1.Mp / BM, nN, S);
     auto kern = conv_dma_pair_kernel<BM, BN, BK3, BK1, NST>;
     if (Cfg::LDS_BYTES > 48 * 1024) {
         static std::atomic<unsigned long long> attr_done{0};
@@ -1076,3 +1173,21 @@
 }
 
 }
+
+extern "C" int lds_test_dma_magic_div(uint32_t d, uint32_t n_count, uint32_t* out) {
+    if (d < 1 || d >= (1u << 31) || n_count > (1u << 31) || !out) return (int)hipErrorInvalidValue;
+    const lds::DmaMagic m = lds::dma_magic(d);
+    for (uint32_t n = 0; n < n_count; ++n) out[n] = lds::dma_magic_div(n, m.m, m.s);
+    return 0;
+}
+extern "C" int lds_test_dma_tile_order(int nMb, int nN, int B, int S, int32_t* out) {
+    if (nMb < 1 || nN < 1 || B < 1 || S < 1 || !out || (long long)nMb * nN * B * S >= (1ll << 31)) return (int)hipErrorInvalidValue;
+    lds::DmaConvArgs a{};
+    lds::dma_set_order(a, nMb, nN, S);
+    const int total = nMb * nN * B * S;
+    for (int id = 0; id < total; ++id) {
+        const lds::DmaTile t = lds::dma_tile_of(id, total, nMb, nN, S, a.ord_m, a.ord_s);
+        out[4 * id] = t.mb; out[4 * id + 1] = t.nb; out[4 * id + 2] = t.b; out[4 * id + 3] = t.ksp;
+    }
+    return 0;
+}
diff --git a/latent-diffusion-speech_amd/csrc/k4p.h b/latent-diffusion-speech_amd/csrc/k4p.h
--- a/latent-diffusion-speech_amd/csrc/k4p.h
+++ b/latent-diffusion-speech_amd/csrc/k4p.h
@@ -13,6 +13,27 @@
     __hip_atomic_store(reinterpret_cast<unsigned long long*>(p), __builtin_bit_cast(unsigned long long, v), __ATOMIC_RELAXED, __HIP_MEMORY_SCOPE_AGENT);
 }
 
+typedef float k4p_f32x4 __attribute__((ext_vector_type(4)));
+typedef float k4p_f32x16 __attribute__((ext_vector_type(16)));
+typedef unsigned k4p_u32x4 __attribute__((ext_vector_type(4)));
+static __device__ __forceinline__ void k4p_tile_entries(const k4p_f32x16& acc, k4p_f32x4 (&e)[4]) {
+#pragma unroll
+    for (int g = 0; g < 4; ++g) {
+        const float r0 = acc[4 * g], r1 = acc[4 * g + 1], r2 = acc[4 * g + 2], r3 = acc[4 * g + 3];
+        const auto s01 = __builtin_amdgcn_permlane32_swap(__builtin_bit_cast(unsigned, r0), __builtin_bit_cast(unsigned, r1), false, false);
+        const auto s23 = __builtin_amdgcn_permlane32_swap(__builtin_bit_cast(unsigned, r2), __builtin_bit_cast(unsigned, r3), false, false);
+        const unsigned u0 = s01[0], u1 = s23[0], u2 = s01[1], u3 = s23[1];
+        e[g] = k4p_f32x4{__builtin_bit_cast(float, u0), __builtin_bit_cast(float, u1), __builtin_bit_cast(float, u2), __builtin_bit_cast(float, u3)};
+    }
+}
+static __device__ __forceinline__ int k4p_entry_off(int q, int h, int Tp, int e) { return ((q * 2 + h) * Tp + e) * 16; }
+static __device__ __forceinline__ void k4p_store16_wt(__amdgpu_buffer_rsrc_t r, int off, k4p_f32x4 v) {
+    __builtin_amdgcn_raw_buffer_store_b128(__builtin_bit_cast(k4p_u32x4, v), r, off, 0, 16);
+}
+static __device__ __forceinline__ void k4p_store16(__amdgpu_buffer_rsrc_t r, int off, k4p_f32x4 v) {
+    __builtin_amdgcn_raw_buffer_store_b128(__builtin_bit_cast(k4p_u32x4, v), r, off, 0, 0);
+}
+
 static __device__ __forceinline__ int ragged_len(const int* lens, int b, int lvl, int T) {
     if (!lens) return T;
     int n = lens[b];
diff --git a/latent-diffusion-speech_amd/csrc/kernels.h b/latent-diffusion-speech_amd/csrc/kernels.h
--- a/latent-diffusion-speech_amd/csrc/kernels.h
+++ b/latent-diffusion-speech_amd/csrc/kernels.h
@@ -102,7 +102,26 @@
     int ksplit;
     float* kpart; unsigned* kcount;
     long long kpart_cap; int kcount_cap;
-};
+    unsigned ord_m[3], ord_s;
+};
+struct DmaMagic { unsigned m, s; };
+inline DmaMagic dma_magic(unsigned d) {
+    unsigned s = 0;
+    while ((1ull << s) < d) ++s;
+    return DmaMagic{(unsigned)((1ull << (31 + s)) / d + 1), s};
+}
+__host__ __device__ inline unsigned dma_magic_div(unsigned n, unsigned m, unsigned s) {
+    return (unsigned)(((unsigned long long)(n << 1) * m) >> 32) >> s;
+}
+struct DmaTile { int mb, nb, b, ksp; };
+inline DmaTile dma_tile_of(int id, int total, int nMb, int nN, int S, const unsigned* ord_m, unsigned ord_s) {
+    const int xcd = id & 7, slot = id >> 3, per = total >> 3, rem = total & 7;
+    const unsigned L = (unsigned)(xcd * per + (xcd < rem ? xcd : rem) + slot);
+    const unsigned tb = dma_magic_div(L, ord_m[0], ord_s & 255);
+    const unsigned by = dma_magic_div(tb, ord_m[1], (ord_s >> 8) & 255);
+    const unsigned b = dma_magic_div(by, ord_m[2], (ord_s >> 16) & 255);
+    return DmaTile{(int)(L - tb * nMb), (int)(tb - by * nN), (int)b, (int)(by - b * S)};
+}
 hipError_t launch_conv_dma(const DmaConvArgs& a, int cfg, hipStream_t s);
 hipError_t launch_conv_dma_pair(const DmaConvArgs& a3, const DmaConvArgs& a1, hipStream_t s);
 bool conv_dma_pair_applies(const DmaConvArgs& a3, const DmaConvArgs& a1);
diff --git a/latent-diffusion-speech_amd/csrc/model.hip b/latent-diffusion-speech_amd/csrc/model.hip
--- a/latent-diffusion-speech_amd/csrc/model.hip
+++ b/latent-diffusion-speech_amd/csrc/model.hip
@@ -3164,6 +3164,24 @@
     float* f(size_t n) { void* d = nullptr; if (hipMalloc(&d, n * sizeof(float) + 65536) != hipSuccess) return nullptr; p.push_back(d); return (float*)d; }
 };
 
+static thread_local float* g_tap_dst = nullptr;
+static thread_local size_t g_tap_floats = 0;
+extern "C" int lds_test_tap_k4p(float* dst, size_t floats) {
+    if ((dst != nullptr) != (floats > 0)) return fail(LDS_EINVAL, "bad argument");
+    g_tap_dst = dst; g_tap_floats = floats;
+    return LDS_OK;
+}
+static hipError_t tap_fill(float* k, size_t floats, hipStream_t st) {
+    return g_tap_dst ? hipMemsetAsync(k, 0xff, floats * sizeof(float), st) : hipSuccess;
+}
+static hipError_t tap_take(const float* k, size_t floats, hipStream_t st) {
+    if (!g_tap_dst) return hipSuccess;
+    float* dst = g_tap_dst;
+    g_tap_dst = nullptr;
+    if (floats != g_tap_floats) return hipErrorInvalidValue;
+    return hipMemcpyAsync(dst, k, floats * sizeof(float), hipMemcpyDeviceToDevice, st);
+}
+
 static int dconv_test_impl(const lds_dconv_test* a, float* out, float* lnpart, int B, int iters, float* ms_out, void* stream, int bf3 = 0, int nprod = 0, int fmt = 0,
                            const int* alt_cfgs = nullptr, int n_alt = 0) {
     hipStream_t st = (hipStream_t)stream;
@@ -3209,6 +3227,8 @@
         if (a->v_split > 1) o.vt_D = a->v_split;
     }
     o.lnpart_out = (float2*)lnpart;
+    const bool tap = !bf3 && !a->plain_out;
+    if (tap) HIP_TRY(tap_fill(kout, (size_t)B * Ck * (To + 2), st));
     auto run = [&]() { return bf3 ? run_dconv_bf3(W, k1, a->C1, k2, a->C2, T, o, kout, B, st, nprod, fmt) : run_dconv(W, k1, a->C1, k2, a->C2, T, o, kout, B, st); };
     int r = run();
     if (r == LDS_OK && iters > 0 && ms_out) {
@@ -3229,6 +3249,7 @@
         (void)hipEventDestroy(e1);
     }
     auto from_out = [&](const float* src, float* dst, int C, int Tl) { return qk_f32 ? launch_from_k4p(src, dst, B, C, Tl, st) : from_act(src, dst, C, Tl); };
+    if (r == LDS_OK && tap) HIP_TRY(tap_take(kout, (size_t)B * Ck * (To + 2), st));
     if (r == LDS_OK && !a->plain_out) {
         if (a->v_split > 1) {
             HIP_TRY(from_out(kout, out, Ck, To));
@@ -3506,12 +3527,14 @@
     float* part = tmp.f((size_t)B * (C / 32) * T * 2);
     if (!kx || !km || !ko || !part) return fail(LDS_ENOMEM, "alloc");
     HIP_TRY(launch_to_k4p(x, kx, B, C, T, C, 0, st));
+    HIP_TRY(tap_fill(ko, (size_t)B * Co * (T + 2), st));
     DOpt o1;
     o1.lnpart_out = (float2*)part;
     LDS_TRY(run_dconv(W1, kx, C, nullptr, 0, T, o1, km, B, st));
     DOpt o2;
     o2.ln_part = (const float2*)part; o2.ln_np = C / 32; o2.ln_eps = eps; o2.ln_c1 = c1; o2.ln_c2 = c2;
     LDS_TRY(run_dconv(W2, km, C, nullptr, 0, T, o2, ko, B, st));
+    HIP_TRY(tap_take(ko, (size_t)B * Co * (T + 2), st));
     HIP_TRY(launch_from_k4p(km, mid, B, C, T, st));
     HIP_TRY(launch_from_k4p(ko, out, B, Co, T, st));
     HIP_TRY(hipStreamSynchronize(st));
@@ -3583,8 +3606,10 @@
     }
     HIP_TRY(launch_to_k4p(qkp, kqk, B, 2 * C, T, 2 * C, 0, st));
     HIP_TRY(launch_plain_to_vt(vpl, vt, B, C, T, C / heads, st));
+    HIP_TRY(tap_fill(ko, (size_t)B * C * (T + 2), st));
     if (f16math) HIP_TRY(launch_attention_k4p_f16math(kqk, vt, ko, B, C, T, heads, st, tile_batch));
     else HIP_TRY(launch_attention_k4p(kqk, vt, ko, B, C, T, heads, st, tile_batch));
+    HIP_TRY(tap_take(ko, (size_t)B * C * (T + 2), st));
     HIP_TRY(launch_from_k4p(ko, out, B, C, T, st));
     HIP_TRY(hipStreamSynchronize(st));
     return LDS_OK;
@@ -3790,6 +3815,7 @@
     if (rc == 1) rc = fail(LDS_EINVAL, "dconv pair: no fused variant for Cm %d C1 %d C2 %d Co %d T %d (fmt %d, tile_batch %d)", Cm, C1, C2, Co, T, fmt, tile_batch);
     if (rc == LDS_OK) {
         if (cfg_out && cfg_cap) snprintf(cfg_out, cfg_cap, "%s", f32 ? conv_dma_last_config() : conv_bf3_last_config());
+        if (f32) HIP_TRY(tap_take(ko, act.floats(Co, T), st));
         HIP_TRY(act.from(ko, out, Co, T));
     }
     HIP_TRY(hipStreamSynchronize(st));
@@ -3861,6 +3887,7 @@
     }
     if (rc == LDS_OK) {
         if (cfg_out && cfg_cap) snprintf(cfg_out, cfg_cap, "%s", f32 ? conv_dma_last_config() : conv_bf3_last_config());
+        if (f32) HIP_TRY(tap_take(ko, act.floats(a->Co, To), st));
         HIP_TRY(act.from(ko, out, a->Co, To));
     }
     HIP_TRY(hipStreamSynchronize(st));
diff --git a/latent-diffusion-speech_amd/lds/native.py b/latent-diffusion-speech_amd/lds/native.py
--- a/latent-diffusion-speech_amd/lds/native.py
+++ b/latent-diffusion-speech_amd/lds/native.py
@@ -187,6 +187,9 @@
 lds_test_lm_beam_step            i:piiiiiifiippppppppppppppppp
 lds_test_dconv_pair              i:pppppppiiiiiipiiipppzp
 lds_test_dconv_ex                i:pppipzp
+lds_test_dma_magic_div           i:uup
+lds_test_dma_tile_order          i:iiiip
+lds_test_tap_k4p                 i:pz
 lds_test_voc_ups                 i:pppiiiiiipppppzp
 lds_test_w2v_conv0               i:ppppppfpiiqp
 lds_test_w2v_ln_act              i:ppppfppiiip
```

Measured after the change: 24380 mel-frames/s (median of 6 runs). 1.6% higher.
